# HorizonRobotics/HoloAgent

Hardware: AMD Instinct MI355X
Metric: HMSG frames/sec (one scene per GPU: map A1-A2, fusion A3-A5, merge A6, pooling A7, floors A8, rooms by the device watershed N1, room clouds, room embeddings and View nodes A9, objects with the view <-> object test A10 and graph assembly A11, nothing handed in -- plus 1000 coarse-to-fine retrieval qu (higher is better)
Workload: dtype f64 geometry / f32 features

## Files before the change

### holoagent_amd/csrc/hmsg_api.hip

```cpp
#include "hmsg_common.h"
#include "hmsg_ckdtree.h"
#include "hmsg_nn.h"

#include <algorithm>
#include <cstring>

void hmsg_bitset_and_fp(hmsg_ctx* h, int first, int n, int M, const unsigned char* d_masks, const float* d_fg,
                        const float* d_fm, const float* d_fc, const int* d_nmask);

__global__ void k_nn_patch(const long long* __restrict__ qid, const int* __restrict__ val, unsigned n, int* __restrict__ target) {
    const unsigned i = blockIdx.x * blockDim.x + threadIdx.x;
    if (i < n) target[qid[i]] = val[i];
}

void hmsg_kd_join(hmsg_ctx* h) {
    if (h->kd_thread.joinable()) h->kd_thread.join();
}

void hmsg_kd_start(hmsg_ctx* h) {
    hmsg_kd_join(h);
    h->host_pts.resize((size_t)h->V * 3);
    if (h->V) HIP_TRY(hipMemcpyAsync(h->host_pts.data(), h->pts.p, (size_t)h->V * 24, hipMemcpyDeviceToHost, h->stream));
    HIP_TRY(hipStreamSynchronize(h->stream));
    h->kd = std::make_shared<CKDTree>();
    std::shared_ptr<CKDTree> kd = h->kd;
    const double* pts = h->host_pts.data();
    const long long V = h->V;
    h->kd_thread = std::thread([kd, pts, V] { kd->build(pts, V); });
}

bool hmsg_resolve_ties(hmsg_ctx* h, TieBuf& tb, int* target) {
    unsigned n = 0;
    HIP_TRY(hipMemcpyAsync(&n, tb.count.p, 4, hipMemcpyDeviceToHost, h->stream));
    HIP_TRY(hipStreamSynchronize(h->stream));
    if (n == 0) return true;
    if (n > tb.cap) {
        tb.cap = 0;
        tb.prepare(h->stream, n + n / 2 + 1024);
        return false;
    }
    std::vector<TieRec> recs(n);
    HIP_TRY(hipMemcpy(recs.data(), tb.recs.p, (size_t)n * sizeof(TieRec), hipMemcpyDeviceToHost));
    hmsg_kd_join(h);
    std::vector<long long> q(n);
    std::vector<int> v(n);
    for (unsigned i = 0; i < n; ++i) {
        const double x[3] = {recs[i].x, recs[i].y, recs[i].z};
        q[i] = recs[i].qid;
        v[i] = (int)h->kd->query1(x);
    }
    tb.pq.ensure(n);
    tb.pv.ensure(n);
    HIP_TRY(hipMemcpyAsync(tb.pq.p, q.data(), (size_t)n * 8, hipMemcpyHostToDevice, h->stream));
    HIP_TRY(hipMemcpyAsync(tb.pv.p, v.data(), (size_t)n * 4, hipMemcpyHostToDevice, h->stream));
    hipLaunchKernelGGL(k_nn_patch, dim3(cdiv(n, 256)), dim3(256), 0, h->stream, (const long long*)tb.pq.p, (const int*)tb.pv.p, n,
                       target);
    HMSG_CHECK_LAUNCH();
    HIP_TRY(hipStreamSynchronize(h->stream));
    h->n_tie_queries += n;
    return true;
}

namespace {

void copy_in(void* dst, const void* src, size_t bytes, hipStream_t s) {
    if (!bytes) return;
    HIP_TRY(hipMemcpyAsync(dst, src, bytes, hmsg_is_device_ptr(src) ? hipMemcpyDeviceToDevice : hipMemcpyHostToDevice, s));
}

template <typename F>
int guard(hmsg_ctx* h, F&& fn) {
    try {
        if (h) HIP_TRY(hipSetDevice(h->cfg.device_id));
        fn();
        return HMSG_OK;
    } catch (const hmsg_error& e) {
        if (h) h->err = e.msg;
        return e.code;
    } catch (const std::exception& e) {
        if (h) h->err = e.what();
        return HMSG_ERR_INVALID;
    } catch (...) {
        if (h) h->err = "unknown error";
        return HMSG_ERR_INVALID;
    }
}

static const size_t FRAME_STORE_LARGE = (size_t)96 << 30;
void alloc_frame_store(hmsg_ctx* h) {
    const size_t HW = (size_t)h->cfg.height * h->cfg.width, F = (size_t)h->cfg.max_frames, NW = (size_t)h->NW;
    const size_t b_rgb = HW * 3 * F, b_depth = HW * 2 * F, b_bits = HW * NW * 8 * F, b_nn = HW * 4 * F;
    auto up = [](size_t v) { return (v + ((size_t)1 << 21) - 1) & ~(((size_t)1 << 21) - 1); };
    if (b_rgb + b_depth + b_bits + b_nn >= FRAME_STORE_LARGE) {
        h->frame_arena.alloc(up(b_rgb) + up(b_depth) + up(b_bits) + up(b_nn));
        unsigned char* p = h->frame_arena.p;
        h->rgb.view(p, HW * 3 * F);
        p += up(b_rgb);
        h->depth.view((unsigned short*)p, HW * F);
        p += up(b_depth);
        h->bits.view((unsigned long long*)p, HW * NW * F);
        p += up(b_bits);
        h->nn.view((int*)p, HW * F);
    } else {
        h->rgb.alloc(HW * 3 * F);
        h->depth.alloc(HW * F);
    }
}

void release_frame_store_if_large(hmsg_ctx* h) {
    const size_t bytes = h->rgb.bytes() + h->depth.bytes() + h->bits.bytes() + h->nn.bytes();
    if (bytes < FRAME_STORE_LARGE || h->n_fused < h->n_feat_frames) return;
    HIP_TRY(hipStreamSynchronize(h->stream));
    h->rgb.release();
    h->depth.release();
    h->bits.release();
    h->nn.release();
    h->frame_arena.release();
    h->frames_released = true;
    if (h->fold_pipe) dev_cache().trim();
}

}

extern "C" {

const char* hmsg_version(void) { return "hmsg-mi355x 0.1 (gfx950)"; }

void hmsg_default_config(hmsg_config* c) {
    memset(c, 0, sizeof(*c));
    c->device_id = 0;
    c->feat_dim = 512;
    c->height = 480;
    c->width = 640;
    c->max_frames = 1024;
    c->max_masks = 64;
    c->voxel_size = 0.05;
    c->depth_scale = 1000.0;
    c->init_overlap_thresh = 0.75;
    c->overlap_thresh_factor = 0.025;
    c->iou_thresh = 0.05;
    c->clip_masked_weight = 0.4418;
    c->max_mask_distance = 10000.0;
    c->merge_type = HMSG_MERGE_SEQUENTIAL;
    c->outlier_nb_points = 1000;
    c->outlier_radius = 1.0;
    c->pool_max_dist = 0.8;
    c->feat_dbscan_eps = 0.01;
    c->feat_dbscan_min = 100;
    c->merge_dbscan_eps = 0.1;
    c->merge_dbscan_min = 10;
    c->min_instance_points = 10;
    c->skip_frames = 1;
    c->depth_cut = 0.0;
    c->grid_resolution = 0.05;
    c->overlap_distance_form = HMSG_OVERLAP_DIRECT;
}

size_t hmsg_config_size(void) { return sizeof(hmsg_config); }

int hmsg_create(const hmsg_config* cfg, hmsg_t** out) {
    if (!cfg || !out) return HMSG_ERR_INVALID;
    *out = nullptr;
    if (cfg->feat_dim <= 0 || cfg->height <= 0 || cfg->width <= 0 || cfg->max_frames <= 0 || cfg->voxel_size <= 0 ||
        cfg->max_masks <= 0 || cfg->max_masks > 256)
        return HMSG_ERR_INVALID;
    hmsg_ctx* h = new hmsg_ctx();
    h->cfg = *cfg;
    h->NW = (cfg->max_masks + 63) / 64;
    h->MS = h->NW * 64;
    int rc = guard(h, [&] {
        int ndev = 0;
        HIP_TRY(hipGetDeviceCount(&ndev));
        HMSG_REQUIRE(cfg->device_id >= 0 && cfg->device_id < ndev, HMSG_ERR_INVALID, "device_id out of range");
        HIP_TRY(hipSetDevice(cfg->device_id));
        HIP_TRY(hipStreamCreateWithFlags(&h->stream, hipStreamNonBlocking));
        alloc_frame_store(h);
        h->pose.alloc((size_t)16 * cfg->max_frames);
    });
    if (rc != HMSG_OK) {
        fprintf(stderr, "hmsg_create: %s\n", h->err.c_str());
        delete h;
        return rc;
    }
    *out = h;
    return HMSG_OK;
}

void hmsg_destroy(hmsg_t* h) {
    if (!h) return;
    hmsg_kd_join(h);
    (void)hipSetDevice(h->cfg.device_id);
    try {
        hmsg_fold_pipe_abort(h);
    } catch (...) {
    }
    h->fold_cache.trim();
    if (h->stream) {
        (void)hipStreamSynchronize(h->stream);
        (void)hipStreamDestroy(h->stream);
    }
    delete h;
}

const char* hmsg_last_error(const hmsg_t* h) { return h ? h->err.c_str() : "null handle"; }

void hmsg_release_cached_memory(void) { dev_cache().trim(); }

int hmsg_reset(hmsg_t* h) {
    if (!h) return HMSG_ERR_INVALID;
    return guard(h, [&] {
        HIP_TRY(hipStreamSynchronize(h->stream));
        hmsg_kd_join(h);
        hmsg_fold_pipe_abort(h);
        h->n_tie_queries = 0;
        h->n_frames = h->n_feat_frames = h->n_fused = 0;
        h->n_offered = 0;
        h->room_n = 0;
        h->room_total = 0;
        if (h->frames_released) {
            alloc_frame_store(h);
            h->frames_released = false;
        }
        h->nmask.clear();
        h->mask_first.clear();
        h->have_K = false;
        h->map_ready = h->feats_final = h->merged = h->pooled = h->inst_denoised = h->tree_partial = false;
        h->frame_window = 0;
        h->nodes.clear();
        h->V = h->V0 = 0;
        h->masks3d.off.clear();
        h->masks3d.total = 0;
        h->inst.off.clear();
        h->inst.total = 0;
        h->prof.clear();
    });
}

int hmsg_set_profiling(hmsg_t* h, int32_t on) {
    if (!h) return HMSG_ERR_INVALID;
    h->prof.enabled = on != 0;
    h->prof.detail = on >= 2;
    return HMSG_OK;
}

static void prof_aggregate(hmsg_ctx* h, std::vector<std::string>& names, std::vector<long long>& cnt, std::vector<double>& ms,
                           std::vector<double>* work = nullptr) {
    (void)hipStreamSynchronize(h->stream);
    for (auto& e : h->prof.ev) {
        float t = 0.f;
        if (hipEventElapsedTime(&t, e.a, e.b) != hipSuccess) continue;
        size_t k = 0;
        for (; k < names.size(); ++k)
            if (names[k] == e.name) break;
        if (k == names.size()) {
            names.push_back(e.name);
            cnt.push_back(0);
            ms.push_back(0.0);
            if (work) work->push_back(0.0);
        }
        cnt[k]++;
        ms[k] += t;
        if (work) (*work)[k] += e.work;
    }
}

int32_t hmsg_profile_count(hmsg_t* h) {
    if (!h) return 0;
    std::vector<std::string> n;
    std::vector<long long> c;
    std::vector<double> m;
    prof_aggregate(h, n, c, m);
    return (int32_t)n.size();
}

int hmsg_profile_entry(hmsg_t* h, int32_t i, char* name, int64_t* launches, double* total_ms, double* total_work) {
    if (!h || !name || !launches || !total_ms) return HMSG_ERR_INVALID;
    std::vector<std::string> n;
    std::vector<long long> c;
    std::vector<double> m, w;
    prof_aggregate(h, n, c, m, &w);
    if (i < 0 || i >= (int32_t)n.size()) return HMSG_ERR_INVALID;
    snprintf(name, 64, "%s", n[i].c_str());
    *launches = c[i];
    *total_ms = m[i];
    if (total_work) *total_work = w[i];
    return HMSG_OK;
}

__global__ void k_depth_cut(unsigned short* __restrict__ depth, size_t n, double limit) {
    const size_t i = (size_t)blockIdx.x * blockDim.x + threadIdx.x;
    if (i < n && (double)depth[i] > limit) depth[i] = 0;
}

int hmsg_add_frames(hmsg_t* h, int32_t n, const uint8_t* rgb, const uint16_t* depth, const double* pose, const double* K) {
    if (!h) return HMSG_ERR_INVALID;
    return guard(h, [&] {
        HMSG_REQUIRE(n >= 0 && rgb && depth && pose && K, HMSG_ERR_INVALID, "hmsg_add_frames: null argument");
        HMSG_REQUIRE(!h->map_ready, HMSG_ERR_INVALID, "hmsg_add_frames after hmsg_finalize_map");
        HMSG_REQUIRE(!h->frames_released, HMSG_ERR_INVALID, "hmsg_add_frames: the frame store was released (hmsg_reset first)");
        double Kh[9];
        if (hmsg_is_device_ptr(K)) {
            HIP_TRY(hipMemcpy(Kh, K, sizeof(Kh), hipMemcpyDeviceToHost));
        } else {
            memcpy(Kh, K, sizeof(Kh));
        }
        if (h->have_K)
            HMSG_REQUIRE(memcmp(Kh, h->K, sizeof(Kh)) == 0, HMSG_ERR_UNSUPPORTED, "intrinsics must be the same for all frames");
        memcpy(h->K, Kh, sizeof(Kh));
        h->have_K = true;
        h->cam = CamK{Kh[0], Kh[4], Kh[2], Kh[5]};
        const size_t HW = (size_t)h->cfg.height * h->cfg.width;
        const int skip = std::max(1, h->cfg.skip_frames);
        int kept = 0;
        if (skip == 1) {
            HMSG_REQUIRE(h->n_frames + n <= h->cfg.max_frames, HMSG_ERR_INVALID, "frame store full (cfg.max_frames)");
            copy_in(h->rgb.p + (size_t)h->n_frames * HW * 3, rgb, (size_t)n * HW * 3, h->stream);
            copy_in(h->depth.p + (size_t)h->n_frames * HW, depth, (size_t)n * HW * 2, h->stream);
            copy_in(h->pose.p + (size_t)h->n_frames * 16, pose, (size_t)n * 16 * 8, h->stream);
            kept = n;
        } else {
            for (int i = 0; i < n; ++i) {
                if ((h->n_offered + i) % skip != 0) continue;
                HMSG_REQUIRE(h->n_frames + kept < h->cfg.max_frames, HMSG_ERR_INVALID, "frame store full (cfg.max_frames)");
                const size_t f = (size_t)h->n_frames + kept;
                copy_in(h->rgb.p + f * HW * 3, rgb + (size_t)i * HW * 3, HW * 3, h->stream);
                copy_in(h->depth.p + f * HW, depth + (size_t)i * HW, HW * 2, h->stream);
                copy_in(h->pose.p + f * 16, pose + (size_t)i * 16, 16 * 8, h->stream);
                ++kept;
            }
        }
        h->n_offered += n;
        if (h->cfg.depth_cut > 0.0 && kept > 0) {
            const size_t cnt = (size_t)kept * HW;
            hipLaunchKernelGGL(k_depth_cut, dim3(cdiv(cnt, 256)), dim3(256), 0, h->stream, h->depth.p + (size_t)h->n_frames * HW, cnt,
                               h->cfg.depth_cut * h->cfg.depth_scale);
            HMSG_CHECK_LAUNCH();
        }
        HIP_TRY(hipStreamSynchronize(h->stream));
        h->n_frames += kept;
    });
}

int hmsg_finalize_map(hmsg_t* h) {
    if (!h) return HMSG_ERR_INVALID;
    return guard(h, [&] {
        HMSG_REQUIRE(!h->map_ready, HMSG_ERR_INVALID, "map already finalised");
        hmsg_build_map(h);
    });
}
// ... 8 lines not shown
    return guard(h, [&] {
        HMSG_REQUIRE(h->map_ready, HMSG_ERR_INVALID, "map not finalised");
        if (xyz) d2h_bounce(xyz, h->pts.p, (size_t)h->V * 24);
        if (rgb) d2h_bounce(rgb, h->cols.p, (size_t)h->V * 24);
    });
}

int hmsg_add_frame_features(hmsg_t* h, int32_t first, int32_t n, int32_t M, const uint8_t* masks, const float* F_g,
                            const float* F_masked, const float* F_crop, const int32_t* n_masks) {
    if (!h) return HMSG_ERR_INVALID;
    return guard(h, [&] {
        HMSG_REQUIRE(n >= 0 && F_g, HMSG_ERR_INVALID, "hmsg_add_frame_features: null argument");
        HMSG_REQUIRE(M >= 0 && M <= h->cfg.max_masks, HMSG_ERR_INVALID, "M out of range (cfg.max_masks, <= 256)");
        HMSG_REQUIRE(M == 0 || (masks && F_masked && F_crop), HMSG_ERR_INVALID, "hmsg_add_frame_features: null argument");
        HMSG_REQUIRE(first == h->n_feat_frames, HMSG_ERR_INVALID, "frames must be handed over in order (first == #frames so far)");
        HMSG_REQUIRE(first + n <= h->n_frames, HMSG_ERR_INVALID, "features for a frame without geometry");
        HMSG_REQUIRE(!h->frames_released, HMSG_ERR_INVALID, "hmsg_add_frame_features: the frame store was released (hmsg_reset first)");
        if (n == 0) return;
        const size_t HW = (size_t)h->cfg.height * h->cfg.width;
        const int D = h->cfg.feat_dim;
        const size_t NW = (size_t)h->NW, MS = (size_t)h->MS;
        if (h->bits.n < (size_t)h->cfg.max_frames * HW * NW) h->bits.alloc((size_t)h->cfg.max_frames * HW * NW);
        if (h->fp.n < (size_t)h->cfg.max_frames * MS * D) h->fp.alloc((size_t)h->cfg.max_frames * MS * D);
        std::vector<int> nm((size_t)n, M);
        if (n_masks) {
            if (hmsg_is_device_ptr(n_masks)) {
                HIP_TRY(hipMemcpy(nm.data(), n_masks, (size_t)n * 4, hipMemcpyDeviceToHost));
            } else {
                memcpy(nm.data(), n_masks, (size_t)n * 4);
            }
            for (int v : nm) HMSG_REQUIRE(v >= 0 && v <= M, HMSG_ERR_INVALID, "n_masks[f] must be in [0, M]");
        }
        DevBuf<int> d_nm;
        d_nm.alloc((size_t)n);
        HIP_TRY(hipMemcpyAsync(d_nm.p, nm.data(), (size_t)n * 4, hipMemcpyHostToDevice, h->stream));
        if (M == 0) {
            HIP_TRY(hipMemsetAsync(h->bits.p + (size_t)first * HW * NW, 0, (size_t)n * HW * NW * 8, h->stream));
            HIP_TRY(hipStreamSynchronize(h->stream));
            h->nmask.insert(h->nmask.end(), nm.begin(), nm.end());
            h->n_feat_frames += n;
            return;
        }
        const bool dev = hmsg_is_device_ptr(masks);
        const int chunk = dev ? n : std::max(1, (int)(((size_t)512 << 20) / ((size_t)M * HW)));
        DevBuf<unsigned char> st_m;
        DevBuf<float> st_f;
        for (int c0 = 0; c0 < n; c0 += chunk) {
            int nc = std::min(chunk, n - c0);
            const unsigned char* dm = masks + (size_t)c0 * M * HW;
            const float *dg = F_g + (size_t)c0 * D, *dfm = F_masked + (size_t)c0 * M * D, *dfc = F_crop + (size_t)c0 * M * D;
            if (!dev) {
                st_m.ensure((size_t)nc * M * HW);
                HIP_TRY(hipMemcpyAsync(st_m.p, dm, (size_t)nc * M * HW, hipMemcpyHostToDevice, h->stream));
                dm = st_m.p;
            }
            if (!hmsg_is_device_ptr(F_g) || !hmsg_is_device_ptr(F_masked) || !hmsg_is_device_ptr(F_crop)) {
                st_f.ensure((size_t)nc * (2 * M + 1) * D);
                float* g = st_f.p;
                float* fm = g + (size_t)nc * D;
                float* fc = fm + (size_t)nc * M * D;
                copy_in(g, dg, (size_t)nc * D * 4, h->stream);
                copy_in(fm, dfm, (size_t)nc * M * D * 4, h->stream);
                copy_in(fc, dfc, (size_t)nc * M * D * 4, h->stream);
                dg = g;
                dfm = fm;
                dfc = fc;
            }
            hmsg_bitset_and_fp(h, first + c0, nc, M, dm, dg, dfm, dfc, d_nm.p + c0);
            HIP_TRY(hipStreamSynchronize(h->stream));
        }
        h->nmask.insert(h->nmask.end(), nm.begin(), nm.end());
        h->n_feat_frames += n;
    });
}

int hmsg_set_frame_window(hmsg_t* h, int32_t first_frame) {
    if (!h) return HMSG_ERR_INVALID;
    return guard(h, [&] {
        HMSG_REQUIRE(h->map_ready, HMSG_ERR_INVALID, "hmsg_set_frame_window: call hmsg_finalize_map first");
        HMSG_REQUIRE(h->n_feat_frames == 0 && h->n_fused == 0, HMSG_ERR_INVALID, "hmsg_set_frame_window: features already handed over");
        HMSG_REQUIRE(first_frame >= 0 && first_frame <= h->n_frames, HMSG_ERR_INVALID, "hmsg_set_frame_window: frame out of range");
        h->frame_window = first_frame;
        h->n_feat_frames = h->n_fused = first_frame;
        h->nmask.assign((size_t)first_frame, 0);
        h->mask_first.assign((size_t)first_frame + 1, 0);
        h->masks3d.off.assign(1, 0);
        h->masks3d.total = 0;
    });
}

int hmsg_merge_tree_local(hmsg_t* h, int32_t total_frames, double* th_next, int64_t* lists_now, int64_t* my_index) {
    if (!h || !th_next || !lists_now || !my_index) return HMSG_ERR_INVALID;
    return guard(h, [&] {
        long long l = 0, i = 0;
        hmsg_fold_pipe_abort(h);
        release_frame_store_if_large(h);
        hmsg_merge_tree_local_impl(h, total_frames, th_next, &l, &i);
        *lists_now = l;
        *my_index = i;
    });
}

int hmsg_merge_tree_join(hmsg_t* h, int32_t n_ext, const int64_t* ext_sizes, const double* ext_points, double th, int32_t final_pass) {
    if (!h) return HMSG_ERR_INVALID;
    return guard(h, [&] { hmsg_merge_tree_join_impl(h, n_ext, (const long long*)ext_sizes, ext_points, th, final_pass); });
}

int hmsg_fuse_frames(hmsg_t* h) {
    if (!h) return HMSG_ERR_INVALID;
    return guard(h, [&] { hmsg_fuse(h); });
}

int hmsg_get_map_feats(const hmsg_t* hc, float* feats, float* counter) {
    hmsg_ctx* h = const_cast<hmsg_ctx*>(hc);
    if (!h) return HMSG_ERR_INVALID;
    return guard(h, [&] {
        HMSG_REQUIRE(h->feats_final, HMSG_ERR_INVALID, "hmsg_fuse_frames not run");
        if (feats) d2h_bounce(feats, h->feats.p, (size_t)h->V * h->cfg.feat_dim * 4);
        if (counter) {
            std::vector<unsigned> c((size_t)h->V);
            HIP_TRY(hipMemcpy(c.data(), h->cnt.p, (size_t)h->V * 4, hipMemcpyDeviceToHost));
            for (long long i = 0; i < h->V; ++i) counter[i] = (float)c[i];
        }
    });
}

__global__ void k_feats_refresh(const float* __restrict__ sum, const unsigned* __restrict__ cnt, long long V, int D,
                                float* __restrict__ feats) {
    size_t t = (size_t)blockIdx.x * blockDim.x + threadIdx.x;
    if (t >= (size_t)V * D) return;
    unsigned c = cnt[t / D];
    float d = c == 0u ? 1e-5f : (float)c;
    feats[t] = __fdiv_rn(sum[t], d);
}

int hmsg_get_feature_sums(const hmsg_t* hc, float* sum, uint32_t* counter) {
    hmsg_ctx* h = const_cast<hmsg_ctx*>(hc);
    if (!h) return HMSG_ERR_INVALID;
    return guard(h, [&] {
        HMSG_REQUIRE(h->feats_final, HMSG_ERR_INVALID, "hmsg_fuse_frames not run");
        const size_t n = (size_t)h->V * h->cfg.feat_dim;
        if (sum && n) HIP_TRY(hipMemcpyAsync(sum, h->sum.p, n * 4, hmsg_is_device_ptr(sum) ? hipMemcpyDeviceToDevice : hipMemcpyDeviceToHost, h->stream));
        if (counter && h->V)
            HIP_TRY(hipMemcpyAsync(counter, h->cnt.p, (size_t)h->V * 4, hmsg_is_device_ptr(counter) ? hipMemcpyDeviceToDevice : hipMemcpyDeviceToHost, h->stream));
        HIP_TRY(hipStreamSynchronize(h->stream));
    });
}

int hmsg_set_feature_sums(hmsg_t* h, const float* sum, const uint32_t* counter) {
    if (!h) return HMSG_ERR_INVALID;
    return guard(h, [&] {
        HMSG_REQUIRE(h->feats_final && sum && counter, HMSG_ERR_INVALID, "hmsg_set_feature_sums: run hmsg_fuse_frames first");
        HMSG_REQUIRE(!h->pooled, HMSG_ERR_INVALID, "hmsg_set_feature_sums after hmsg_pool_instances");
        const size_t n = (size_t)h->V * h->cfg.feat_dim;
        copy_in(h->sum.p, sum, n * 4, h->stream);
        copy_in(h->cnt.p, counter, (size_t)h->V * 4, h->stream);
        if (n) hipLaunchKernelGGL(k_feats_refresh, dim3(cdiv(n, 256)), dim3(256), 0, h->stream, (const float*)h->sum.p,
                                  (const unsigned*)h->cnt.p, (long long)h->V, h->cfg.feat_dim, h->feats.p);
        HMSG_CHECK_LAUNCH();
        HIP_TRY(hipStreamSynchronize(h->stream));
    });
}

int hmsg_get_frame_nn(const hmsg_t* hc, int32_t frame, int32_t* idx) {
    hmsg_ctx* h = const_cast<hmsg_ctx*>(hc);
    if (!h) return HMSG_ERR_INVALID;
    return guard(h, [&] {
        HMSG_REQUIRE(frame >= 0 && frame < h->n_fused && idx, HMSG_ERR_INVALID, "frame not fused");
        HMSG_REQUIRE(!h->frames_released, HMSG_ERR_INVALID, "hmsg_get_frame_nn: the frame store was released by the merge (very long episode)");
        const size_t HW = (size_t)h->cfg.height * h->cfg.width;
        HIP_TRY(hipMemcpy(idx, h->nn.p + (size_t)frame * HW, HW * 4, hipMemcpyDeviceToHost));
    });
}

int hmsg_get_frame_fp(const hmsg_t* hc, int32_t frame, float* f_p) {
    hmsg_ctx* h = const_cast<hmsg_ctx*>(hc);
    if (!h) return HMSG_ERR_INVALID;
    return guard(h, [&] {
        HMSG_REQUIRE(frame >= 0 && frame < h->n_feat_frames && f_p, HMSG_ERR_INVALID, "frame has no features");
        const size_t D = (size_t)h->cfg.feat_dim, n = (size_t)h->nmask[frame] * D;
        if (n) HIP_TRY(hipMemcpy(f_p, h->fp.p + (size_t)frame * h->MS * D, n * 4, hipMemcpyDeviceToHost));
    });
}

int32_t hmsg_get_frame_num_masks(const hmsg_t* h, int32_t frame) {
    return (h && frame >= 0 && frame < h->n_feat_frames) ? h->nmask[frame] : -1;
}

int hmsg_get_frame_mask_sizes(const hmsg_t* hc, int32_t frame, int64_t* sizes) {
    hmsg_ctx* h = const_cast<hmsg_ctx*>(hc);
    if (!h) return HMSG_ERR_INVALID;
    return guard(h, [&] {
        HMSG_REQUIRE(frame >= 0 && frame < h->n_fused && sizes, HMSG_ERR_INVALID, "frame not fused");
        for (int i = 0; i < h->nmask[frame]; ++i) {
            size_t k = (size_t)h->mask_first[frame] + i;
            sizes[i] = h->masks3d.off[k + 1] - h->masks3d.off[k];
        }
    });
}

int hmsg_get_frame_mask_points(const hmsg_t* hc, int32_t frame, double* xyz) {
    hmsg_ctx* h = const_cast<hmsg_ctx*>(hc);
    if (!h) return HMSG_ERR_INVALID;
    return guard(h, [&] {
        HMSG_REQUIRE(frame >= 0 && frame < h->n_fused && xyz, HMSG_ERR_INVALID, "frame not fused");
        long long a = h->masks3d.off[(size_t)h->mask_first[frame]], b = h->masks3d.off[(size_t)h->mask_first[frame + 1]];
        if (b > a) d2h_bounce(xyz, h->masks3d.pts.p + (size_t)a * 3, (size_t)(b - a) * 24);
    });
}

int hmsg_merge_instances(hmsg_t* h) {
    if (!h) return HMSG_ERR_INVALID;
    return guard(h, [&] {
        release_frame_store_if_large(h);
        hmsg_merge(h);
    });
}

int64_t hmsg_num_instances(const hmsg_t* h) { return h && (h->merged || h->tree_partial) ? (int64_t)h->inst.off.size() - 1 : -1; }

int hmsg_get_instance_sizes(const hmsg_t* hc, int64_t* sizes) {
    hmsg_ctx* h = const_cast<hmsg_ctx*>(hc);
    if (!h) return HMSG_ERR_INVALID;
    return guard(h, [&] {
        HMSG_REQUIRE((h->merged || h->tree_partial) && sizes, HMSG_ERR_INVALID, "hmsg_merge_instances not run");
        for (size_t i = 0; i + 1 < h->inst.off.size(); ++i) sizes[i] = h->inst.off[i + 1] - h->inst.off[i];
    });
}

int hmsg_get_instance_points(const hmsg_t* hc, double* xyz) {
    hmsg_ctx* h = const_cast<hmsg_ctx*>(hc);
    if (!h) return HMSG_ERR_INVALID;
    return guard(h, [&] {
        HMSG_REQUIRE((h->merged || h->tree_partial) && xyz, HMSG_ERR_INVALID, "hmsg_merge_instances not run");
        if (h->inst.total) {
            if (hmsg_is_device_ptr(xyz)) {
                HIP_TRY(hipMemcpyAsync(xyz, h->inst.pts.p, (size_t)h->inst.total * 24, hipMemcpyDeviceToDevice, h->stream));
                HIP_TRY(hipStreamSynchronize(h->stream));
            } else
                d2h_bounce(xyz, h->inst.pts.p, (size_t)h->inst.total * 24);
        }
    });
}

int hmsg_denoise_instances(hmsg_t* h, double eps, int32_t min_points) {
    if (!h) return HMSG_ERR_INVALID;
    return guard(h, [&] {
        hmsg_denoise_inst(h, eps, min_points);
        if (eps == 0.05 && min_points == 10) h->inst_denoised = true;
    });
}

int hmsg_voxel_down_sample(hmsg_t* h, const double* points, int64_t n, double voxel_size, double* out_points, int64_t* out_n) {
    if (!h) return HMSG_ERR_INVALID;
    return guard(h, [&] {
        HMSG_REQUIRE((points || n == 0) && out_points && out_n, HMSG_ERR_INVALID, "hmsg_voxel_down_sample: null argument");
        *out_n = (int64_t)hmsg_voxel_ds(h, points, (long long)n, voxel_size, out_points);
    });
}

int hmsg_instance_room_share(hmsg_t* h, int32_t n_rooms, const int64_t* vert_off, const double* verts_xz, double radius,
                             double* share) {
    if (!h) return HMSG_ERR_INVALID;
    return guard(h, [&] {
        HMSG_REQUIRE(n_rooms >= 0 && vert_off && verts_xz && share && radius > 0, HMSG_ERR_INVALID,
                     "hmsg_instance_room_share: bad argument");
        hmsg_room_share(h, n_rooms, (const long long*)vert_off, verts_xz, radius, share);
    });
}

int hmsg_get_instance_boxes(const hmsg_t* hc, double* boxes) {
    hmsg_ctx* h = const_cast<hmsg_ctx*>(hc);
    if (!h) return HMSG_ERR_INVALID;
    return guard(h, [&] {
        HMSG_REQUIRE(h->merged && boxes, HMSG_ERR_INVALID, "hmsg_merge_instances not run");
        if (!h->inst.box.empty()) memcpy(boxes, h->inst.box.data(), h->inst.box.size() * 8);
    });
}

int hmsg_pool_instances(hmsg_t* h) {
    if (!h) return HMSG_ERR_INVALID;
    return guard(h, [&] { hmsg_pool(h); });
}

int hmsg_get_instance_feats(const hmsg_t* hc, float* feats) {
    hmsg_ctx* h = const_cast<hmsg_ctx*>(hc);
    if (!h) return HMSG_ERR_INVALID;
    return guard(h, [&] {
        HMSG_REQUIRE(h->pooled && feats, HMSG_ERR_INVALID, "hmsg_pool_instances not run");
        size_t n = (h->inst.off.size() - 1) * (size_t)h->cfg.feat_dim;
        if (n) d2h_bounce(feats, h->inst_feats.p, n * 4);
    });
}

int hmsg_test_ckdtree(const double* pts, int64_t n, const double* queries, int64_t nq, int64_t* out_idx,
                      int64_t* out_indices, int64_t* out_n_nodes) {
    if (!pts || n < 0 || nq < 0) return HMSG_ERR_INVALID;
    CKDTree t;
    t.build(pts, n);
    if (out_indices) memcpy(out_indices, t.indices.data(), (size_t)n * 8);
    if (out_n_nodes) *out_n_nodes = (int64_t)t.nodes.size();
    for (int64_t i = 0; i < nq; ++i) out_idx[i] = t.query1(queries + i * 3);
    return HMSG_OK;
}

}
// ... 1 lines not shown
```

### holoagent_amd/csrc/hmsg_comm.hip

```cpp
#include "hmsg_common.h"

#include <dlfcn.h>

#include <algorithm>

#include <functional>
#include <mutex>

__global__ void k_cm_gather_rows(const float* __restrict__ src, const int* __restrict__ row, int n, int D, float* __restrict__ dst) {
    const size_t t = (size_t)blockIdx.x * blockDim.x + threadIdx.x;
    if (t >= (size_t)n * D) return;
    dst[t] = src[(size_t)row[t / D] * D + t % D];
}
__global__ void k_cm_feats_refresh(const float* __restrict__ sum, const unsigned* __restrict__ cnt, long long V, int D, float* __restrict__ feats) {
    const size_t t = (size_t)blockIdx.x * blockDim.x + threadIdx.x;
    if (t >= (size_t)V * D) return;
    const unsigned c = cnt[t / D];
    const float d = c == 0u ? 1e-5f : (float)c;
    feats[t] = __fdiv_rn(sum[t], d);
}

namespace {

typedef void* rcclComm_t;
// ... 112 lines not shown
        if (err) *err = "unknown error";
        return HMSG_ERR_INVALID;
    }
}
}

extern "C" {

int hmsg_comm_unique_id(uint8_t* out_id) {
    if (!out_id) return HMSG_ERR_INVALID;
    return comm_guard(&g_comm_err, [&] {
        rccl_need();
        rcclUniqueId id;
        rccl_try(rccl().GetUniqueId(&id), "ncclGetUniqueId");
        memcpy(out_id, id.internal, sizeof(id.internal));
    });
}

int hmsg_comm_create(const uint8_t* id, int32_t rank, int32_t world, int32_t device_id, hmsg_comm_t** out) {
    if (!out) return HMSG_ERR_INVALID;
    *out = nullptr;
    if (world < 1 || rank < 0 || rank >= world) return HMSG_ERR_INVALID;
    hmsg_comm* c = nullptr;
    const int rc = comm_guard(&g_comm_err, [&] {
        c = new hmsg_comm();
        c->rank = rank;
        c->world = world;
        c->device = device_id;
        if (id == nullptr) {
            HMSG_REQUIRE(world == 1, HMSG_ERR_INVALID, "hmsg_comm_create: more than one rank needs the id of hmsg_comm_unique_id");
            return;
        }
        rccl_need();
        HIP_TRY(hipSetDevice(device_id));
        rcclUniqueId uid;
        memcpy(uid.internal, id, sizeof(uid.internal));
        rccl_try(rccl().CommInitRank(&c->comm, world, uid, rank), "ncclCommInitRank");
        HIP_TRY(hipMalloc((void**)&c->flag, 64));
        HIP_TRY(hipMalloc((void**)&c->hdr, (size_t)world * HMSG_COMM_HDR_BYTES));
    });
    if (rc != HMSG_OK) {
        delete c;
        return rc;
    }
    *out = c;
    return HMSG_OK;
}

void hmsg_comm_destroy(hmsg_comm_t* c) {
    if (!c) return;
    if (c->comm) (void)rccl().CommDestroy(c->comm);
    if (c->flag) (void)hipFree(c->flag);
    if (c->hdr) (void)hipFree(c->hdr);
    delete c;
}

const char* hmsg_comm_last_error(const hmsg_comm_t* c) { return c ? c->err.c_str() : g_comm_err.c_str(); }

int hmsg_allgather_nodes(hmsg_t* h, hmsg_comm_t* c, int32_t n_rooms_local, hmsg_index_t** out_index, int64_t* node_off, int64_t* room_off) {
    if (!h || !c || !out_index) return HMSG_ERR_INVALID;
    *out_index = nullptr;
    int rc_index = HMSG_OK;
    const int rc = comm_guard(&h->err, [&] {
        HIP_TRY(hipSetDevice(h->cfg.device_id));
        hipStream_t s = h->stream;
        const int W = c->world, D = h->cfg.feat_dim;
        const long long n = (long long)h->nodes.size();
        std::string mine;
        if (n_rooms_local < 0) mine = "hmsg_allgather_nodes: negative room count";
        for (long long k = 0; k < n && mine.empty(); ++k)
            if (h->nodes[(size_t)k].room < 0 || h->nodes[(size_t)k].room >= n_rooms_local) mine = "hmsg_allgather_nodes: a node's room lies outside n_rooms_local";
        if (n && !h->pooled) mine = "hmsg_allgather_nodes: run hmsg_pool_instances first";
        if (!all_ranks_ok(c, mine.empty(), s))
            throw hmsg_error{HMSG_ERR_INVALID, mine.empty() ? "hmsg_allgather_nodes: another rank's node table is invalid (see its hmsg_last_error)" : mine};
        std::vector<long long> meta((size_t)W * 2, 0);
        meta[(size_t)c->rank * 2] = n;
        meta[(size_t)c->rank * 2 + 1] = n_rooms_local;
        if (c->comm) {
            DevBuf<long long> dm;
            dm.alloc((size_t)W * 2);
            HIP_TRY(hipMemcpyAsync(dm.p + (size_t)c->rank * 2, meta.data() + (size_t)c->rank * 2, 16, hipMemcpyHostToDevice, s));
            rccl_try(rccl().AllGather(dm.p + (size_t)c->rank * 2, dm.p, 2, RCCL_INT64, c->comm, s), "ncclAllGather (counts)");
            HIP_TRY(hipMemcpyAsync(meta.data(), dm.p, (size_t)W * 16, hipMemcpyDeviceToHost, s));
            HIP_TRY(hipStreamSynchronize(s));
        }
        std::vector<long long> noff((size_t)W + 1, 0), roff((size_t)W + 1, 0);
        long long nmax = 1;
        for (int r = 0; r < W; ++r) {
            noff[(size_t)r + 1] = noff[(size_t)r] + meta[(size_t)r * 2];
            roff[(size_t)r + 1] = roff[(size_t)r] + meta[(size_t)r * 2 + 1];
            nmax = std::max(nmax, meta[(size_t)r * 2]);
        }
        const long long N = noff[(size_t)W];
        if (node_off) for (int r = 0; r <= W; ++r) node_off[r] = noff[(size_t)r];
        if (room_off) for (int r = 0; r <= W; ++r) room_off[r] = roff[(size_t)r];
        HMSG_REQUIRE(N > 0, HMSG_ERR_INVALID, "hmsg_allgather_nodes: no nodes on any rank (hmsg_build_object_nodes)");
        DevBuf<float> emb;
        DevBuf<int> room;
        float* my_emb = nullptr;
        int* my_room = nullptr;
        local_phase_then_agree(c, s, "hmsg_allgather_nodes", [&] {
        emb.alloc((size_t)W * nmax * D);
        room.alloc((size_t)W * nmax);
        my_emb = emb.p + (size_t)c->rank * nmax * D;
        my_room = room.p + (size_t)c->rank * nmax;
        if (n) {
            std::vector<int> inst((size_t)n), rm((size_t)n);
            for (long long k = 0; k < n; ++k) {
                inst[(size_t)k] = h->nodes[(size_t)k].instance;
                rm[(size_t)k] = h->nodes[(size_t)k].room + (int)roff[(size_t)c->rank];
            }
            DevBuf<int> d_inst;
            d_inst.alloc((size_t)n);
            HIP_TRY(hipMemcpyAsync(d_inst.p, inst.data(), (size_t)n * 4, hipMemcpyHostToDevice, s));
            HIP_TRY(hipMemcpyAsync(my_room, rm.data(), (size_t)n * 4, hipMemcpyHostToDevice, s));
            hipLaunchKernelGGL(k_cm_gather_rows, dim3(cdiv((size_t)n * D, 256)), dim3(256), 0, s, (const float*)h->inst_feats.p, (const int*)d_inst.p,
                               (int)n, D, my_emb);
            HMSG_CHECK_LAUNCH();
            HIP_TRY(hipStreamSynchronize(s));
        }
        });
        if (c->comm) {
            rccl_try(rccl().AllGather(my_emb, emb.p, (size_t)nmax * D, RCCL_FLOAT32, c->comm, s), "ncclAllGather (embeddings)");
            rccl_try(rccl().AllGather(my_room, room.p, (size_t)nmax, RCCL_INT32, c->comm, s), "ncclAllGather (rooms)");
        }
        DevBuf<float> packed;
        DevBuf<int> proom;
        packed.alloc((size_t)N * D);
        proom.alloc((size_t)N);
        for (int r = 0; r < W; ++r) {
            const long long nr = meta[(size_t)r * 2];
            if (!nr) continue;
            HIP_TRY(hipMemcpyAsync(packed.p + (size_t)noff[(size_t)r] * D, emb.p + (size_t)r * nmax * D, (size_t)nr * D * 4, hipMemcpyDeviceToDevice, s));
            HIP_TRY(hipMemcpyAsync(proom.p + (size_t)noff[(size_t)r], room.p + (size_t)r * nmax, (size_t)nr * 4, hipMemcpyDeviceToDevice, s));
        }
        HIP_TRY(hipStreamSynchronize(s));
        rc_index = hmsg_index_create(h->cfg.device_id, D, N, packed.p, 0, proom.p, out_index);
        if (rc_index != HMSG_OK) throw hmsg_error{rc_index, "hmsg_allgather_nodes: hmsg_index_create failed"};
    });
    if (rc != HMSG_OK) c->err = h->err;
    return rc;
}

int hmsg_allreduce_feature_sums(hmsg_t* h, hmsg_comm_t* c) {
    if (!h || !c) return HMSG_ERR_INVALID;
    const int rc = comm_guard(&h->err, [&] {
        HIP_TRY(hipSetDevice(h->cfg.device_id));
        hipStream_t s = h->stream;
        std::string mine;
        if (!h->feats_final) mine = "hmsg_allreduce_feature_sums: run hmsg_fuse_frames first";
        else if (h->pooled) mine = "hmsg_allreduce_feature_sums after hmsg_pool_instances";
        if (!all_ranks_ok(c, mine.empty(), s))
            throw hmsg_error{HMSG_ERR_INVALID, mine.empty() ? "hmsg_allreduce_feature_sums: another rank is not ready (see its hmsg_last_error)" : mine};
        const size_t n = (size_t)h->V * h->cfg.feat_dim;
        if (c->comm && n) {
            rccl_try(rccl().AllReduce(h->sum.p, h->sum.p, n, RCCL_FLOAT32, RCCL_SUM, c->comm, s), "ncclAllReduce (feature sums)");
            rccl_try(rccl().AllReduce(h->cnt.p, h->cnt.p, (size_t)h->V, RCCL_UINT32, RCCL_SUM, c->comm, s), "ncclAllReduce (frame counters)");
        }
        if (n) hipLaunchKernelGGL(k_cm_feats_refresh, dim3(cdiv(n, 256)), dim3(256), 0, s, (const float*)h->sum.p, (const unsigned*)h->cnt.p,
                                  (long long)h->V, h->cfg.feat_dim, h->feats.p);
        HMSG_CHECK_LAUNCH();
        HIP_TRY(hipStreamSynchronize(s));
    });
    if (rc != HMSG_OK) c->err = h->err;
    return rc;
}

}

void hmsg_comm_allgather_bytes(hmsg_ctx* h, hmsg_comm* c, const void* mine, size_t my_bytes, std::vector<std::vector<char>>& all) {
    const int W = c->world;
    all.assign((size_t)W, std::vector<char>());
    if (!c->comm) {
        all[0].assign((const char*)mine, (const char*)mine + my_bytes);
        return;
    }
    hipStream_t s = h->stream;
    std::vector<long long> len((size_t)W, 0);
    len[(size_t)c->rank] = (long long)my_bytes;
    DevBuf<long long> dl;
    dl.alloc((size_t)W);
    HIP_TRY(hipMemcpyAsync(dl.p + c->rank, &len[(size_t)c->rank], 8, hipMemcpyHostToDevice, s));
    rccl_try(rccl().AllGather(dl.p + c->rank, dl.p, 1, RCCL_INT64, c->comm, s), "ncclAllGather (table lengths)");
    HIP_TRY(hipMemcpyAsync(len.data(), dl.p, (size_t)W * 8, hipMemcpyDeviceToHost, s));
    HIP_TRY(hipStreamSynchronize(s));
    long long mx = 1;
    for (long long v : len) mx = std::max(mx, v);
    mx = (mx + 15) & ~15ll;
    DevBuf<char> buf;
    buf.alloc((size_t)W * (size_t)mx);
    if (my_bytes) HIP_TRY(hipMemcpyAsync(buf.p + (size_t)c->rank * (size_t)mx, mine, my_bytes, hipMemcpyHostToDevice, s));
    rccl_try(rccl().AllGather(buf.p + (size_t)c->rank * (size_t)mx, buf.p, (size_t)mx, RCCL_INT8, c->comm, s), "ncclAllGather (tables)");
    std::vector<char> hostbuf((size_t)W * (size_t)mx);
    HIP_TRY(hipMemcpyAsync(hostbuf.data(), buf.p, hostbuf.size(), hipMemcpyDeviceToHost, s));
    HIP_TRY(hipStreamSynchronize(s));
    for (int r = 0; r < W; ++r) all[(size_t)r].assign(hostbuf.begin() + (ptrdiff_t)((size_t)r * (size_t)mx), hostbuf.begin() + (ptrdiff_t)((size_t)r * (size_t)mx + (size_t)len[(size_t)r]));
}
int hmsg_comm_rank(const hmsg_comm* c) { return c->rank; }
int hmsg_comm_world(const hmsg_comm* c) { return c->world; }
void hmsg_comm_set_error(hmsg_comm* c, const std::string& e) { c->err = e; }
int hmsg_comm_device(const hmsg_comm* c) { return c->device; }
void hmsg_comm_local_phase_then_agree(hmsg_comm* c, hipStream_t s, const char* what, const std::function<void()>& f) {
    if (!c) {
        f();
        return;
    }
    local_phase_then_agree(c, s, what, f);
}
void hmsg_comm_allgather_header(hmsg_comm* c, const void* mine, size_t bytes, void* all, hipStream_t s) {
    if (bytes > HMSG_COMM_HDR_BYTES) throw hmsg_error{HMSG_ERR_INVALID, "hmsg_comm_allgather_header: header too long"};
    if (!c->comm) {
        memcpy(all, mine, bytes);
        return;
    }
    HIP_TRY(hipMemcpyAsync(c->hdr + (size_t)c->rank * HMSG_COMM_HDR_BYTES, mine, bytes, hipMemcpyHostToDevice, s));
    rccl_try(rccl().AllGather(c->hdr + (size_t)c->rank * HMSG_COMM_HDR_BYTES, c->hdr, HMSG_COMM_HDR_BYTES, RCCL_INT8, c->comm, s), "ncclAllGather (header)");
    std::vector<char> h((size_t)c->world * HMSG_COMM_HDR_BYTES);
    HIP_TRY(hipMemcpyAsync(h.data(), c->hdr, h.size(), hipMemcpyDeviceToHost, s));
    HIP_TRY(hipStreamSynchronize(s));
    for (int r = 0; r < c->world; ++r) memcpy((char*)all + (size_t)r * bytes, h.data() + (size_t)r * HMSG_COMM_HDR_BYTES, bytes);
}
void hmsg_comm_allgather_inplace(hmsg_comm* c, void* buf, size_t slot_bytes, hipStream_t s) {
    if (!c->comm || !slot_bytes) return;
    char* b = (char*)buf;
    rccl_try(rccl().AllGather(b + (size_t)c->rank * slot_bytes, b, slot_bytes, RCCL_INT8, c->comm, s), "ncclAllGather (sharded query)");
}

extern "C" {

int hmsg_comm_send(hmsg_t* h, hmsg_comm_t* c, const void* dev_buf, int64_t bytes, int32_t dst) {
    if (!h || !c || bytes < 0 || (bytes && !dev_buf) || dst < 0 || dst >= c->world || dst == c->rank) return HMSG_ERR_INVALID;
    const int rc = comm_guard(&h->err, [&] {
        HMSG_REQUIRE(c->comm, HMSG_ERR_INVALID, "hmsg_comm_send: a communicator of one rank has nobody to send to");
        HIP_TRY(hipSetDevice(h->cfg.device_id));
        if (bytes) rccl_try(rccl().Send(dev_buf, (size_t)bytes, RCCL_INT8, dst, c->comm, h->stream), "ncclSend");
        HIP_TRY(hipStreamSynchronize(h->stream));
    });
    if (rc != HMSG_OK) c->err = h->err;
    return rc;
}
int hmsg_comm_recv(hmsg_t* h, hmsg_comm_t* c, void* dev_buf, int64_t bytes, int32_t src) {
    if (!h || !c || bytes < 0 || (bytes && !dev_buf) || src < 0 || src >= c->world || src == c->rank) return HMSG_ERR_INVALID;
    const int rc = comm_guard(&h->err, [&] {
        HMSG_REQUIRE(c->comm, HMSG_ERR_INVALID, "hmsg_comm_recv: a communicator of one rank has nobody to receive from");
        HIP_TRY(hipSetDevice(h->cfg.device_id));
        if (bytes) rccl_try(rccl().Recv(dev_buf, (size_t)bytes, RCCL_INT8, src, c->comm, h->stream), "ncclRecv");
        HIP_TRY(hipStreamSynchronize(h->stream));
    });
    if (rc != HMSG_OK) c->err = h->err;
    return rc;
}

int hmsg_merge_tree_sharded(hmsg_t* h, hmsg_comm_t* c, int32_t total_frames, int32_t* holds_result) {
    if (!h || !c || !holds_result) return HMSG_ERR_INVALID;
    *holds_result = 0;
    const int rc = comm_guard(&h->err, [&] {
        HIP_TRY(hipSetDevice(h->cfg.device_id));
        hipStream_t s = h->stream;
        const int W = c->world, me = c->rank;
        const double factor = h->cfg.overlap_thresh_factor;
        auto next_th = [&](double th, long long lists) { return lists > 1 ? th - factor * (double)(lists - 2) / (double)std::max<long long>(1, lists - 1) : th; };
        double th = 0.0;
        int64_t lists = 0, idx = 0;
        const int rc_local = hmsg_merge_tree_local(h, total_frames, &th, &lists, &idx);
        if (!all_ranks_ok(c, rc_local == HMSG_OK, s))
            throw hmsg_error{rc_local != HMSG_OK ? rc_local : HMSG_ERR_INVALID,
                             rc_local != HMSG_OK ? h->err : std::string("hmsg_merge_tree_sharded: another rank's local merge failed (see its hmsg_last_error)")};
        std::vector<long long> meta((size_t)W * 2, 0);
        meta[(size_t)me * 2] = lists;
        meta[(size_t)me * 2 + 1] = idx;
        if (c->comm) {
            DevBuf<long long> dm;
            dm.alloc((size_t)W * 2);
            HIP_TRY(hipMemcpyAsync(dm.p + (size_t)me * 2, meta.data() + (size_t)me * 2, 16, hipMemcpyHostToDevice, s));
            rccl_try(rccl().AllGather(dm.p + (size_t)me * 2, dm.p, 2, RCCL_INT64, c->comm, s), "ncclAllGather (tree levels)");
            HIP_TRY(hipMemcpyAsync(meta.data(), dm.p, (size_t)W * 16, hipMemcpyDeviceToHost, s));
            HIP_TRY(hipStreamSynchronize(s));
        }
        long long target = meta[0];
        for (int r = 0; r < W; ++r) target = std::min(target, meta[(size_t)r * 2]);
        std::vector<int> owner;
        for (int r = 0; r < W; ++r) {
            long long l = meta[(size_t)r * 2], i = meta[(size_t)r * 2 + 1];
            double t = th;
            while (l > target) {
                HMSG_REQUIRE(i == l - 1 && l % 2 == 1, HMSG_ERR_INVALID,
                             "hmsg_merge_tree_sharded: rank " + std::to_string(r) + "'s frame window is not a subtree of the merge tree");
                i /= 2;
                l = (l + 1) / 2;
                t = next_th(t, l);
            }
            if ((long long)owner.size() <= i) owner.resize((size_t)i + 1, -1);
            HMSG_REQUIRE(owner[(size_t)i] < 0, HMSG_ERR_INVALID, "hmsg_merge_tree_sharded: two ranks hold list " + std::to_string(i));
            owner[(size_t)i] = r;
            if (r == me) {
                th = t;
                lists = l;
                idx = i;
            }
        }
        HMSG_REQUIRE((long long)owner.size() == lists && std::find(owner.begin(), owner.end(), -1) == owner.end(), HMSG_ERR_INVALID,
                     "hmsg_merge_tree_sharded: the ranks' windows do not cover the lists of their common level");
        if (lists == 1) {
            if (owner[0] == me) {
                const int rj = hmsg_merge_tree_join(h, 0, nullptr, nullptr, th, 1);
                if (rj != HMSG_OK) throw hmsg_error{rj, h->err};
// ... 69 lines not shown
```

### holoagent_amd/csrc/hmsg_common.h

```cpp
#pragma once
#include <hip/hip_runtime.h>

#include <algorithm>
#include <chrono>
#include <cstdarg>
#include <cstdint>
#include <cstdio>
#include <cstdlib>
#include <cstring>
#include <map>
#include <memory>
#include <mutex>
#include <thread>
#include <string>
#include <vector>

#include "../../include/hmsg.h"
#include "../../include/hmsg_test.h"

#define HMSG_WAVE 64

struct hmsg_error {
    int code;
    std::string msg;
// ... 382 lines not shown
    return v;
}
__device__ __forceinline__ int wave_sum_i32(int v) {
    for (int o = 32; o > 0; o >>= 1) v += __shfl_xor(v, o);
    return v;
}

__device__ __forceinline__ double repeat_add(double s, double p, int len) {
    while (len > 0) {
        const double as = fabs(s), ap = fabs(p);
        if (ap == 0.0) return __dadd_rn(s, p);
        const long long bs = __double_as_longlong(as);
        const int e = (int)(bs >> 52);
        if (as >= ap && ((s < 0.0) == (p < 0.0)) && e >= 1 && e < 2046) {
            unsigned long long S = ((unsigned long long)bs & 0xfffffffffffffull) | (1ull << 52);
            const double q = ldexp(ap, 1075 - e);
            if (q < 0.5) return s;
            const double qi = floor(q), qf = q - qi;
            if (qf != 0.5) {
                const unsigned long long iq = (unsigned long long)qi;
                const unsigned long long d = iq + (qf > 0.5 ? 1ull : 0ull);
                const unsigned long long top = (1ull << 53) - 1ull;
                if (S + iq <= top) {
                    unsigned long long k = (unsigned long long)len;
                    const unsigned long long room = top - iq - S;
                    if (__umul64hi(k - 1ull, d) != 0ull || (k - 1ull) * d > room) k = room / d + 1ull;
                    S += k * d;
                    const double r = ldexp((double)S, e - 1075);
                    s = s < 0.0 ? -r : r;
                    len -= (int)k;
                    continue;
                }
            }
        }
        s = __dadd_rn(s, p);
        --len;
    }
    return s;
}

__device__ __forceinline__ double wave_bcast_f64(double v, int src) {
    const long long b = __double_as_longlong(v);
    const unsigned lo = (unsigned)__builtin_amdgcn_readlane((int)(unsigned)b, src);
    const unsigned hi = (unsigned)__builtin_amdgcn_readlane((int)(unsigned)((unsigned long long)b >> 32), src);
    return __longlong_as_double((long long)(((unsigned long long)hi << 32) | lo));
}

struct MaskCloudSet {
    DevBuf<double> pts;
    std::vector<long long> off;
    long long total = 0;
};

struct InstanceSet {
    DevBuf<double> pts;
    std::vector<long long> off;
    std::vector<double> box;
    long long total = 0;
};

struct ProfEntry {
    std::string name;
    hipEvent_t a, b;
    double work;
};
struct Prof {
    bool enabled = false;
    bool detail = false;
    std::vector<ProfEntry> ev;
    void clear() {
        for (auto& e : ev) {
            (void)hipEventDestroy(e.a);
            (void)hipEventDestroy(e.b);
        }
        ev.clear();
    }
};
struct ProfScope {
    Prof* p;
    hipStream_t s;
    size_t i = 0;
    ProfScope(Prof& pr, hipStream_t st, const char* name, double work = 0.0, bool fine = false) : ProfScope(&pr, st, name, work, fine) {}
    ProfScope(Prof* pr, hipStream_t st, const char* name, double work = 0.0, bool fine = false)
        : p(pr && pr->enabled && (!fine || pr->detail) ? pr : nullptr), s(st) {
        if (!p) return;
        ProfEntry e;
        e.name = name;
        e.work = work;
        (void)hipEventCreate(&e.a);
        (void)hipEventCreate(&e.b);
        (void)hipEventRecord(e.a, s);
        i = p->ev.size();
        p->ev.push_back(e);
    }
    ~ProfScope() {
        if (p) (void)hipEventRecord(p->ev[i].b, s);
    }
};

struct hmsg_ctx {
    Prof prof;
    hmsg_config cfg;
    hipStream_t stream = nullptr;
    std::string err;
    int n_frames = 0;
    long long n_offered = 0;
    int n_feat_frames = 0;
    int n_fused = 0;
    int MS = 0;
    int NW = 0;
    std::vector<int> nmask;
    std::vector<long long> mask_first;
    CamK cam;
    double K[9];
    bool have_K = false;
    DevBuf<unsigned char> rgb;
    DevBuf<unsigned short> depth;
    DevBuf<double> pose;
    DevBuf<unsigned long long> bits;
    DevBuf<float> fp;
    DevBuf<int> nn;
    DevBuf<unsigned char> frame_arena;
    bool map_ready = false;
    GridGeom grid;
    long long V0 = 0;
    long long V = 0;
    DevBuf<unsigned long long> bitmap;
    DevBuf<unsigned> rank;
    DevBuf<double> pts;
    DevBuf<double> cols;
    std::vector<double> host_pts;
    std::shared_ptr<struct CKDTree> kd;
    std::thread kd_thread;
    long long n_tie_queries = 0;
    DevBuf<unsigned long long> bitmap_rm;
    DevBuf<unsigned> rank_rm, cand_off;
    DevBuf<int> cand;
    bool have_cand = false;
    DevBuf<float> sum;
    DevBuf<unsigned> cnt;
    bool feats_final = false;
    DevBuf<float> feats;
    MaskCloudSet masks3d;
    InstanceSet inst;
    bool merged = false;
    int frame_window = 0;
    bool tree_partial = false;
    bool frames_released = false;
    DevBuf<float> inst_feats;
    bool pooled = false;
    std::shared_ptr<struct FoldPipe> fold_pipe;
    int fold_pipe_frames = 0;
    DevCache fold_cache;
    bool inst_denoised = false;
    std::vector<hmsg_node> nodes;
    DevBuf<int> room_sel, room_fmap;
    DevBuf<long long> room_off_dev;
    std::shared_ptr<void> room_scratch;
    int room_n = 0;
    long long room_total = 0;
    std::vector<int> node_label;
    DevBuf<unsigned> scan_tmp;
};

__device__ __forceinline__ unsigned long long scan_pack(unsigned epoch, unsigned flag, unsigned value) {
    return ((unsigned long long)((epoch << 2) | flag) << 32) | (unsigned long long)value;
}
__device__ __forceinline__ unsigned scan_lookback_prefix(unsigned long long* __restrict__ state, long long tile, unsigned epoch,
                                                         unsigned agg) {
    const int lane = threadIdx.x & 63;
    if (lane == 0)
        __hip_atomic_store(&state[tile], scan_pack(epoch, tile == 0 ? 2u : 1u, agg), __ATOMIC_RELAXED, __HIP_MEMORY_SCOPE_AGENT);
    unsigned prefix = 0;
    if (tile > 0) {
        long long hi = tile - 1;
        for (;;) {
            const long long idx = hi - lane;
            unsigned long long sw = scan_pack(epoch, 2u, 0u);
            if (idx >= 0) sw = __hip_atomic_load(&state[idx], __ATOMIC_RELAXED, __HIP_MEMORY_SCOPE_AGENT);
            const unsigned tag = (unsigned)(sw >> 32);
            const unsigned flag = (tag >> 2) == (epoch & 0x3fffffffu) ? (tag & 3u) : 0u;
            const unsigned long long has_prefix = __ballot(flag == 2u), not_ready = __ballot(flag == 0u);
            unsigned long long take = ~0ull;
            if (has_prefix) {
                const int first = __ffsll(has_prefix) - 1;
                take = first == 63 ? ~0ull : ((1ull << (first + 1)) - 1ull);
            }
            if (not_ready & take) continue;
            unsigned part = ((take >> lane) & 1ull) ? (unsigned)sw : 0u;
            for (int o = 32; o > 0; o >>= 1) part += __shfl_xor(part, o);
            prefix += part;
            if (has_prefix) break;
            hi -= 64;
        }
        if (lane == 0)
            __hip_atomic_store(&state[tile], scan_pack(epoch, 2u, prefix + agg), __ATOMIC_RELAXED, __HIP_MEMORY_SCOPE_AGENT);
    }
    return prefix;
}
unsigned hmsg_scan_epoch(DevBuf<unsigned>& tmp, size_t ntiles, hipStream_t s);
void hmsg_scan_u32(const unsigned* in, unsigned* out, size_t n, hipStream_t s, DevBuf<unsigned>& tmp,
                   unsigned long long* total);
unsigned long long hmsg_bitmap_rank(const unsigned long long* bitmap, unsigned* rank, size_t nwords, hipStream_t s,
                                    DevBuf<unsigned>& tmp);

struct SortBufs {
    DevBuf<unsigned> keys, keys_alt, hist, scan_tmp;
    DevBuf<unsigned long long> vals, vals_alt;
    unsigned* res_keys = nullptr;
    unsigned long long* res_vals = nullptr;
};
void hmsg_sort_pairs(SortBufs& b, size_t n, int key_bits, hipStream_t s);
void hmsg_sort_segment_starts(const unsigned* sorted_keys, size_t n, unsigned* off, unsigned nkeys, hipStream_t s);
static inline int bits_for(unsigned long long n) {
    int b = 1;
    while (b < 63 && (1ull << b) < n) ++b;
    return b;
}

struct DbgLaps {
    const char* tag;
    hipStream_t s;
    bool on;
    std::chrono::steady_clock::time_point t;
    DbgLaps(const char* tag_, hipStream_t s_) : tag(tag_), s(s_), on(getenv("HMSG_DEBUG_TIMING") != nullptr) {
        if (on) {
            (void)hipStreamSynchronize(s);
            t = std::chrono::steady_clock::now();
        }
    }
    void lap(const char* what) {
        if (!on) return;
        (void)hipStreamSynchronize(s);
        const auto n = std::chrono::steady_clock::now();
        fprintf(stderr, "[hmsg %s] %-26s %.3f ms\n", tag, what, std::chrono::duration<double, std::milli>(n - t).count());
        t = n;
    }
};

static inline void hmsg_dump(const char* name, const void* dev, size_t bytes, hipStream_t s) {
    const char* dir = getenv("HMSG_DEBUG_DUMP");
    if (!dir || !bytes) return;
    std::vector<char> host(bytes);
    (void)hipStreamSynchronize(s);
    (void)hipMemcpy(host.data(), dev, bytes, hipMemcpyDeviceToHost);
    std::string path = std::string(dir) + "/" + name + ".bin";
    if (FILE* f = fopen(path.c_str(), "wb")) {
        fwrite(host.data(), 1, bytes, f);
        fclose(f);
    }
}

void hmsg_kd_start(hmsg_ctx* h);
void hmsg_kd_join(hmsg_ctx* h);
void hmsg_build_map(hmsg_ctx* h);
void hmsg_fuse(hmsg_ctx* h);
void hmsg_merge(hmsg_ctx* h);
void hmsg_fold_pipe_feed(hmsg_ctx* h, int f0, int nfr);
void hmsg_fold_pipe_abort(hmsg_ctx* h);
void hmsg_merge_tree_local_impl(hmsg_ctx* h, int total_frames, double* th_next, long long* lists_now, long long* my_index);
void hmsg_merge_tree_join_impl(hmsg_ctx* h, int n_ext, const long long* ext_sizes, const double* ext_pts, double th, int final_pass);
void hmsg_denoise_inst(hmsg_ctx* h, double eps, int min_points);
void hmsg_room_share(hmsg_ctx* h, int R, const long long* vert_off, const double* verts_xz, double radius,
                     double* share_out);
void hmsg_pool(hmsg_ctx* h);
long long hmsg_voxel_ds(hmsg_ctx* h, const double* pts, long long n, double vs, double* out);
```

### holoagent_amd/csrc/hmsg_fuse.hip

```cpp
#include "hmsg_common.h"

#include <hip/hip_fp16.h>

#include <algorithm>
#include <cmath>

#define FB 64
#define MFIX_SCALE 17592186044416.0

__global__ void k_bitset(const unsigned char* __restrict__ masks, int M, size_t HW, int nfr, size_t mask_stride_frame,
                         const int* __restrict__ nmask, int NW, unsigned long long* __restrict__ bits) {
    const size_t chunks = (HW + 15) / 16;
    size_t t = (size_t)blockIdx.x * blockDim.x + threadIdx.x;
    if (t >= chunks * nfr) return;
    int f = (int)(t / chunks);
    size_t p0 = (t - (size_t)f * chunks) * 16;
    const unsigned char* mf = masks + (size_t)f * mask_stride_frame;
    const int nm = min(nmask[f], M);
    unsigned long long* o = bits + ((size_t)f * HW + p0) * NW;
    _Pragma("unroll") for (int w = 0; w < 4; ++w) if (w < NW) {
        unsigned long long b[16];
        for (int j = 0; j < 16; ++j) b[j] = 0ull;
        const int i0 = w * 64, i1 = min(nm, i0 + 64);
        if (p0 + 16 <= HW && (HW & 15) == 0) {
// ... 448 lines not shown
            const unsigned long long rec = recs[k];
            const double* p = pts + (size_t)(rec >> 8) * 3;
            s_len[k - c0] = (unsigned char)(rec & 255ull);
            s_v[k - c0] = (unsigned)(rec >> 8);
            s_p[k - c0][0] = p[0];
            s_p[k - c0][1] = p[1];
            s_p[k - c0][2] = p[2];
        }
        __syncthreads();
        const unsigned e = r1 < c1 ? r1 : c1;
        for (;;) {
            if (rem == 0) {
                if (r >= e) break;
                const unsigned i = r - c0;
                rem = (int)s_len[i];
                px = s_p[i][0];
                py = s_p[i][1];
                pz = s_p[i][2];
                ++r;
                while (r < e && s_v[r - c0] == s_v[i]) rem += (int)s_len[r++ - c0];
                n += (unsigned long long)rem;
                if (rem >= 256) {
                    sx = repeat_add(sx, px, rem);
                    sy = repeat_add(sy, py, rem);
                    sz = repeat_add(sz, pz, rem);
                    rem = 0;
                    continue;
                }
            }
            sx = __dadd_rn(sx, px);
            sy = __dadd_rn(sy, py);
            sz = __dadd_rn(sz, pz);
            --rem;
        }
        __syncthreads();
    }
    if (live) {
        const double dn = (double)n;
        out[(size_t)s * 3 + 0] = __ddiv_rn(sx, dn);
        out[(size_t)s * 3 + 1] = __ddiv_rn(sy, dn);
        out[(size_t)s * 3 + 2] = __ddiv_rn(sz, dn);
    }
}

__global__ void __launch_bounds__(256) k_mwalk_heavy(const unsigned* __restrict__ off, const unsigned long long* __restrict__ recs,
                                                     const double* __restrict__ pts, double* __restrict__ out,
                                                     const unsigned* __restrict__ heavy_cnt, const unsigned* __restrict__ heavy_list) {
    const int lane = threadIdx.x & 63;
    const unsigned nwaves = (gridDim.x * blockDim.x) >> 6, nheavy = *heavy_cnt;
    if (__ballot(1) == 0ull) return;
    const unsigned long long top = (1ull << 53) - 1ull;
    for (unsigned t = (blockIdx.x * blockDim.x + threadIdx.x) >> 6; t < nheavy; t += nwaves) {
        const unsigned slot = heavy_list[t];
        const unsigned r0 = off[slot], r1 = off[slot + 1];
        double res[3];
        unsigned long long n = 0;
        for (int c = 0; c < 3; ++c) {
            double s = 0.0;
            for (unsigned rb = r0; rb < r1; rb += 64) {
                const int cnt = (int)min(64u, r1 - rb);
                const unsigned long long rec = lane < cnt ? recs[rb + lane] : 0ull;
                const int len = (int)(rec & 255ull);
                const double p = lane < cnt ? pts[(size_t)(rec >> 8) * 3 + c] : 0.0;
                if (c == 0) {
                    int tl = len;
                    for (int o = 32; o > 0; o >>= 1) tl += __shfl_xor(tl, o);
                    n += (unsigned long long)tl;
                }
                int j0 = 0;
                while (j0 < cnt) {
                    const double as = fabs(s);
                    const long long bs = __double_as_longlong(as);
                    const int e = (int)(bs >> 52);
                    const unsigned long long S = ((unsigned long long)bs & 0xfffffffffffffull) | (1ull << 52);
                    const bool st_ok = e >= 1 && e < 2046;
                    const double ap = fabs(p);
                    bool ok = st_ok && lane >= j0 && lane < cnt && as >= ap && (ap == 0.0 || (p < 0.0) == (s < 0.0));
                    unsigned long long d = 0ull, iq = 0ull;
                    if (ok && ap != 0.0) {
                        const double q = ldexp(ap, 1075 - e);
                        if (q >= 0.5) {
                            const double qi = floor(q), qf = q - qi;
                            iq = (unsigned long long)qi;
                            d = iq + (qf > 0.5 ? 1ull : 0ull);
                            ok = qf != 0.5 && d < (1ull << 44);
                        }
                    }
                    const unsigned long long inc = ok ? (unsigned long long)len * d : 0ull;
                    unsigned long long pre = inc;
                    for (int o = 1; o < 64; o <<= 1) {
                        const unsigned long long u = __shfl_up(pre, o);
                        if (lane >= o) pre += u;
                    }
                    const bool fits = ok && S + pre - d + iq <= top;
                    const unsigned long long todo = ((cnt == 64 ? ~0ull : ((1ull << cnt) - 1ull)) >> j0) << j0;
                    const unsigned long long bad = ~__ballot(fits) & todo;
                    const int f = bad ? __ffsll(bad) - 1 : cnt;
                    if (f > j0) {
                        const unsigned long long add = __shfl(pre, f - 1);
                        const double rr = ldexp((double)(S + add), e - 1075);
                        s = s < 0.0 ? -rr : rr;
                    }
                    if (f < cnt) s = repeat_add(s, wave_bcast_f64(p, f), __builtin_amdgcn_readlane(len, f));
                    j0 = f + 1;
                }
            }
            res[c] = s;
        }
        if (lane == 0) {
            const double dn = (double)n;
            out[(size_t)slot * 3 + 0] = __ddiv_rn(res[0], dn);
            out[(size_t)slot * 3 + 1] = __ddiv_rn(res[1], dn);
            out[(size_t)slot * 3 + 2] = __ddiv_rn(res[2], dn);
        }
    }
}

__global__ void k_gather_u32(const unsigned* __restrict__ src, const long long* __restrict__ idx, int n, unsigned* __restrict__ dst) {
    int t = blockIdx.x * blockDim.x + threadIdx.x;
    if (t < n) dst[t] = src[idx[t]];
}

template <int VEC, int NJ>
static void launch_fuse(hmsg_ctx* h, const unsigned* stamp, int f0, int nfr) {
    const size_t HW = (size_t)h->cfg.height * h->cfg.width;
    hipLaunchKernelGGL((k_fuse<VEC, NJ>), dim3(cdiv((size_t)h->V * 64, 256)), dim3(256), 0, h->stream, stamp, h->V, f0, nfr,
                       h->MS, h->NW, h->cfg.feat_dim, HW, (const unsigned long long*)h->bits.p, (const float*)h->fp.p, h->sum.p,
                       h->cnt.p);
    HMSG_CHECK_LAUNCH();
}

static void dispatch_fuse(hmsg_ctx* h, const unsigned* stamp, int f0, int nfr) {
    const int D = h->cfg.feat_dim;
    if (D % 256 == 0 && D <= 1024) {
        switch (D / 256) {
            case 1: launch_fuse<4, 1>(h, stamp, f0, nfr); return;
            case 2: launch_fuse<4, 2>(h, stamp, f0, nfr); return;
            case 3: launch_fuse<4, 3>(h, stamp, f0, nfr); return;
            case 4: launch_fuse<4, 4>(h, stamp, f0, nfr); return;
        }
    }
    if (D <= 64) return launch_fuse<1, 1>(h, stamp, f0, nfr);
    if (D <= 128) return launch_fuse<1, 2>(h, stamp, f0, nfr);
    if (D <= 192) return launch_fuse<1, 3>(h, stamp, f0, nfr);
    if (D <= 256) return launch_fuse<1, 4>(h, stamp, f0, nfr);
    throw hmsg_error{HMSG_ERR_UNSUPPORTED, "feat_dim must be <= 256 or a multiple of 256 up to 1024"};
}

void hmsg_fuse(hmsg_ctx* h) {
    const hmsg_config& c = h->cfg;
    hipStream_t s = h->stream;
    HMSG_REQUIRE(h->map_ready, HMSG_ERR_INVALID, "hmsg_fuse_frames: call hmsg_finalize_map first");
    HMSG_REQUIRE(!h->feats_final || h->n_fused == h->n_feat_frames, HMSG_ERR_INVALID, "feature map already finalised");
    const int H = c.height, W = c.width, D = c.feat_dim, MS = h->MS, NW = h->NW;
    const size_t HW = (size_t)H * W;
    const long long V = h->V;
    const float scale = (float)c.depth_scale;
    if (h->sum.n < (size_t)V * D || h->n_fused == h->frame_window) {
        h->sum.alloc((size_t)V * D);
        h->cnt.alloc((size_t)V);
        h->sum.zero(s);
        h->cnt.zero(s);
    }
    if (h->nn.n < (size_t)c.max_frames * HW) h->nn.alloc((size_t)c.max_frames * HW);
    DevBuf<unsigned> stamp;
    stamp.alloc((size_t)std::max<long long>(V, 1) * FB);
    const int nmask_max = FB * MS;
    DevBuf<unsigned long long> d_bounds, d_dstat;
    d_bounds.alloc((size_t)nmask_max * 6);
    d_dstat.alloc((size_t)nmask_max * 2);
    DevBuf<MaskGeom> d_geom;
    d_geom.alloc((size_t)nmask_max);
    DevBuf<unsigned long long> mbitmap;
    DevBuf<unsigned> mrank, chunk_recs, rec_off, heavy, run_count;
    DevBuf<unsigned long long> runs;
    const unsigned heavy_thr = getenv("HMSG_DEBUG_MWALK_HEAVY") ? (unsigned)atoi(getenv("HMSG_DEBUG_MWALK_HEAVY")) : 32u;
    DevBuf<long long> d_offidx;
    DevBuf<unsigned> d_offval;
    d_offidx.alloc((size_t)nmask_max);
    d_offval.alloc((size_t)nmask_max);
    SortBufs sb;
    TieBuf ties;
    std::vector<unsigned long long> hb((size_t)nmask_max * 6), hd((size_t)nmask_max * 2);
    std::vector<MaskGeom> hg((size_t)nmask_max);
    std::vector<long long> hoffidx((size_t)nmask_max);
    std::vector<unsigned> hoffval((size_t)nmask_max);
    if (h->masks3d.off.empty()) h->masks3d.off.assign(1, 0);
    if (h->mask_first.empty()) h->mask_first.assign(1, 0);
    const double filt_mm = c.max_mask_distance * c.depth_scale;

    for (int fb0 = h->n_fused; fb0 < h->n_feat_frames; fb0 += FB) {
        const int nb = std::min(FB, h->n_feat_frames - fb0);
        stamp.zero(s);
        for (;;) {
            ties.prepare(s);
            {
                ProfScope ps(h->prof, s, "k_nn", (double)nb * ((double)HW * 6.0 + 128.0));
                hipLaunchKernelGGL(k_nn, dim3(cdiv(HW * nb, 256)), dim3(256), 0, s, (const unsigned short*)h->depth.p,
                                   (const double*)h->pose.p, h->cam, scale, H, W, fb0, nb, hmsg_nn_index(h), h->nn.p, ties.list());
            }
            HMSG_CHECK_LAUNCH();
            if (hmsg_resolve_ties(h, ties, h->nn.p)) break;
        }
        hipLaunchKernelGGL(k_stamp, dim3(cdiv(HW * nb, 256)), dim3(256), 0, s, (const int*)h->nn.p, HW, fb0, nb, stamp.p);
        HMSG_CHECK_LAUNCH();
        {
            ProfScope ps(h->prof, s, "k_fuse", (double)V * 256.0);
            dispatch_fuse(h, stamp.p, fb0, nb);
        }
        const int nmask = nb * MS;
        const unsigned cpf = cdiv(HW, MCHUNK);
        const unsigned nchunks = cpf * (unsigned)nb;
        for (int i = 0; i < nmask; ++i)
            for (int a = 0; a < 6; ++a) hb[(size_t)i * 6 + a] = a < 3 ? ~0ull : 0ull;
        HIP_TRY(hipMemcpyAsync(d_bounds.p, hb.data(), (size_t)nmask * 48, hipMemcpyHostToDevice, s));
        HIP_TRY(hipMemsetAsync(d_dstat.p, 0, (size_t)nmask * 16, s));
        runs.ensure((size_t)nchunks * MCHUNK * (size_t)(1 + NW));
        run_count.ensure((size_t)nchunks);
        {
            ProfScope ps(h->prof, s, "k_mbounds", (double)nb * (double)HW * (6.0 + 8.0 * NW));
            hipLaunchKernelGGL(k_mbounds, dim3(cpf, nb), dim3(256), 0, s, (const int*)h->nn.p, (const unsigned long long*)h->bits.p,
                               (const unsigned short*)h->depth.p, HW, W, fb0, NW, MS, (const double*)h->pts.p, d_bounds.p,
                               d_dstat.p, runs.p, run_count.p);
        }
        HMSG_CHECK_LAUNCH();
        HIP_TRY(hipMemcpyAsync(hb.data(), d_bounds.p, (size_t)nmask * 48, hipMemcpyDeviceToHost, s));
        HIP_TRY(hipMemcpyAsync(hd.data(), d_dstat.p, (size_t)nmask * 16, hipMemcpyDeviceToHost, s));
        HIP_TRY(hipStreamSynchronize(s));
        long long nwords = 0;
        for (int i = 0; i < nmask; ++i) {
            MaskGeom& mg = hg[i];
            mg.word_off = nwords;
            mg.pad = 0;
            const bool none = hb[(size_t)i * 6] == ~0ull;
            const bool far = !none && (double)hd[(size_t)i * 2] / (double)hd[(size_t)i * 2 + 1] > filt_mm;
            if (none || far) {
                mg.ox = mg.oy = mg.oz = 0.0;
                mg.nx = mg.ny = mg.nz = 0;
                continue;
            }
            double mn[3], mx[3];
            for (int a = 0; a < 3; ++a) {
                mn[a] = dec_f64(hb[(size_t)i * 6 + a]);
                mx[a] = dec_f64(hb[(size_t)i * 6 + 3 + a]);
            }
            mg.ox = mn[0] - c.voxel_size * 0.5;
            mg.oy = mn[1] - c.voxel_size * 0.5;
            mg.oz = mn[2] - c.voxel_size * 0.5;
            mg.nx = (int)std::floor((mx[0] - mg.ox) / c.voxel_size) + 2;
            mg.ny = (int)std::floor((mx[1] - mg.oy) / c.voxel_size) + 2;
            mg.nz = (int)std::floor((mx[2] - mg.oz) / c.voxel_size) + 2;
            nwords += ((long long)mg.nx * mg.ny * mg.nz + 63) / 64;
        }
        long long npts = 0;
        std::vector<long long> start(nmask + 1, 0);
        if (nwords) {
            HMSG_REQUIRE(nwords < (1ll << 31), HMSG_ERR_UNSUPPORTED, "mask grids of one frame batch exceed 2^31 words");
            HIP_TRY(hipMemcpyAsync(d_geom.p, hg.data(), (size_t)nmask * sizeof(MaskGeom), hipMemcpyHostToDevice, s));
            mbitmap.ensure((size_t)nwords);
            mrank.ensure((size_t)nwords);
            chunk_recs.ensure((size_t)nchunks + 1);
            HIP_TRY(hipMemsetAsync(mbitmap.p, 0, (size_t)nwords * 8, s));
            {
                ProfScope ps(h->prof, s, "k_mmark", (double)nb * (double)HW * (4.0 + 8.0 * NW));
                hipLaunchKernelGGL(k_mmark, dim3(cpf, nb), dim3(256), 0, s, (const unsigned long long*)runs.p, (const unsigned*)run_count.p, NW,
                                   MS, (const double*)h->pts.p, (const MaskGeom*)d_geom.p, c.voxel_size, mbitmap.p, chunk_recs.p);
            }
            HMSG_CHECK_LAUNCH();
            npts = (long long)hmsg_bitmap_rank(mbitmap.p, mrank.p, (size_t)nwords, s, h->scan_tmp);
            unsigned long long nrec = 0;
            hmsg_scan_u32(chunk_recs.p, chunk_recs.p, (size_t)nchunks, s, h->scan_tmp, &nrec);
            HMSG_REQUIRE(npts < (1ll << 32) && nrec < (1ull << 32), HMSG_ERR_UNSUPPORTED, "mask batch too large");
            sb.keys.ensure((size_t)std::max<unsigned long long>(nrec, 1));
            sb.vals.ensure((size_t)std::max<unsigned long long>(nrec, 1));
            {
                ProfScope ps(h->prof, s, "k_memit", (double)nb * (double)HW * (4.0 + 8.0 * NW) + (double)nrec * 12.0);
                hipLaunchKernelGGL(k_memit, dim3(cpf, nb), dim3(256), 0, s, (const unsigned long long*)runs.p, (const unsigned*)run_count.p, NW,
                                   MS, (const double*)h->pts.p, (const MaskGeom*)d_geom.p, c.voxel_size,
                                   (const unsigned long long*)mbitmap.p, (const unsigned*)mrank.p, (const unsigned*)chunk_recs.p,
                                   sb.keys.p, sb.vals.p);
            }
            HMSG_CHECK_LAUNCH();
            {
                ProfScope ps(h->prof, s, "sort_mask_recs", (double)nrec * 12.0 * 4.0);
                hmsg_sort_pairs(sb, (size_t)nrec, bits_for((unsigned long long)npts), s);
            }
            rec_off.ensure((size_t)npts + 1);
            hmsg_sort_segment_starts(sb.res_keys, (size_t)nrec, rec_off.p, (unsigned)npts, s);
            size_t need = (size_t)(h->masks3d.total + npts) * 3;
            if (need > h->masks3d.pts.n) {
                DevBuf<double> bigger;
                bigger.alloc(std::max(need * 2, (size_t)1 << 20));
                if (h->masks3d.total)
                    HIP_TRY(hipMemcpyAsync(bigger.p, h->masks3d.pts.p, (size_t)h->masks3d.total * 24, hipMemcpyDeviceToDevice, s));
                HIP_TRY(hipStreamSynchronize(s));
                bigger.swap(h->masks3d.pts);
            }
            {
                ProfScope ps(h->prof, s, "k_mwalk", (double)nrec * 8.0 + (double)npts * 32.0);
                heavy.ensure((size_t)npts + 1);
                HIP_TRY(hipMemsetAsync(heavy.p, 0, 4, s));
                hipLaunchKernelGGL(k_mwalk, dim3(cdiv((size_t)npts, 256)), dim3(256), 0, s, (const unsigned*)rec_off.p,
                                   (const unsigned long long*)sb.res_vals, npts, (const double*)h->pts.p,
                                   h->masks3d.pts.p + (size_t)h->masks3d.total * 3, heavy.p, heavy.p + 1, heavy_thr);
                hipLaunchKernelGGL(k_mwalk_heavy, dim3(2048), dim3(256), 0, s, (const unsigned*)rec_off.p,
                                   (const unsigned long long*)sb.res_vals, (const double*)h->pts.p,
                                   h->masks3d.pts.p + (size_t)h->masks3d.total * 3, (const unsigned*)heavy.p,
                                   (const unsigned*)(heavy.p + 1));
            }
            HMSG_CHECK_LAUNCH();
            if (getenv("HMSG_DEBUG_TIMING"))
                fprintf(stderr, "[hmsg fuse] batch at frame %d: mask voxels %lld  records %llu  bitmap words %lld\n", fb0, npts, nrec, nwords);
            int ng = 0;
            for (int i = 0; i < nmask; ++i)
                if (hg[i].nx) hoffidx[ng++] = hg[i].word_off;
            HIP_TRY(hipMemcpyAsync(d_offidx.p, hoffidx.data(), (size_t)ng * 8, hipMemcpyHostToDevice, s));
            hipLaunchKernelGGL(k_gather_u32, dim3(cdiv(ng, 256)), dim3(256), 0, s, (const unsigned*)mrank.p,
                               (const long long*)d_offidx.p, ng, d_offval.p);
            HMSG_CHECK_LAUNCH();
            HIP_TRY(hipMemcpyAsync(hoffval.data(), d_offval.p, (size_t)ng * 4, hipMemcpyDeviceToHost, s));
            HIP_TRY(hipStreamSynchronize(s));
            start.assign(nmask + 1, npts);
            int k = 0;
            for (int i = 0; i < nmask; ++i)
                if (hg[i].nx) start[i] = hoffval[k++];
            for (int i = nmask - 1; i >= 0; --i)
                if (!hg[i].nx) start[i] = start[i + 1];
        }
        for (int fl = 0; fl < nb; ++fl) {
            const int nm = h->nmask[(size_t)fb0 + fl];
            for (int i = 0; i < nm; ++i) h->masks3d.off.push_back(h->masks3d.total + start[(size_t)fl * MS + i + 1]);
            h->mask_first.push_back(h->mask_first.back() + nm);
        }
        h->masks3d.total += npts;
        h->n_fused = fb0 + nb;
        hmsg_fold_pipe_feed(h, fb0, nb);
    }
    h->feats.alloc((size_t)std::max<long long>(V, 1) * D);
    hipLaunchKernelGGL(k_feats_final, dim3(cdiv((size_t)V * D, 256)), dim3(256), 0, s, (const float*)h->sum.p,
                       (const unsigned*)h->cnt.p, V, D, h->feats.p);
    HMSG_CHECK_LAUNCH();
    HIP_TRY(hipStreamSynchronize(s));
    h->feats_final = true;
}

void hmsg_bitset_and_fp(hmsg_ctx* h, int first, int n, int M, const unsigned char* d_masks, const float* d_fg,
                        const float* d_fm, const float* d_fc, const int* d_nmask) {
    const size_t HW = (size_t)h->cfg.height * h->cfg.width;
    const int D = h->cfg.feat_dim;
    const size_t chunks = (HW + 15) / 16;
    {
        ProfScope ps(h->prof, h->stream, "k_bitset", (double)n * (double)HW * (M + 8.0 * h->NW));
        hipLaunchKernelGGL(k_bitset, dim3(cdiv(chunks * n, 256)), dim3(256), 0, h->stream, d_masks, M, HW, n, (size_t)M * HW,
                           d_nmask, h->NW, h->bits.p + (size_t)first * HW * h->NW);
    }
    HMSG_CHECK_LAUNCH();
    const float wm = (float)h->cfg.clip_masked_weight, wc = (float)(1.0 - h->cfg.clip_masked_weight);
    hipLaunchKernelGGL(k_fp, dim3(n), dim3(256), 0, h->stream, d_fg, d_fm, d_fc, M, D, wm, wc, d_nmask, h->MS,
                       h->fp.p + (size_t)first * h->MS * D);
    HMSG_CHECK_LAUNCH();
}
```

### holoagent_amd/csrc/hmsg_merge.hip

```cpp
#include "hmsg_cloudops.h"

#include <algorithm>
#include <cmath>
#include <numeric>
#include <chrono>
#include <unordered_map>
#include <condition_variable>
#include <deque>
#include <mutex>
#include <thread>

namespace {

struct Cloud {
    long long off = 0;
    int n = 0;
    double mn[3] = {0, 0, 0}, mx[3] = {0, 0, 0};
    bool fixed = false;
    bool fresh = true;
    bool raw = false;
    bool anchor = false;
    unsigned long long uid = 0;
    unsigned id = 0;
    int cap = 0;
    bool has_index = false;
    bool has_index_before = false;
    int nb = 0;
    long long ix_cell = 0, ix_pt = 0;
    int gd[3] = {0, 0, 0};
    float bmn[3] = {0, 0, 0};
    bool has_delta = false;
    long long ix_cell2 = 0, ix_pt2 = 0;
    int gd2[3] = {0, 0, 0};
    float dmn[3] = {0, 0, 0};
};

template <typename T>
__device__ __forceinline__ int find_entry(const T* __restrict__ e, int n, unsigned blk) {
    int lo = 0, hi = n - 1;
    while (lo < hi) {
        const int mid = (lo + hi + 1) >> 1;
        if ((unsigned)e[mid].blk0 <= blk) lo = mid; else hi = mid - 1;
    }
    return lo;
}

struct OvGrid {
    int blk0, next;
    long long pt_off;
    long long ix_pt;
    long long ix_cell;
    int n, gx, gy, gz;
    float mnx, mny, mnz, mxx, mxy, mxz;
    double ox, oy, oz, cell;
};

struct OvTask {
    int x, y;
    int dep_n;
    int blk0;
};

struct OvSpec {
    OvGrid g;
    int seg, singleton, inherit, nb_first, n_first, n_in, out_mode, delta_always;
    long long out_off;
    long long ncell;
};
__host__ __device__ inline int ov_spec_decide(const OvSpec& sp, int n_out, int first_kept, int* first, int* n_idx) {
    *first = 0;
    *n_idx = 0;
    if (n_out <= 0) return 0;
    if (sp.singleton && n_out == sp.n_in) return 0;
    const bool inherit = sp.inherit && first_kept >= 0 && first_kept == sp.n_first && sp.nb_first > 0;
    if (inherit && sp.nb_first == n_out) return 1;
    const bool delta = inherit && sp.nb_first < n_out &&
                       (sp.delta_always || ((long long)(n_out - sp.nb_first) * 4 <= (long long)sp.nb_first && sp.ncell <= 4ll * sp.nb_first));
    *first = delta ? sp.nb_first : 0;
    *n_idx = n_out - *first;
    return delta ? 2 : 3;
}
__host__ __device__ inline void ov_spec_result(const OvSpec& sp, const unsigned* res, int K, int* n_out, int* first_kept, int* start) {
    const int oend = (int)res[sp.seg], ostart = (int)res[(size_t)K * 16 + 8 + sp.seg], ofirst = (int)res[(size_t)K * 17 + 8 + sp.seg];
    *start = ostart;
    *n_out = sp.out_mode == 2 ? sp.n_first + oend : oend - ostart;
    *first_kept = sp.n_first <= 0 ? -1 : (sp.out_mode == 2 ? sp.n_first : (sp.n_first < sp.n_in ? ofirst - ostart : *n_out));
}
__global__ void k_ov_spec(const OvSpec* __restrict__ spec , int nspec, const unsigned* __restrict__ res, int K,
                          OvGrid* __restrict__ out) {
    const int j = blockIdx.x * blockDim.x + threadIdx.x;
    if (j >= nspec) return;
    const OvSpec sp = spec[j];
    int n_out, first_kept, start, first, n_idx;
    ov_spec_result(sp, res, K, &n_out, &first_kept, &start);
    ov_spec_decide(sp, n_out, first_kept, &first, &n_idx);
    OvGrid g = sp.g;
    g.n = n_idx;
    g.pt_off = sp.out_off + (sp.out_mode == 0 ? (long long)start : 0ll) + first;
    out[j] = g;
}

}

__device__ __forceinline__ long long ov_cell(const OvGrid& g, float x, float y, float z) {
    int ix = (int)floor(((double)x - g.ox) / g.cell), iy = (int)floor(((double)y - g.oy) / g.cell),
        iz = (int)floor(((double)z - g.oz) / g.cell);
    ix = min(max(ix, 0), g.gx - 1);
    iy = min(max(iy, 0), g.gy - 1);
    iz = min(max(iz, 0), g.gz - 1);
    return g.ix_cell + ((long long)ix * g.gy + iy) * g.gz + iz;
}
static const int OVI_CHUNK = 512;
__global__ void k_ov_count(const double* __restrict__ pool, const OvGrid* __restrict__ gr, int ngr, unsigned* __restrict__ cursor,
                           long long cursor_base, int chunk) {
    const OvGrid g = gr[find_entry(gr, ngr, blockIdx.x)];
    const int i0 = (int)(blockIdx.x - (unsigned)g.blk0) * chunk, i1 = min(g.n, i0 + chunk);
    for (int i = i0 + threadIdx.x; i < i1; i += blockDim.x) {
        const double* p = pool + (size_t)(g.pt_off + i) * 3;
        atomicAdd(&cursor[ov_cell(g, (float)p[0], (float)p[1], (float)p[2]) - cursor_base], 1u);
    }
}
__global__ void k_ov_fill(const double* __restrict__ pool, const OvGrid* __restrict__ gr, int ngr, const unsigned* __restrict__ cells,
                          unsigned* __restrict__ cursor, long long cursor_base, float* __restrict__ sorted, int chunk) {
    const OvGrid g = gr[find_entry(gr, ngr, blockIdx.x)];
    const int i0 = (int)(blockIdx.x - (unsigned)g.blk0) * chunk, i1 = min(g.n, i0 + chunk);
    for (int i = i0 + threadIdx.x; i < i1; i += blockDim.x) {
        const double* p = pool + (size_t)(g.pt_off + i) * 3;
        float x = (float)p[0], y = (float)p[1], z = (float)p[2];
        long long c = ov_cell(g, x, y, z);
        size_t pos = (size_t)g.ix_pt + cells[c] + (atomicSub(&cursor[c - cursor_base], 1u) - 1u);
        sorted[(size_t)pos * 3] = x;
        sorted[(size_t)pos * 3 + 1] = y;
        sorted[(size_t)pos * 3 + 2] = z;
    }
}

#define OV_UNROLL 4
__device__ __forceinline__ float ov_norm2(float a, float b, float c) { return __fadd_rn(__fadd_rn(__fmul_rn(a, a), __fmul_rn(b, b)), __fmul_rn(c, c)); }
template <bool BLAS>
__device__ __forceinline__ float ov_dist2(float x, float y, float z, float qx, float qy, float qz, float nx) {
    if (!BLAS) {
        const float ddx = __fsub_rn(x, qx), ddy = __fsub_rn(y, qy), ddz = __fsub_rn(z, qz);
        return __fadd_rn(__fadd_rn(__fmul_rn(ddx, ddx), __fmul_rn(ddy, ddy)), __fmul_rn(ddz, ddz));
    }
    const float ip = __fmaf_rn(z, qz, __fmaf_rn(y, qy, __fmul_rn(x, qx)));
    const float d = __fsub_rn(__fadd_rn(nx, ov_norm2(qx, qy, qz)), __fmul_rn(2.0f, ip));
    return d < 0.f ? 0.f : d;
}
template <bool BLAS = false>
__device__ __forceinline__ bool ov_scan(const float* __restrict__ sorted, unsigned s0, unsigned e0, float x, float y, float z,
                                        float r2, unsigned* ncand = nullptr, float nx = 0.f) {
    for (unsigned k = s0; k < e0; k += OV_UNROLL) {
        bool h = false;
#pragma unroll
        for (int j = 0; j < OV_UNROLL; ++j) {
            const unsigned kk = min(k + (unsigned)j, e0 - 1u);
            const float d2 = ov_dist2<BLAS>(x, y, z, sorted[(size_t)kk * 3], sorted[(size_t)kk * 3 + 1], sorted[(size_t)kk * 3 + 2], nx);
            h = h || (k + (unsigned)j < e0 && d2 < r2);
        }
        if (ncand) *ncand += min(OV_UNROLL, (int)(e0 - k));
        if (h) return true;
    }
    return false;
}

struct OvProbe {
    int cx, cy, cz, z0, z1;
    bool own, any;
};
__device__ __forceinline__ OvProbe ov_probe(const OvGrid& Y, float x, float y, float z) {
    OvProbe p;
    p.cx = (int)floor(((double)x - Y.ox) / Y.cell);
    p.cy = (int)floor(((double)y - Y.oy) / Y.cell);
    p.cz = (int)floor(((double)z - Y.oz) / Y.cell);
    p.z0 = max(p.cz - 1, 0);
// ... 214 lines not shown
    }
    for (int o = 32; o > 0; o >>= 1) local += __shfl_xor(local, o);
    if ((threadIdx.x & 63) == 0 && local) atomicAdd(&counts[ti], local);
}
#define OV2_MAX_PAIRS 2048
template <bool BLAS, bool STATS>
__global__ void __launch_bounds__(256) k_ov_query_second(const double* __restrict__ pool, const OvGrid* __restrict__ gr, const OvTask* __restrict__ tasks,
                                                         const unsigned* __restrict__ cells, const float* __restrict__ sorted, float r2, float r,
                                                         int npairs, unsigned* __restrict__ counts, double th, int chunk,
                                                         unsigned long long* __restrict__ st, int sorted_src) {
    __shared__ unsigned s_off[OV2_MAX_PAIRS + 1];
    __shared__ unsigned s_w[4], s_carry;
    const int tid = threadIdx.x, lane = tid & 63, wv = tid >> 6;
    if (tid == 0) s_carry = 0u;
    __syncthreads();
    for (int k0 = 0; k0 < npairs; k0 += 256) {
        const int k = k0 + tid;
        unsigned nch = 0;
        if (k < npairs) {
            const OvTask t = tasks[npairs + k];
            const bool first_decides = (double)counts[k] / (double)t.dep_n > th;
            const bool bounded = counts[npairs + k] == 0x80000000u;
            if (!first_decides && !bounded) nch = ((unsigned)gr[t.x].n + (unsigned)chunk - 1u) / (unsigned)chunk;
        }
        unsigned incl = nch;
        for (int o = 1; o < 64; o <<= 1) {
            const unsigned u = __shfl_up(incl, o);
            if (lane >= o) incl += u;
        }
        if (lane == 63) s_w[wv] = incl;
        __syncthreads();
        unsigned base = s_carry;
        for (int q = 0; q < wv; ++q) base += s_w[q];
        if (k < npairs) s_off[k] = base + incl - nch;
        __syncthreads();
        if (tid == 0) s_carry += s_w[0] + s_w[1] + s_w[2] + s_w[3];
        __syncthreads();
    }
    if (tid == 0) s_off[npairs] = s_carry;
    __syncthreads();
    const unsigned total = s_off[npairs];
    for (unsigned j = blockIdx.x; j < total; j += gridDim.x) {
        int lo = 0, hi = npairs - 1;
        while (lo < hi) {
            const int mid = (lo + hi + 1) >> 1;
            if (s_off[mid] <= j) lo = mid; else hi = mid - 1;
        }
        const OvTask t = tasks[npairs + lo];
        const OvGrid X = gr[t.x], Y = gr[t.y];
        const int b0 = (int)(j - s_off[lo]) * chunk;
        const int b1 = b0 + chunk < X.n ? b0 + chunk : X.n;
        unsigned local = ov_probe_chunk<BLAS, STATS>(pool, gr, X, Y, t.x, t.y, cells, sorted, r2, r, b0, b1, sorted_src, st);
        for (int o = 32; o > 0; o >>= 1) local += __shfl_xor(local, o);
        if (lane == 0 && local) atomicAdd(&counts[npairs + lo], local);
    }
}

static const int CAT_CHUNK = 512;
__global__ void k_concat(const double* __restrict__ pool, const CatSeg* __restrict__ segs, int nsegs, double* __restrict__ dst,
                         const unsigned char* __restrict__ poolcore, unsigned char* __restrict__ dstcore, int chunk) {
    const CatSeg sg = segs[find_entry(segs, nsegs, blockIdx.x)];
    const long long p0 = (long long)(blockIdx.x - (unsigned)sg.blk0) * chunk, p1 = min((long long)sg.n, p0 + chunk);
    for (long long i = p0 * 3 + threadIdx.x; i < p1 * 3; i += blockDim.x) dst[sg.dst * 3 + i] = pool[sg.src * 3 + i];
    if (dstcore)
        for (long long i = p0 + threadIdx.x; i < p1; i += blockDim.x)
            dstcore[sg.dst + i] = sg.anchor ? poolcore[sg.src + i] : (unsigned char)0;
}

namespace {

double bbox_iou(const Cloud& a, const Cloud& b) {
    if (a.mx[0] <= b.mn[0] || b.mx[0] <= a.mn[0] || a.mx[1] <= b.mn[1] || b.mx[1] <= a.mn[1] || a.mx[2] <= b.mn[2] ||
        b.mx[2] <= a.mn[2])
        return 0.0;
    double ov = 1, va = 1, vb = 1;
    for (int k = 0; k < 3; ++k) {
        double omin = std::max(a.mn[k], b.mn[k]), omax = std::min(a.mx[k], b.mx[k]);
        ov *= std::max(omax - omin, 0.0);
        va *= a.mx[k] - a.mn[k];
        vb *= b.mx[k] - b.mn[k];
    }
    return ov / (va + vb - ov);
}

#define HMSG_BOX_MASK_BODY                                                                                          \
    for (int j = 0; j < n; ++j)                                                                                     \
        cm[j] = (unsigned char)!((q[1] <= lo0[j]) | (hi0[j] <= q[0]) | (q[3] <= lo1[j]) | (hi1[j] <= q[2]) |        \
                                 (q[5] <= lo2[j]) | (hi2[j] <= q[4]));
#if !defined(__HIP_DEVICE_COMPILE__) && defined(__x86_64__)
__attribute__((target("avx2"))) void box_mask_avx2(int n, const double* lo0, const double* hi0, const double* lo1,
                                                   const double* hi1, const double* lo2, const double* hi2, const double* q,
                                                   unsigned char* cm) {
    HMSG_BOX_MASK_BODY
}
#endif
void box_mask(int n, const double* lo0, const double* hi0, const double* lo1, const double* hi1, const double* lo2,
              const double* hi2, const double* q, unsigned char* cm) {
#if !defined(__HIP_DEVICE_COMPILE__) && defined(__x86_64__)
    static const bool have_avx2 = __builtin_cpu_supports("avx2");
    if (have_avx2) {
        box_mask_avx2(n, lo0, hi0, lo1, hi1, lo2, hi2, q, cm);
        return;
    }
#endif
    HMSG_BOX_MASK_BODY
}

struct IntSpan {
    const int* b;
    const int* e;
    size_t size() const { return (size_t)(e - b); }
    int operator[](size_t k) const { return b[k]; }
    const int* begin() const { return b; }
    const int* end() const { return e; }
};
struct CompList {
    std::vector<int> off, mem;
    size_t size() const { return off.empty() ? 0 : off.size() - 1; }
    IntSpan operator[](size_t c) const { return IntSpan{mem.data() + off[c], mem.data() + off[c + 1]}; }
};

struct Merger {
    hmsg_ctx* h = nullptr;
    hipStream_t s = nullptr;
    CloudOps ops;
    DevBuf<double> pool;
    DevBuf<unsigned char> poolcore;
    long long pool_used = 0;
    DevBuf<unsigned> ix_cells;
    long long ix_cells_used = 0;
    DevBuf<float> ix_pts;
    long long ix_pts_used = 0;
    DevBuf<double> concat;
    DevBuf<unsigned char> concat_core;
    DevBuf<OvGrid> d_grids;
    PinnedBuf<OvGrid> h_grids;
    PinnedBuf<CatSeg> h_cat;
    DevBuf<unsigned> d_cursor;
    DevBuf<CatSeg> d_cat;
    DevBuf<unsigned long long> ovstat;
    Publisher pub_counts;
    PinnedBuf<char> h_ovpack;
    DevBuf<char> d_ovpack;
    PinnedBuf<OvSpec> h_spec[2];
    DevBuf<OvGrid> d_spec[2];
    int spec_turn = 0;
    std::vector<OvSpec> spec;
    std::vector<int> spec_of_seg;
    bool spec_wanted = getenv("HMSG_DEBUG_NO_SPEC_INDEX") == nullptr;
    double spec_built = 0, spec_built_pts = 0, spec_skipped = 0;
    size_t cursor_clean = 0;
    SpinWait spin;
    unsigned long long next_uid = 1;
    std::unordered_map<unsigned long long, double> ratio_cache;
    bool use_cache = false;
    bool use_anchor = true;
    bool inplace_wanted = getenv("HMSG_DEBUG_NO_INPLACE") == nullptr;
    double radius = 0;
    double reach = 0;
    int faiss_form = 0;
    double cell = 0;
    double eps = 0.1;
    int minpts = 10;
    double iou_thresh = 0.05;
    double tphase[6] = {0, 0, 0, 0, 0, 0};
    struct Stats {
        double steps = 0, clouds = 0, fresh_raw = 0, fresh_g = 0, pairs_raw = 0, pairs_g = 0;
        double scan1_raw = 0, scan2_raw = 0, scan1_g = 0, scan2_g = 0;
        double idx_pts = 0;
        double ccount[5] = {0, 0, 0, 0, 0}, cpts[5] = {0, 0, 0, 0, 0}, cB[5] = {0, 0, 0, 0, 0}, cmem[5] = {0, 0, 0, 0, 0};
        double cchanged[5] = {0, 0, 0, 0, 0}, cmulti[5] = {0, 0, 0, 0, 0}, ccontested[5] = {0, 0, 0, 0, 0}, cnonfixed[5] = {0, 0, 0, 0, 0};
    } st;
    bool want_stats = false;

    template <typename T>
    void grow(DevBuf<T>& b, size_t used_elems, size_t need_elems) {
        if (need_elems <= b.n) return;
        CarveScope carve;
        DevBuf<T> nb;
        nb.alloc(std::max(need_elems * 2, (size_t)1 << 18));
        if (used_elems) HIP_TRY(hipMemcpyAsync(nb.p, b.p, used_elems * sizeof(T), hipMemcpyDeviceToDevice, s));
        HIP_TRY(hipStreamSynchronize(s));
        nb.swap(b);
    }

    OvGrid grid_at(const Cloud& c, const float* lo, const int* gd, long long ix_cell, long long ix_pt, long long pt_off, int n) const {
        OvGrid g;
        g.blk0 = 0;
        g.next = -1;
        g.pt_off = pt_off;
        g.ix_cell = ix_cell;
        g.ix_pt = ix_pt;
        g.n = n;
        g.gx = gd[0];
        g.gy = gd[1];
        g.gz = gd[2];
        g.mnx = (float)c.mn[0]; g.mny = (float)c.mn[1]; g.mnz = (float)c.mn[2];
        g.mxx = (float)c.mx[0]; g.mxy = (float)c.mx[1]; g.mxz = (float)c.mx[2];
        g.ox = (double)lo[0] - 1e-3;
        g.oy = (double)lo[1] - 1e-3;
        g.oz = (double)lo[2] - 1e-3;
        g.cell = cell;
        return g;
    }
    void push_grids(const Cloud& c, std::vector<OvGrid>& g) const {
        g.push_back(grid_at(c, c.bmn, c.gd, c.ix_cell, c.ix_pt, c.off, c.n));
        g.back().blk0 = c.nb;
        if (c.has_delta) {
            g.back().next = (int)g.size();
            g.push_back(grid_at(c, c.dmn, c.gd2, c.ix_cell2, c.ix_pt2, c.off + c.nb, c.n - c.nb));
        }
    }

    void build_indices(std::vector<Cloud>& L) {
        std::vector<int> todo;
        long long ncell_new = 0, npts_new = 0;
        int maxn = 0;
        std::vector<OvGrid> g;
        unsigned nblk = 0;
        for (int i = 0; i < (int)L.size(); ++i) {
            Cloud& c = L[i];
            if (c.has_index || c.n == 0) continue;
            const float lo[3] = {(float)c.mn[0], (float)c.mn[1], (float)c.mn[2]};
            int gd[3];
            for (int a = 0; a < 3; ++a) gd[a] = (int)std::floor(((double)(float)c.mx[a] - (double)lo[a] + 2e-3) / cell) + 1;
            const long long ncell = (long long)gd[0] * gd[1] * gd[2] + 1;
            const bool delta = c.nb > 0 && c.nb < c.n && (delta_always || ((long long)(c.n - c.nb) * 4 <= (long long)c.nb && ncell <= 4ll * c.nb));
            (delta ? grid_delta : grid_full) += 1;
            (delta ? grid_delta_pts : grid_full_pts) += delta ? c.n - c.nb : c.n;
            int first = 0;
            if (delta) {
                first = c.nb;
                c.has_delta = true;
                for (int a = 0; a < 3; ++a) {
                    c.gd2[a] = gd[a];
                    c.dmn[a] = lo[a];
                }
                c.ix_cell2 = ix_cells_used + ncell_new;
                c.ix_pt2 = ix_pts_used;
                g.push_back(grid_at(c, lo, c.gd2, c.ix_cell2, c.ix_pt2, c.off + first, c.n - first));
            } else {
                c.nb = c.n;
                c.has_delta = false;
                for (int a = 0; a < 3; ++a) {
                    c.gd[a] = gd[a];
                    c.bmn[a] = lo[a];
                }
                c.ix_cell = ix_cells_used + ncell_new;
                c.ix_pt = ix_pts_used;
                g.push_back(grid_at(c, lo, c.gd, c.ix_cell, c.ix_pt, c.off, c.n));
            }
            g.back().blk0 = (int)nblk;
            nblk += cdiv((size_t)(c.n - first), OVI_CHUNK);
            ncell_new += ncell;
            npts_new += c.n - first;
            maxn = std::max(maxn, c.n - first);
            todo.push_back(i);
        }
        if (todo.empty()) return;
        HMSG_REQUIRE(ncell_new < (1ll << 32) && npts_new < (1ll << 32), HMSG_ERR_UNSUPPORTED,
                     "one batch of overlap grids exceeds 2^32 entries");
        grow(ix_cells, (size_t)ix_cells_used, (size_t)(ix_cells_used + ncell_new));
        grow(ix_pts, (size_t)ix_pts_used * 3, (size_t)(ix_pts_used + npts_new) * 3);
        d_grids.ensure(g.size());
        h_grids.ensure(g.size());
        memcpy(h_grids.p, g.data(), g.size() * sizeof(OvGrid));
        upload_pinned(d_grids.p, h_grids.p, g.size() * sizeof(OvGrid), s);
        unsigned* cells = ix_cells.p + ix_cells_used;
        {
            const unsigned* before = d_cursor.p;
            d_cursor.ensure((size_t)ncell_new);
            if (d_cursor.p != before) cursor_clean = 0;
            if (cursor_clean < (size_t)ncell_new) {
                HIP_TRY(hipMemsetAsync(d_cursor.p, 0, d_cursor.n * 4, s));
                cursor_clean = d_cursor.n;
            }
        }
        hipLaunchKernelGGL(k_ov_count, dim3(nblk), dim3(256), 0, s, (const double*)pool.p, (const OvGrid*)d_grids.p, (int)g.size(),
                           d_cursor.p, ix_cells_used, OVI_CHUNK);
        HMSG_CHECK_LAUNCH();
        hmsg_scan_u32(d_cursor.p, cells, (size_t)ncell_new, s, ops.scan_tmp, nullptr);
        hipLaunchKernelGGL(k_ov_fill, dim3(nblk), dim3(256), 0, s, (const double*)pool.p, (const OvGrid*)d_grids.p, (int)g.size(),
                           (const unsigned*)ix_cells.p, d_cursor.p, ix_cells_used, ix_pts.p, OVI_CHUNK);
        HMSG_CHECK_LAUNCH();
        for (int i : todo) L[i].has_index = true;
        ix_cells_used += ncell_new;
        ix_pts_used += npts_new;
    }

    void prebuild(std::vector<std::vector<Cloud>>& frames, size_t a, size_t b) {
        b = std::min(b, frames.size());
        std::vector<Cloud> all;
        for (size_t f = a; f < b; ++f) all.insert(all.end(), frames[f].begin(), frames[f].end());
        build_indices(all);
        spin.wait(s);
        size_t k = 0;
        for (size_t f = a; f < b; ++f)
            for (auto& cl : frames[f]) cl = all[k++];
    }

    bool needs_collect() const {
        return pool_used > (long long)gc_pool_points || ix_cells_used > (long long)gc_index_entries || ix_pts_used > (long long)gc_index_entries;
    }
    void collect(std::vector<Cloud>& G, std::vector<std::vector<Cloud>>& frames, size_t f_next) {
        long long live = 0;
        unsigned blocks = 0;
// ... 481 lines not shown
        for (auto& sd : segs) {
            if (sd.out_mode == 1) sd.out_off += pool_used;
            if (sd.out_mode == 0) dense_total += sd.n;
        }
        long long out_base = pool_used + region_total;
        if (!segs.empty() && cat_total > 0) {
            concat.ensure((size_t)cat_total * 3);
            concat_core.ensure((size_t)cat_total);
            grow(pool, (size_t)pool_used * 3, (size_t)(out_base + dense_total) * 3);
            grow(poolcore, (size_t)pool_used, (size_t)(out_base + dense_total));
            lap(3);
            DbGather ga;
            ga.pool = pool.p;
            ga.host_segs = cat.data();
            ga.nsegs = (int)cat.size();
            ga.poolcore = poolcore.p;
            ga.dstcore = use_anchor ? concat_core.p : nullptr;
            ga.pool_w = pool.p;
            ga.poolcore_w = poolcore.p;
            spec.clear();
            spec_of_seg.assign(segs.size(), -1);
            const bool speculate = spec_wanted && CloudOps::regions_supported();
            ops.dbscan_keep_largest(concat.p, segs, eps, minpts, pool.p + (size_t)out_base * 3, res,
                                    use_anchor ? (const unsigned char*)concat_core.p : nullptr, poolcore.p + out_base, &ga,
                                    speculate ? std::function<void(const unsigned*, int)>([&](const unsigned* d_res, int K) {
                                        speculate_indices(L, comps, seg_of_comp, segs, out_base, d_res, K);
                                    }) : std::function<void(const unsigned*, int)>());
            lap(4);
            if (want_stats) {
                for (size_t c = 0; c < comps.size(); ++c) {
                    if (seg_of_comp[c] < 0) continue;
                    const auto& mem = comps[c];
                    const DbscanResult& r = res[seg_of_comp[c]];
                    long long tot = 0, rest = 0;
                    bool rest_raw = true;
                    for (size_t q = 0; q < mem.size(); ++q) {
                        tot += L[mem[q]].n;
                        if (q) {
                            rest += L[mem[q]].n;
                            rest_raw = rest_raw && L[mem[q]].raw;
                        }
                    }
                    int cls;
                    if (mem.size() == 1) cls = L[mem[0]].raw ? 0 : 1;
                    else if (L[mem[0]].anchor && L[mem[0]].n > rest) cls = rest_raw ? 2 : 3;
                    else cls = 4;
                    st.ccount[cls] += 1;
                    st.cpts[cls] += tot;
                    st.cB[cls] += mem.size() == 1 ? tot : rest;
                    st.cmem[cls] += mem.size();
                    st.cchanged[cls] += r.changed;
                    st.cmulti[cls] += r.n_clusters > 1;
                    st.ccontested[cls] += r.contested != 0;
                    const bool fx = !r.changed || r.n_clusters == 1 || (r.n_clusters > 1 && !r.contested);
                    st.cnonfixed[cls] += !fx;
                }
            }
            static const bool stats_step = getenv("HMSG_DEBUG_MERGESTATS_STEP") != nullptr;
            if (stats_step) {
                long long fixed_pts = 0, big_fixed = 0, removed = 0;
                int nchanged = 0, multi = 0, multicl = 0, multicl_changed = 0;
                long long multicl_pts = 0;
                for (size_t c = 0; c < comps.size(); ++c) {
                    if (seg_of_comp[c] < 0) continue;
                    multi += comps[c].size() > 1;
                    int best = 0;
                    for (int i : comps[c])
                        if (L[i].fixed) {
                            fixed_pts += L[i].n;
                            best = std::max(best, L[i].n);
                        }
                    big_fixed += best;
                    const DbscanResult& r = res[seg_of_comp[c]];
                    nchanged += r.changed;
                    removed += segs[seg_of_comp[c]].n - r.n_out;
                    if (r.n_clusters > 1) {
                        ++multicl;
                        multicl_pts += r.n_out;
                        multicl_changed += r.changed;
                    }
                }
                fprintf(stderr, "[mstat] clouds %d pairs %zu segs %zu multi %d N %lld fixed_pts %lld anchor_pts %lld changed %d removed %lld multicl %d multicl_changed %d multicl_pts %lld\n",
                        n, pairs.size(), segs.size(), multi, cat_total, fixed_pts, big_fixed, nchanged, removed, multicl,
                        multicl_changed, multicl_pts);
            }
        } else {
            res.assign(segs.size(), DbscanResult{});
            spec.clear();
            spec_of_seg.assign(segs.size(), -1);
        }
        std::vector<int> spec_code(spec.size(), 0), spec_first(spec.size(), 0);
        std::vector<long long> spec_pt(spec.size(), 0);
        {
            long long pts = 0, cells_end = 0;
            for (size_t j = 0; j < spec.size(); ++j) {
                const DbscanResult& r = res[(size_t)spec[j].seg];
                int n_idx = 0;
                spec_code[j] = ov_spec_decide(spec[j], r.n_out, r.first_kept, &spec_first[j], &n_idx);
                spec_pt[j] = pts;
                pts += n_idx;
                if (n_idx > 0) {
                    cells_end = (spec[j].g.ix_cell - ix_cells_used) + spec[j].ncell;
                    spec_built += 1;
                    spec_built_pts += n_idx;
                    (spec_code[j] == 2 ? grid_delta : grid_full) += 1;
                    (spec_code[j] == 2 ? grid_delta_pts : grid_full_pts) += n_idx;
                } else {
                    spec_skipped += 1;
                }
            }
            for (size_t j = 0; j < spec.size(); ++j) spec_pt[j] = ix_pts_used;
            ix_cells_used += cells_end;
            ix_pts_used += pts;
        }
        std::vector<Cloud> out;
        out.reserve(comps.size());
        long long cursor = out_base;
        for (size_t c = 0; c < comps.size(); ++c) {
            const auto& mem = comps[c];
            int sg = seg_of_comp[c];
            if (sg < 0) {
                Cloud k = L[mem[0]];
                k.fresh = false;
                k.fixed = true;
                out.push_back(k);
                continue;
            }
            const DbscanResult& r = res[sg];
            if (mem.size() == 1 && !r.changed) {
                Cloud k = L[mem[0]];
                k.fresh = false;
                k.fixed = true;
                k.raw = false;
                k.off = cursor;
                k.cap = k.n;
                k.anchor = r.n_clusters == 1;
                out.push_back(k);
                cursor += r.n_out;
                continue;
            }
            Cloud k;
            const int mode = segs[sg].out_mode;
            k.off = mode ? segs[sg].out_off : cursor;
            k.cap = mode ? seg_cap[sg] : r.n_out;
            k.n = r.n_out;
            for (int a = 0; a < 3; ++a) {
                k.mn[a] = r.mn[a];
                k.mx[a] = r.mx[a];
            }
            k.fixed = !r.changed || r.n_clusters == 1 || (r.n_clusters > 1 && !r.contested);
            k.anchor = k.fixed && r.n_clusters >= 1 && (r.changed || r.n_clusters == 1);
            k.fresh = true;
            k.uid = next_uid++;
            int f = -1;
            for (int i : mem)
                if (L[i].n > 0) {
                    f = i;
                    break;
                }
            auto take_base = [&] {
                k.nb = L[f].nb;
                k.ix_cell = L[f].ix_cell;
                k.ix_pt = L[f].ix_pt;
                for (int a = 0; a < 3; ++a) {
                    k.gd[a] = L[f].gd[a];
                    k.bmn[a] = L[f].bmn[a];
                }
            };
            const int sj = spec_of_seg.empty() ? -1 : spec_of_seg[(size_t)sg];
            if (sj >= 0) {
                const OvSpec& sp = spec[(size_t)sj];
                const int code = spec_code[(size_t)sj];
                if (code == 1 || code == 2) take_base();
                if (code == 2) {
                    k.has_delta = true;
                    k.ix_cell2 = sp.g.ix_cell;
                    k.ix_pt2 = spec_pt[(size_t)sj];
                    k.gd2[0] = sp.g.gx, k.gd2[1] = sp.g.gy, k.gd2[2] = sp.g.gz;
                    for (int a = 0; a < 3; ++a) k.dmn[a] = (float)segs[sg].mn[a];
                }
                if (code == 3) {
                    k.nb = k.n;
                    k.ix_cell = sp.g.ix_cell;
                    k.ix_pt = spec_pt[(size_t)sj];
                    k.gd[0] = sp.g.gx, k.gd[1] = sp.g.gy, k.gd[2] = sp.g.gz;
                    for (int a = 0; a < 3; ++a) k.bmn[a] = (float)segs[sg].mn[a];
                }
                k.has_index = code != 0;
            } else if (inherit_grids && r.first_kept >= 0 && f >= 0 && r.first_kept == L[f].n && L[f].has_index && L[f].nb > 0) {
                take_base();
                k.has_index = k.nb == k.n;
            }
            out.push_back(k);
            if (!mode) cursor += r.n_out;
        }
        pool_used = cursor;
        lap(5);
        return out;
    }
};

}

#include "hmsg_fold.inl"

namespace {

void merger_init(Merger& m, hmsg_ctx* h) {
    const hmsg_config& c = h->cfg;
    m.h = h;
    m.s = h->stream;
    m.ops.s = h->stream;
    m.ops.prof = &h->prof;
    m.radius = 1.5 * c.voxel_size;
    m.reach = m.radius;
    m.faiss_form = c.overlap_distance_form == HMSG_OVERLAP_FAISS_BLAS ? 1 : 0;
    if (m.faiss_form) {
        const GridGeom& g = h->grid;
        double m2 = 0.0;
        const double lo[3] = {g.ox, g.oy, g.oz}, ext[3] = {g.nx * g.vs, g.ny * g.vs, g.nz * g.vs};
        for (int a = 0; a < 3; ++a) {
            const double v = std::max(std::fabs(lo[a]), std::fabs(lo[a] + ext[a])) + 1.0;
            m2 += v * v;
        }
        m.reach = std::sqrt(m.radius * m.radius + 16.0 * 5.9604644775390625e-08 * m2);
    }
    m.cell = m.reach * (1.0 + 1e-3) + 2e-3;
    m.eps = c.merge_dbscan_eps;
    m.minpts = c.merge_dbscan_min;
    m.iou_thresh = c.iou_thresh;
    m.use_anchor = !getenv("HMSG_DEBUG_NOANCHOR");
    m.want_stats = getenv("HMSG_DEBUG_MERGESTATS") != nullptr;
    HMSG_REQUIRE(c.iou_thresh >= 0.0, HMSG_ERR_UNSUPPORTED, "pipeline.iou_thresh must be >= 0");
}

std::vector<std::vector<Cloud>> seed_frames(Merger& m, hmsg_ctx* h, int first, bool legacy_grids = true, long long pool_factor = 2) {
    const int F = h->n_fused;
    const long long total = h->masks3d.total;
    m.pool.alloc((size_t)std::max<long long>(total * pool_factor, 1 << 16) * 3);
    m.poolcore.alloc((size_t)std::max<long long>(total * pool_factor, 1 << 16));
    if (total) HIP_TRY(hipMemcpyAsync(m.pool.p, h->masks3d.pts.p, (size_t)total * 24, hipMemcpyDeviceToDevice, h->stream));
    m.pool_used = total;
    std::vector<SegDesc> msegs((size_t)h->mask_first[F]);
    for (size_t id = 0; id < msegs.size(); ++id) {
        msegs[id].pt_base = h->masks3d.off[id];
        msegs[id].n = (int)(h->masks3d.off[id + 1] - h->masks3d.off[id]);
    }
    m.ops.bounds(m.pool.p, msegs);
    std::vector<std::vector<Cloud>> frames((size_t)(F - first));
    for (int f = first; f < F; ++f) {
        const int nm = (int)(h->mask_first[f + 1] - h->mask_first[f]);
        auto& fr = frames[(size_t)(f - first)];
        fr.reserve(nm);
        for (int i = 0; i < nm; ++i) {
            const SegDesc& sd = msegs[(size_t)h->mask_first[f] + i];
            if (sd.n == 0) continue;
            fr.emplace_back();
            Cloud& k = fr.back();
            k.off = sd.pt_base;
            k.n = sd.n;
            k.raw = true;
            k.uid = m.next_uid++;
            for (int a = 0; a < 3; ++a) {
                k.mn[a] = sd.mn[a];
                k.mx[a] = sd.mx[a];
            }
        }
    }
    if (!legacy_grids) return frames;
    if (h->cfg.merge_type == HMSG_MERGE_HIERARCHICAL || first != 0) {
        for (size_t a = 0; a < frames.size(); a += Merger::PREBUILD_WINDOW) m.prebuild(frames, a, a + Merger::PREBUILD_WINDOW);
    } else {
        m.prebuild(frames, 0, Merger::PREBUILD_WINDOW);
    }
    return frames;
}

void store_instances(Merger& m, hmsg_ctx* h, const std::vector<Cloud>& result, int min_points) {
    long long keep_total = 0;
    unsigned cat_blocks = 0;
    std::vector<CatSeg> cat;
    h->inst.off.assign(1, 0);
    h->inst.box.clear();
    for (auto& k : result) {
        if (k.n < min_points) continue;
        for (int a = 0; a < 3; ++a) h->inst.box.push_back(k.mn[a]);
        for (int a = 0; a < 3; ++a) h->inst.box.push_back(k.mx[a]);
        cat.push_back(CatSeg{k.off, keep_total, k.n, 0, (int)cat_blocks, 0});
        cat_blocks += cdiv((size_t)k.n, CAT_CHUNK);
        keep_total += k.n;
        h->inst.off.push_back(keep_total);
    }
    h->inst.total = keep_total;
    DevBuf<double> fresh;
    fresh.alloc((size_t)std::max<long long>(keep_total, 1) * 3);
    if (!cat.empty()) {
        m.d_cat.ensure(cat.size());
        HIP_TRY(hipMemcpyAsync(m.d_cat.p, cat.data(), cat.size() * sizeof(CatSeg), hipMemcpyHostToDevice, m.s));
        if (cat_blocks)
            hipLaunchKernelGGL(k_concat, dim3(cat_blocks), dim3(256), 0, m.s, (const double*)m.pool.p, (const CatSeg*)m.d_cat.p,
                               (int)cat.size(), fresh.p, (const unsigned char*)nullptr, (unsigned char*)nullptr, CAT_CHUNK);
        HMSG_CHECK_LAUNCH();
    }
    HIP_TRY(hipStreamSynchronize(m.s));
    fresh.swap(h->inst.pts);
}

double next_level_threshold(double th, double factor, long long lists) {
    return th - factor * (double)(lists - 2) / (double)std::max<long long>(1, lists - 1);
}

}

static bool fold_begin(Folder& m, hmsg_ctx* h, std::vector<Cloud>& G, std::vector<std::vector<Cloud>>& frames, size_t f_next) {
    const double cs = m.eps / std::sqrt(3.0) * (1.0 - 1e-7);
    if (!(m.radius + 1e-4 < 1.9 * cs)) return false;
    if (m.faiss_form) return false;
    long long live = 0, n_clouds = 0;
    for (auto& k : G) live += k.n, ++n_clouds;
    for (size_t f = f_next; f < frames.size(); ++f)
        for (auto& k : frames[f]) live += k.n, ++n_clouds;
    if (n_clouds == 0 || live >= (1ll << 28) || n_clouds >= (1ll << 23)) return false;
    CarveScope carve;
    const size_t keep_gc = m.gc_pool_points;
    m.gc_pool_points = (size_t)live * 11;
    m.collect(G, frames, f_next);
    m.gc_pool_points = keep_gc;
    double lo[3] = {1e300, 1e300, 1e300}, hi[3] = {-1e300, -1e300, -1e300};
    std::vector<FInsSeg> segs;
    auto take = [&](Cloud& k) {
        for (int a = 0; a < 3; ++a) {
            lo[a] = std::min(lo[a], k.mn[a]);
            hi[a] = std::max(hi[a], k.mx[a]);
        }
        k.id = m.next_id++;
        k.cap = k.n;
        segs.push_back(FInsSeg{k.off, k.id, k.n, 0, 0, k.anchor ? 1 : 0, 0});
    };
    for (auto& k : G) take(k);
    for (size_t f = f_next; f < frames.size(); ++f)
        for (auto& k : frames[f]) take(k);
    m.index_init(live, n_clouds, lo, hi);
    m.index_bulk(segs);
    return true;
}
static void fold_report(Folder& m, hmsg_ctx* h) {
    fprintf(stderr, "[hmsg fold] pairs(host) %.1f  overlap %.1f  tables %.1f  step kernels %.1f  bookkeeping %.1f ms\n", m.tphase[1],
            m.tphase[2], m.tphase[3], m.tphase[4], m.tphase[5]);
    fprintf(stderr, "[hmsg fold] steps %.0f  components: anchor %.0f  plain %.0f  batch %.0f   active points %.0f  relocated %.0f   ids %u\n",
            m.fstat[0], m.fstat[1], m.fstat[2], m.fstat[3], m.fstat[4], m.fstat[5], m.next_id);
    unsigned cnt[FC_N];
    HIP_TRY(hipMemcpy(cnt, m.ix_counters.p, sizeof(cnt), hipMemcpyDeviceToHost));
    fprintf(stderr, "[hmsg fold] index: %u of %u bricks, %u of %u records, hash %u slots\n", cnt[FC_BRICKS], m.ix.brick_cap, cnt[FC_RECS],
            m.ix.rec_cap, m.ix.hmask + 1);
    fprintf(stderr, "[hmsg fold] point pool: %lld points in use (%.2f GB), %lld in the frame masks\n", m.pool_used, m.pool_used * 25e-9, (long long)h->masks3d.total);
    fprintf(stderr, "[hmsg fold] walks: count %u  touch %u  link %u  label %u   touched anchor points %u\n", cnt[FC_STAT], cnt[FC_STAT + 1],
            cnt[FC_STAT + 2], cnt[FC_STAT + 3], cnt[FC_STAT + 4]);
    fprintf(stderr, "[hmsg fold] link walks: anchor comps own %u promoted %u raw %u | plain comps own %u promoted %u raw %u\n", cnt[FC_DBG], cnt[FC_DBG + 1],
            cnt[FC_DBG + 2], cnt[FC_DBG + 4], cnt[FC_DBG + 5], cnt[FC_DBG + 6]);
}

static void merge_report(Folder& m) {
    if (getenv("HMSG_DEBUG_TIMING"))
        fprintf(stderr, "[hmsg merge] index %.1f  pairs(host) %.1f  overlap %.1f  components+concat %.1f  dbscan %.1f  bookkeeping %.1f ms\n",
                m.tphase[0], m.tphase[1], m.tphase[2], m.tphase[3], m.tphase[4], m.tphase[5]);
    if (m.want_stats) {
        const auto& t = m.st;
        const double S = std::max(1.0, t.steps);
        fprintf(stderr, "[mstat] steps %.0f  per step: clouds %.1f  fresh raw %.1f  fresh G %.1f  indexed pts %.0f\n", t.steps, t.clouds / S,
                t.fresh_raw / S, t.fresh_g / S, t.idx_pts / S);
        fprintf(stderr, "[mstat] pairs/step raw %.1f (scan1 %.0f scan2 %.0f pts)   G-fresh %.1f (scan1 %.0f scan2 %.0f pts)\n", t.pairs_raw / S,
                t.scan1_raw / S, t.scan2_raw / S, t.pairs_g / S, t.scan1_g / S, t.scan2_g / S);
        if (m.ovstat.p) {
            unsigned long long hs[16];
            (void)hipMemcpy(hs, m.ovstat.p, 128, hipMemcpyDeviceToHost);
            fprintf(stderr, "[mstat] overlap probes with > 32 candidates: %.1f per step, %.0f candidates per step; longest candidate list of a probe %llu\n",
                    hs[8] / S, hs[9] / S, hs[7]);
            fprintf(stderr, "[mstat] overlap probes/step %.0f: outside the box %.0f  hit own cell %.0f  hit neighbour %.0f  miss %.0f | candidates/step own %.0f  neighbour %.0f\n",
                    hs[0] / S, hs[1] / S, hs[2] / S, hs[3] / S, hs[4] / S, hs[5] / S, hs[6] / S);
        }
        const char* nmc[5] = {"singleton raw", "singleton non-fixed", "anchor+raw", "anchor+any", "other"};
        for (int c = 0; c < 5; ++c)
            fprintf(stderr, "[mstat] dbscan class %-20s comps/step %.2f  pts/step %.0f  B pts/step %.0f  members %.2f  changed %.0f multi %.0f contested %.0f nonfixed %.0f (totals)\n",
                    nmc[c], t.ccount[c] / S, t.cpts[c] / S, t.cB[c] / S, t.ccount[c] ? t.cmem[c] / t.ccount[c] : 0.0, t.cchanged[c],
                    t.cmulti[c], t.ccontested[c], t.cnonfixed[c]);
    }
    if (getenv("HMSG_DEBUG_TIMING"))
        fprintf(stderr, "[hmsg merge] overlap grids: %.0f over whole clouds (%.0f points), %.0f delta grids (%.0f points); of them behind the DBSCAN batches: %.0f (%.0f points), %.0f not needed\n", m.grid_full,
                m.grid_full_pts, m.grid_delta, m.grid_delta_pts, m.spec_built, m.spec_built_pts, m.spec_skipped);
    if (getenv("HMSG_DEBUG_TIMING") && m.n_collects)
        fprintf(stderr, "[hmsg merge] %d collections of the point pool / grid arenas\n", m.n_collects);
    if (getenv("HMSG_DEBUG_TIMING") && m.ops.stat_calls > 0)
        fprintf(stderr, "[hmsg merge] dbscan batches %.0f: mean points %.0f  grid cells %.0f  occupied cells %.0f  counted points %.0f\n",
                m.ops.stat_calls, m.ops.stat_points / m.ops.stat_calls, m.ops.stat_cells / m.ops.stat_calls,
                m.ops.stat_core_cells / m.ops.stat_calls, m.ops.stat_needy / m.ops.stat_calls);
    if (getenv("HMSG_DEBUG_TIMING") && m.ops.stat_calls > 0)
        fprintf(stderr, "[hmsg merge] dbscan segments with a cropped anchor member: %.0f (%.0f anchor points a batch), %.0f of them in place; pool %.2f GB\n",
                m.ops.stat_forced, m.ops.stat_forced_first / m.ops.stat_calls, m.ops.stat_inplace, (double)m.pool_used * 24 / 1e9);
    if (getenv("HMSG_DEBUG_MAXCELL") && m.ops.stat_calls > 0)
        fprintf(stderr, "[hmsg merge] fullest cell of a dbscan batch: mean %.0f points, max %.0f\n", m.ops.stat_maxcell_sum / m.ops.stat_calls, m.ops.stat_maxcell_max);
}

struct SeqFold {
    Folder m;
    hmsg_ctx* h = nullptr;
    std::vector<std::vector<Cloud>> frames;
    size_t f_next = 0;
    size_t prebuilt_upto = 0;
    std::vector<Cloud> G;
    bool incremental = false, never = false;
    int f_switch = -1;
    double batch_mean = 0.0, switch_points = 1500000.0;

    void init(hmsg_ctx* hh, hipStream_t stream, Prof* prof) {
        h = hh;
        merger_init(m, h);
        m.s = stream;
        m.ops.s = stream;
        m.ops.prof = prof;
        if (const char* e = getenv("HMSG_DEBUG_GC_POINTS")) m.gc_pool_points = (size_t)atoll(e);
        never = getenv("HMSG_FOLD_LEGACY") != nullptr;
        switch_points = getenv("HMSG_FOLD_INCREMENTAL") ? 0.0 : 1500000.0;
        if (const char* e = getenv("HMSG_FOLD_SWITCH")) switch_points = atof(e);
        if (const char* e = getenv("HMSG_FOLD_BIG_ACTIVE")) m.big_active = atoll(e);
    }
    void ingest(const double* src, long long npts, const long long* off, const std::vector<int>& nm, long long reserve) {
        if (m.pool.n == 0) {
            m.pool.alloc((size_t)std::max<long long>(npts * reserve, 1 << 16) * 3);
            m.poolcore.alloc((size_t)std::max<long long>(npts * reserve, 1 << 16));
        } else {
            m.grow(m.pool, (size_t)m.pool_used * 3, (size_t)(m.pool_used + npts) * 3);
            m.grow(m.poolcore, (size_t)m.pool_used, (size_t)(m.pool_used + npts));
        }
        const long long base = m.pool_used;
        if (npts) HIP_TRY(hipMemcpyAsync(m.pool.p + (size_t)base * 3, src, (size_t)npts * 24, hipMemcpyDeviceToDevice, m.s));
        m.pool_used += npts;
        size_t nmask = 0;
        for (int v : nm) nmask += (size_t)v;
        std::vector<SegDesc> msegs(nmask);
        for (size_t id = 0; id < nmask; ++id) {
            msegs[id].pt_base = base + (off[id] - off[0]);
            msegs[id].n = (int)(off[id + 1] - off[id]);
        }
        m.ops.bounds(m.pool.p, msegs);
        size_t id = 0;
        for (int v : nm) {
            frames.emplace_back();
            auto& fr = frames.back();
            fr.reserve((size_t)v);
            for (int i = 0; i < v; ++i, ++id) {
                const SegDesc& sd = msegs[id];
                if (sd.n == 0) continue;
                fr.emplace_back();
                Cloud& k = fr.back();
                k.off = sd.pt_base;
                k.n = sd.n;
                k.raw = true;
                k.uid = m.next_uid++;
                for (int a = 0; a < 3; ++a) {
                    k.mn[a] = sd.mn[a];
                    k.mx[a] = sd.mx[a];
                }
            }
        }
    }
    bool pending() const { return f_next < frames.size(); }
    void step(bool input_complete) {
        const hmsg_config& c = h->cfg;
        const size_t f = f_next++;
        if (f == 0) {
            G = std::move(frames[0]);
            std::vector<Cloud>().swap(frames[0]);
            return;
        }
        if (!incremental && !never) {
            const double last_batch = m.ops.stat_points - m.stat_points_seen;
            m.stat_points_seen = m.ops.stat_points;
            batch_mean += (last_batch - batch_mean) / 64.0;
            if (input_complete && (switch_points <= 0.0 || batch_mean > switch_points) && fold_begin(m, h, G, frames, f)) {
                incremental = true;
                f_switch = (int)f;
            }
        }
        if (incremental) {
            G.insert(G.end(), frames[f].begin(), frames[f].end());
            std::vector<Cloud>().swap(frames[f]);
            G = m.fold_step(std::move(G), c.init_overlap_thresh);
            return;
        }
        if (m.needs_collect()) {
            m.collect(G, frames, f);
            prebuilt_upto = f;
        }
        if (f >= prebuilt_upto) {
            const size_t b = std::min(frames.size(), f + Merger::PREBUILD_WINDOW);
            m.prebuild(frames, f, b);
            prebuilt_upto = b;
        }
        G.insert(G.end(), frames[f].begin(), frames[f].end());
        std::vector<Cloud>().swap(frames[f]);
        G = m.merge_3d_masks(std::move(G), c.init_overlap_thresh);
    }
    void finish() {
        const hmsg_config& c = h->cfg;
        std::vector<Cloud> result = incremental ? m.fold_step(std::move(G), c.init_overlap_thresh) : m.merge_3d_masks(std::move(G), c.init_overlap_thresh);
        if (getenv("HMSG_DEBUG_TIMING") && incremental) {
            fprintf(stderr, "[hmsg merge] incremental fold from frame %d of %zu\n", f_switch, frames.size());
            fold_report(m, h);
        }
        store_instances(m, h, result, c.min_instance_points);
        merge_report(m);
    }
};

struct FoldPipe {
    struct Batch {
        DevBuf<double> pts;
        long long npts = 0;
        std::vector<long long> off;
        std::vector<int> nm;
    };
    hmsg_ctx* h = nullptr;
    std::thread th;
    std::mutex mu;
    std::condition_variable cv;
    std::deque<std::unique_ptr<Batch>> q;
    bool closed = false, aborted = false, failed = false;
    hmsg_error err{HMSG_OK, ""};
    Prof prof;
    std::vector<std::unique_ptr<Batch>> spent;

    void run() {
        hipStream_t s = nullptr;
        dev_cache().swap_state(h->fold_cache);
        try {
            HIP_TRY(hipSetDevice(h->cfg.device_id));
            int lo = 0, hi = 0;
            (void)hipDeviceGetStreamPriorityRange(&lo, &hi);
            HIP_TRY(hipStreamCreateWithPriority(&s, hipStreamNonBlocking, hi));
            {
                SeqFold sf;
                sf.init(h, s, &prof);
                for (;;) {
                    std::unique_ptr<Batch> b;
                    bool have = false, done = false, complete = false;
                    {
                        std::unique_lock<std::mutex> lk(mu);
                        if (!sf.pending()) cv.wait(lk, [&] { return !q.empty() || closed || aborted; });
                        if (aborted) break;
                        if (!q.empty()) {
                            b = std::move(q.front());
                            q.pop_front();
                            have = true;
                        }
                        complete = closed && q.empty();
                        done = complete && !have && !sf.pending();
                    }
                    if (have) {
                        sf.ingest(b->pts.p, b->npts, b->off.data(), b->nm, 64);
                        HIP_TRY(hipStreamSynchronize(s));
                        std::lock_guard<std::mutex> lk(mu);
                        spent.push_back(std::move(b));
                        continue;
                    }
                    if (done) {
                        if (!sf.frames.empty()) sf.finish();
                        break;
                    }
                    sf.step(complete);
                }
                HIP_TRY(hipStreamSynchronize(s));
            }
        } catch (const hmsg_error& e) {
            fail(e);
        } catch (const std::exception& e) {
            fail(hmsg_error{HMSG_ERR_HIP, e.what()});
        } catch (...) {
            fail(hmsg_error{HMSG_ERR_HIP, "merge fold worker: unknown exception"});
        }
        if (s) {
            (void)hipStreamSynchronize(s);
            (void)hipStreamDestroy(s);
        }
        h->fold_cache.swap_state(dev_cache());
    }
    void fail(const hmsg_error& e) {
        std::lock_guard<std::mutex> lk(mu);
        failed = true;
        err = e;
    }
    void push(std::unique_ptr<Batch> b) {
        std::vector<std::unique_ptr<Batch>> done;
        {
            std::lock_guard<std::mutex> lk(mu);
            if (!failed) q.push_back(std::move(b));
            done.swap(spent);
        }
        cv.notify_one();
    }
    void join(bool stop) {
        {
            std::lock_guard<std::mutex> lk(mu);
            closed = true;
            aborted = aborted || stop;
        }
        cv.notify_one();
        if (th.joinable()) th.join();
        spent.clear();
        q.clear();
    }
};

static bool fold_pipe_wanted(const hmsg_ctx* h) {
    if (h->rgb.bytes() + h->depth.bytes() + h->bits.bytes() + h->nn.bytes() >= ((size_t)96 << 30)) return false;
    return h->cfg.merge_type != HMSG_MERGE_HIERARCHICAL && h->frame_window == 0 && !getenv("HMSG_FOLD_NOPIPE") &&
           !getenv("HMSG_FOLD_INCREMENTAL") && !getenv("HMSG_FOLD_SWITCH") && !getenv("HMSG_DEBUG_GC_POINTS");
}

void hmsg_fold_pipe_feed(hmsg_ctx* h, int f0, int nfr) {
    if (h->merged || !fold_pipe_wanted(h)) return;
    if (!h->fold_pipe) {
        if (f0 != 0) return;
        h->fold_pipe = std::make_shared<FoldPipe>();
        h->fold_pipe->h = h;
        h->fold_pipe->prof.enabled = h->prof.enabled;
        FoldPipe* fp = h->fold_pipe.get();
        fp->th = std::thread([fp] { fp->run(); });
    }
    std::unique_ptr<FoldPipe::Batch> bp(new FoldPipe::Batch());
    FoldPipe::Batch& b = *bp;
    const size_t m0 = (size_t)h->mask_first[(size_t)f0], m1 = (size_t)h->mask_first[(size_t)f0 + nfr];
    b.off.assign(h->masks3d.off.begin() + (long)m0, h->masks3d.off.begin() + (long)m1 + 1);
    for (int f = f0; f < f0 + nfr; ++f) b.nm.push_back((int)(h->mask_first[(size_t)f + 1] - h->mask_first[(size_t)f]));
    b.npts = b.off.back() - b.off.front();
    b.pts.alloc((size_t)std::max<long long>(b.npts, 1) * 3);
    if (b.npts) {
        HIP_TRY(hipMemcpyAsync(b.pts.p, h->masks3d.pts.p + (size_t)b.off.front() * 3, (size_t)b.npts * 24, hipMemcpyDeviceToDevice, h->stream));
        HIP_TRY(hipStreamSynchronize(h->stream));
    }
    h->fold_pipe_frames = f0 + nfr;
    h->fold_pipe->push(std::move(bp));
}

void hmsg_fold_pipe_abort(hmsg_ctx* h) {
    if (!h->fold_pipe) return;
    h->fold_pipe->join(true);
    h->fold_pipe->prof.clear();
    h->fold_pipe.reset();
    h->fold_pipe_frames = 0;
}

void hmsg_merge(hmsg_ctx* h) {
    const hmsg_config& c = h->cfg;
    HMSG_REQUIRE(h->feats_final && h->n_fused > 0, HMSG_ERR_INVALID, "hmsg_merge_instances: run hmsg_fuse_frames first");
    HMSG_REQUIRE(!h->merged, HMSG_ERR_INVALID, "instances already merged");
    HMSG_REQUIRE(h->frame_window == 0, HMSG_ERR_INVALID, "hmsg_merge_instances on a frame window: use hmsg_merge_tree_local / _join");
    const int F = h->n_fused;
    if (h->fold_pipe && h->fold_pipe_frames == F && fold_pipe_wanted(h)) {
        std::shared_ptr<FoldPipe> fp = h->fold_pipe;
        fp->join(false);
        h->fold_pipe.reset();
        h->fold_pipe_frames = 0;
        for (auto& e : fp->prof.ev) h->prof.ev.push_back(e);
        fp->prof.ev.clear();
        if (fp->failed) throw fp->err;
        h->merged = true;
        return;
    }
    hmsg_fold_pipe_abort(h);
    if (c.merge_type == HMSG_MERGE_HIERARCHICAL) {
        Folder m;
        merger_init(m, h);
        std::vector<std::vector<Cloud>> frames = seed_frames(m, h, 0);
        m.use_cache = true;
        double th = c.init_overlap_thresh;
        std::vector<std::vector<Cloud>> lv = std::move(frames);
        while (lv.size() > 1) {
            std::vector<std::vector<Cloud>> nx;
            for (size_t i = 0; i < lv.size(); i += 2) {
                if (i == lv.size() - 1) {
                    nx.push_back(std::move(lv[i]));
                    break;
                }
                std::vector<Cloud> L = std::move(lv[i]);
                L.insert(L.end(), lv[i + 1].begin(), lv[i + 1].end());
                nx.push_back(m.merge_3d_masks(std::move(L), th));
            }
            lv = std::move(nx);
            if (lv.size() > 1) th = next_level_threshold(th, c.overlap_thresh_factor, (long long)lv.size());
        }
        std::vector<Cloud> result = m.merge_3d_masks(std::move(lv[0]), 0.75);
        store_instances(m, h, result, c.min_instance_points);
        merge_report(m);
    } else {
        SeqFold sf;
        sf.init(h, h->stream, &h->prof);
        std::vector<int> nm((size_t)F);
        for (int f = 0; f < F; ++f) nm[(size_t)f] = (int)(h->mask_first[(size_t)f + 1] - h->mask_first[(size_t)f]);
        sf.ingest(h->masks3d.pts.p, h->masks3d.total, h->masks3d.off.data(), nm, 2);
        while (sf.pending()) sf.step(true);
        sf.finish();
    }
    h->merged = true;
}

void hmsg_merge_tree_local_impl(hmsg_ctx* h, int total_frames, double* th_next, long long* lists_now, long long* my_index) {
    const hmsg_config& c = h->cfg;
    HMSG_REQUIRE(h->feats_final && h->n_fused > h->frame_window, HMSG_ERR_INVALID, "hmsg_merge_tree_local: run hmsg_fuse_frames first");
    HMSG_REQUIRE(!h->merged, HMSG_ERR_INVALID, "instances already merged");
    HMSG_REQUIRE(total_frames >= h->n_fused, HMSG_ERR_INVALID, "hmsg_merge_tree_local: total_frames smaller than the window's end");
    Merger m;
    merger_init(m, h);
    m.use_cache = true;
    std::vector<std::vector<Cloud>> lv = seed_frames(m, h, h->frame_window);
    double th = c.init_overlap_thresh;
    long long lists = total_frames, off = h->frame_window;
    while (lists > 1) {
        const long long n = (long long)lv.size();
        if (n == 1 || (off & 1) || ((n & 1) && off + n < lists)) break;
        std::vector<std::vector<Cloud>> nx;
        for (size_t i = 0; i < lv.size(); i += 2) {
            if (i == lv.size() - 1) {
                nx.push_back(std::move(lv[i]));
                break;
            }
            std::vector<Cloud> L = std::move(lv[i]);
            L.insert(L.end(), lv[i + 1].begin(), lv[i + 1].end());
            nx.push_back(m.merge_3d_masks(std::move(L), th));
        }
        lv = std::move(nx);
        off >>= 1;
        lists = (lists + 1) / 2;
        if (lists > 1) th = next_level_threshold(th, c.overlap_thresh_factor, lists);
    }
    HMSG_REQUIRE(lv.size() == 1, HMSG_ERR_UNSUPPORTED,
                 "hmsg_merge_tree_local: the frame window is not a subtree of the merge tree (first frame must be a multiple of a "
                 "power of two >= the window length)");
    store_instances(m, h, lv[0], 0);
    *th_next = th;
    *lists_now = lists;
    *my_index = off;
    h->tree_partial = true;
}

void hmsg_merge_tree_join_impl(hmsg_ctx* h, int n_ext, const long long* ext_sizes, const double* ext_pts, double th, int final_pass) {
    const hmsg_config& c = h->cfg;
    HMSG_REQUIRE(h->tree_partial, HMSG_ERR_INVALID, "hmsg_merge_tree_join: run hmsg_merge_tree_local first");
    HMSG_REQUIRE(n_ext >= 0 && (n_ext == 0 || (ext_sizes && ext_pts)), HMSG_ERR_INVALID, "hmsg_merge_tree_join: bad argument");
    Merger m;
    merger_init(m, h);
    m.use_cache = true;
    long long ext_total = 0;
    for (int k = 0; k < n_ext; ++k) ext_total += ext_sizes[k];
    const long long own = h->inst.total, total = own + ext_total;
    m.pool.alloc((size_t)std::max<long long>(total * 2, 1 << 16) * 3);
    m.poolcore.alloc((size_t)std::max<long long>(total * 2, 1 << 16));
    if (own) HIP_TRY(hipMemcpyAsync(m.pool.p, h->inst.pts.p, (size_t)own * 24, hipMemcpyDeviceToDevice, h->stream));
    if (ext_total) {
        hipPointerAttribute_t pa;
        memset(&pa, 0, sizeof(pa));
        const bool on_dev = hipPointerGetAttributes(&pa, ext_pts) == hipSuccess && pa.type == hipMemoryTypeDevice;
        if (!on_dev) (void)hipGetLastError();
        HIP_TRY(hipMemcpyAsync(m.pool.p + (size_t)own * 3, ext_pts, (size_t)ext_total * 24, on_dev ? hipMemcpyDeviceToDevice : hipMemcpyHostToDevice, h->stream));
    }
    m.pool_used = total;
    const int n_own = (int)h->inst.off.size() - 1;
    std::vector<SegDesc> segs((size_t)(n_own + n_ext));
    for (int k = 0; k < n_own; ++k) {
        segs[(size_t)k].pt_base = h->inst.off[(size_t)k];
        segs[(size_t)k].n = (int)(h->inst.off[(size_t)k + 1] - h->inst.off[(size_t)k]);
    }
    long long at = own;
    for (int k = 0; k < n_ext; ++k) {
        segs[(size_t)(n_own + k)].pt_base = at;
        segs[(size_t)(n_own + k)].n = (int)ext_sizes[k];
        at += ext_sizes[k];
    }
    m.ops.bounds(m.pool.p, segs);
    std::vector<Cloud> L;
    for (auto& sd : segs) {
        if (sd.n == 0) continue;
        Cloud k;
        k.off = sd.pt_base;
        k.n = sd.n;
        k.uid = m.next_uid++;
        for (int a = 0; a < 3; ++a) {
            k.mn[a] = sd.mn[a];
            k.mx[a] = sd.mx[a];
        }
        L.push_back(k);
    }
    std::vector<Cloud> result = n_ext > 0 ? m.merge_3d_masks(std::move(L), th) : std::move(L);
    if (final_pass) result = m.merge_3d_masks(std::move(result), 0.75);
    store_instances(m, h, result, final_pass ? c.min_instance_points : 0);
    if (final_pass) {
        h->merged = true;
        h->tree_partial = false;
    }
}

void hmsg_denoise_inst(hmsg_ctx* h, double eps, int min_points) {
    HMSG_REQUIRE(h->merged, HMSG_ERR_INVALID, "hmsg_denoise_instances: run hmsg_merge_instances first");
    const int K = (int)h->inst.off.size() - 1;
    if (K <= 0 || h->inst.total == 0) return;
    CloudOps ops;
    ops.s = h->stream;
    std::vector<SegDesc> segs(K);
    for (int k = 0; k < K; ++k) {
        segs[k].pt_base = h->inst.off[k];
        segs[k].n = (int)(h->inst.off[k + 1] - h->inst.off[k]);
    }
    ops.bounds(h->inst.pts.p, segs);
    DevBuf<double> out;
    out.alloc((size_t)h->inst.total * 3);
    std::vector<DbscanResult> res;
    long long total = ops.dbscan_keep_largest(h->inst.pts.p, segs, eps, min_points, out.p, res);
    out.swap(h->inst.pts);
    h->inst.off.assign(1, 0);
// ... 248 lines not shown
```

### holoagent_amd/csrc/hmsg_nn.h

```cpp
#pragma once
#include "hmsg_common.h"

struct NNIndex {
    GridGeom g;
    const unsigned long long* bitmap;
    const unsigned* rank;
    const double* pts;
    const unsigned long long* bitmap_rm;
    const unsigned* rank_rm;
    const unsigned* cand_off;
    const int* cand;
};

struct NNBest {
    double d2;
    int idx;
    int ntie;
};

struct TieRec {
    long long qid;
    double x, y, z;
};
struct TieList {
    unsigned* count;
    TieRec* recs;
    unsigned cap;
};
__device__ __forceinline__ void tie_push(const TieList& t, long long qid, double x, double y, double z) {
    const unsigned k = atomicAdd(t.count, 1u);
    if (k < t.cap) t.recs[k] = TieRec{qid, x, y, z};
}

__device__ __forceinline__ void nn_consider(NNBest& best, int q, double d2) {
    if (d2 < best.d2) {
        best.d2 = d2;
        best.idx = q;
        best.ntie = 1;
    } else if (d2 == best.d2) {
        ++best.ntie;
        if (q < best.idx) best.idx = q;
    }
}
__device__ __forceinline__ double nn_dist2(const double* __restrict__ p, double qx, double qy, double qz) {
    double dx = __dsub_rn(p[0], qx), dy = __dsub_rn(p[1], qy), dz = __dsub_rn(p[2], qz);
    return __dadd_rn(__dadd_rn(__dmul_rn(dx, dx), __dmul_rn(dy, dy)), __dmul_rn(dz, dz));
}

__device__ __forceinline__ void nn_column(const GridGeom& g, const unsigned long long* __restrict__ bitmap,
                                          const unsigned* __restrict__ rank, const double* __restrict__ pts, int ix, int iy,
                                          int z0, int z1, double qx, double qy, double qz, NNBest& best,
                                          const unsigned char* __restrict__ ok = nullptr) {
    if (ix < 0 || iy < 0 || ix >= g.nx || iy >= g.ny) return;
    z0 = z0 < 0 ? 0 : z0;
    z1 = z1 >= g.nz ? g.nz - 1 : z1;
    if (z1 < z0) return;
    long long colw = ((long long)ix * g.ny + iy) * (g.nzp >> 6);
    for (int w = z0 >> 6; w <= z1 >> 6; ++w) {
        unsigned long long word = bitmap[colw + w];
        if (!word) continue;
        int b0 = w * 64;
        int lo = z0 - b0 < 0 ? 0 : z0 - b0, hi = z1 - b0 > 63 ? 63 : z1 - b0;
        unsigned long long m = (hi >= 63 ? ~0ull : ((1ull << (hi + 1)) - 1ull)) & ~((1ull << lo) - 1ull);
        unsigned long long sel = word & m;
        if (!sel) continue;
        unsigned base = rank[colw + w];
        while (sel) {
            int b = __ffsll(sel) - 1;
            sel &= sel - 1;
            int q = (int)(base + (unsigned)__popcll(word & ((1ull << b) - 1ull)));
            if (ok && !ok[q]) continue;
            nn_consider(best, q, nn_dist2(pts + (size_t)q * 3, qx, qy, qz));
        }
    }
}

__device__ inline void nn_rings(const NNIndex& I, int cx, int cy, int cz, double qx, double qy, double qz, NNBest& best,
                                const unsigned char* __restrict__ ok = nullptr) {
    const GridGeom& g = I.g;
    const int rmax = max(g.nx, max(g.ny, g.nz));
    for (int r = 1; r <= rmax; ++r) {
        if (r == 1) {
            for (int dx = -1; dx <= 1; ++dx)
                for (int dy = -1; dy <= 1; ++dy) nn_column(g, I.bitmap, I.rank, I.pts, cx + dx, cy + dy, cz - 1, cz + 1, qx, qy, qz, best, ok);
        } else {
            for (int dx = -r; dx <= r; ++dx)
                for (int dy = -r; dy <= r; ++dy) {
                    bool rim = (dx == -r || dx == r || dy == -r || dy == r);
                    if (rim) {
                        nn_column(g, I.bitmap, I.rank, I.pts, cx + dx, cy + dy, cz - r, cz + r, qx, qy, qz, best, ok);
                    } else {
                        nn_column(g, I.bitmap, I.rank, I.pts, cx + dx, cy + dy, cz - r, cz - r, qx, qy, qz, best, ok);
                        nn_column(g, I.bitmap, I.rank, I.pts, cx + dx, cy + dy, cz + r, cz + r, qx, qy, qz, best, ok);
                    }
                }
        }
        double m = 1e300;
        bool open = false;
        if (cx - r > 0) { m = fmin(m, qx - (g.ox + (cx - r) * g.vs)); open = true; }
        if (cx + r < g.nx - 1) { m = fmin(m, (g.ox + (cx + r + 1) * g.vs) - qx); open = true; }
        if (cy - r > 0) { m = fmin(m, qy - (g.oy + (cy - r) * g.vs)); open = true; }
        if (cy + r < g.ny - 1) { m = fmin(m, (g.oy + (cy + r + 1) * g.vs) - qy); open = true; }
        if (cz - r > 0) { m = fmin(m, qz - (g.oz + (cz - r) * g.vs)); open = true; }
        if (cz + r < g.nz - 1) { m = fmin(m, (g.oz + (cz + r + 1) * g.vs) - qz); open = true; }
        if (!open) break;
        m -= 1e-9;
        if (best.idx >= 0 && m > 0.0 && best.d2 < m * m) break;
    }
}

__device__ inline int nn_search_subset(const NNIndex& I, const unsigned char* __restrict__ ok, double qx, double qy, double qz,
                                       int* out_ntie) {
    const GridGeom& g = I.g;
    int cx, cy, cz;
    cell_of(g, qx, qy, qz, cx, cy, cz);
    NNBest best{1e300, -1, 0};
    cx = cx < 0 ? 0 : (cx >= g.nx ? g.nx - 1 : cx);
    cy = cy < 0 ? 0 : (cy >= g.ny ? g.ny - 1 : cy);
    cz = cz < 0 ? 0 : (cz >= g.nz ? g.nz - 1 : cz);
    nn_rings(I, cx, cy, cz, qx, qy, qz, best, ok);
    if (out_ntie) *out_ntie = best.ntie;
    return best.idx;
}

__device__ inline int nn_search(const NNIndex& I, double qx, double qy, double qz, double* out_d2 = nullptr,
                                int* out_ntie = nullptr) {
    const GridGeom& g = I.g;
    int cx, cy, cz;
    cell_of(g, qx, qy, qz, cx, cy, cz);
    NNBest best{1e300, -1, 0};
    const bool inside = cx >= 0 && cy >= 0 && cz >= 0 && cx < g.nx && cy < g.ny && cz < g.nz;
    bool done = false;
    if (inside && I.bitmap_rm) {
        long long lin = lin_of(g, cx, cy, cz);
        unsigned long long bit = 1ull << (lin & 63);
        unsigned long long wr = I.bitmap_rm[lin >> 6];
        if (wr & bit) {
            unsigned r = I.rank_rm[lin >> 6] + (unsigned)__popcll(wr & (bit - 1ull));
            for (unsigned k = I.cand_off[r]; k < I.cand_off[r + 1]; ++k) {
                int q = I.cand[k];
                nn_consider(best, q, nn_dist2(I.pts + (size_t)q * 3, qx, qy, qz));
            }
            done = best.idx >= 0;
        }
    }
    if (!done) {
        cx = cx < 0 ? 0 : (cx >= g.nx ? g.nx - 1 : cx);
        cy = cy < 0 ? 0 : (cy >= g.ny ? g.ny - 1 : cy);
        cz = cz < 0 ? 0 : (cz >= g.nz ? g.nz - 1 : cz);
        nn_rings(I, cx, cy, cz, qx, qy, qz, best);
    }
    if (out_d2) *out_d2 = best.d2;
    if (out_ntie) *out_ntie = best.ntie;
    return best.idx;
}

struct TieBuf {
    DevBuf<unsigned> count;
    DevBuf<TieRec> recs;
    DevBuf<long long> pq;
    DevBuf<int> pv;
    unsigned cap = 0;
    void prepare(hipStream_t s, unsigned want_cap = 1u << 16) {
        if (cap < want_cap) {
            recs.alloc(want_cap);
            cap = want_cap;
        }
        if (!count.p) count.alloc(1);
        HIP_TRY(hipMemsetAsync(count.p, 0, 4, s));
    }
    TieList list() { return TieList{count.p, recs.p, cap}; }
};
bool hmsg_resolve_ties(hmsg_ctx* h, TieBuf& tb, int* target);

static inline NNIndex hmsg_nn_index(const hmsg_ctx* h) {
    NNIndex I;
    I.g = h->grid;
    I.bitmap = h->bitmap.p;
    I.rank = h->rank.p;
    I.pts = h->pts.p;
    I.bitmap_rm = h->have_cand ? h->bitmap_rm.p : nullptr;
    I.rank_rm = h->rank_rm.p;
    I.cand_off = h->cand_off.p;
    I.cand = h->cand.p;
    return I;
}
```

### holoagent_amd/csrc/hmsg_pool.hip

```cpp
#include "hmsg_cloudops.h"
#include "hmsg_nn.h"
#include "hmsg_dbscan.h"

#include <algorithm>
#include <cmath>

typedef float f32x16 __attribute__((ext_vector_type(16)));

__global__ void k_pool_nn(const double* __restrict__ q, long long N, NNIndex I, double max_dist, int* __restrict__ idx,
                          unsigned* __restrict__ valid, TieList ties) {
    long long i = (long long)blockIdx.x * blockDim.x + threadIdx.x;
    if (i >= N) return;
    double d2 = 0;
    int ntie = 0;
    int v = nn_search(I, q[i * 3], q[i * 3 + 1], q[i * 3 + 2], &d2, &ntie);
    if (ntie > 1) tie_push(ties, i, q[i * 3], q[i * 3 + 1], q[i * 3 + 2]);
    idx[i] = v;
    valid[i] = (v >= 0 && __dsqrt_rn(d2) <= max_dist) ? 1u : 0u;
}

__global__ void k_pool_gather(const int* __restrict__ idx, const unsigned* __restrict__ valid, const unsigned* __restrict__ pos,
                              long long N, const float* __restrict__ feats, int D, float* __restrict__ X, float* __restrict__ Xn) {
    const int lane = threadIdx.x & 63;
    const long long i = ((long long)blockIdx.x * blockDim.x + threadIdx.x) >> 6;
    if (i >= N || !valid[i]) return;
    const float* src = feats + (size_t)idx[i] * D;
    float* dx = X + (size_t)pos[i] * D;
    float* dn = Xn + (size_t)pos[i] * D;
    float n2 = 0.f;
    for (int e = lane; e < D; e += 64) {
        float v = src[e];
        if (v != v) v = 0.f;
        else if (v > 3.4028234663852886e38f) v = 3.4028234663852886e38f;
        else if (v < -3.4028234663852886e38f) v = -3.4028234663852886e38f;
        dx[e] = v;
        n2 += v * v;
    }
    float nrm = __fsqrt_rn(wave_sum_f32(n2));
    if (nrm == 0.f) nrm = 1.f;
    for (int e = lane; e < D; e += 64) dn[e] = __fdiv_rn(dx[e], nrm);
}

#define GRAM_SUP 8
__device__ __forceinline__ void gram_tile_of(long long t, int nt, int& ti, int& tj) {
    int I = 0, r0 = 0, hgt = 0;
    for (;;) {
        r0 = I * GRAM_SUP;
        hgt = min(nt, r0 + GRAM_SUP) - r0;
        const long long cnt = (long long)hgt * (nt - r0) - (long long)hgt * (hgt - 1) / 2;
        if (t < cnt) break;
        t -= cnt;
        ++I;
    }
    const long long dcnt = (long long)hgt * (hgt + 1) / 2;
    if (t < dcnt) {
        int r = 0, len = hgt;
        while (t >= len) {
            t -= len;
            --len;
            ++r;
        }
        ti = r0 + r;
        tj = ti + (int)t;
        return;
    }
    t -= dcnt;
    for (int J = I + 1;; ++J) {
        const int w = min(GRAM_SUP, nt - J * GRAM_SUP);
        const long long c = (long long)hgt * w;
        if (t < c) {
            ti = r0 + (int)(t / w);
            tj = J * GRAM_SUP + (int)(t % w);
            return;
        }
        t -= c;
    }
}
__global__ void __launch_bounds__(256) k_pool_gram(const float* __restrict__ Xn, int D, const PoolSeg* __restrict__ segs, int K,
                                                   float eps, unsigned* __restrict__ adj, unsigned* __restrict__ ncount) {
    __shared__ float sa[GRAM_T][33];
    __shared__ float sb[GRAM_T][33];
    const int tid = threadIdx.x, lane = tid & 63, wv = tid >> 6, wr = wv >> 1, wc = wv & 1;
    const long long tile = blockIdx.x;
    int lo = 0, hi = K - 1;
    while (lo < hi) {
        int mid = (lo + hi + 1) >> 1;
        if (segs[mid].tile_base <= tile) lo = mid; else hi = mid - 1;
    }
    const PoolSeg sg = segs[lo];
    int ti, tj;
    gram_tile_of(tile - sg.tile_base, sg.nt, ti, tj);
    const int r0 = ti * GRAM_T, c0 = tj * GRAM_T;
    f32x16 acc[2][2];
    for (int i = 0; i < 2; ++i)
        for (int j = 0; j < 2; ++j)
            for (int r = 0; r < 16; ++r) acc[i][j][r] = 0.f;
    const float* base = Xn + (size_t)sg.row_base * D;
    const int lrow = tid >> 1, lk = (tid & 1) * 16;
    const bool vec_ok = (D & 3) == 0;
    const int ra = min(r0 + lrow, sg.n - 1), rb = min(c0 + lrow, sg.n - 1);
    for (int k0 = 0; k0 < D; k0 += 32) {
        if (vec_ok && k0 + lk + 16 <= D) {
            const float4* pa = reinterpret_cast<const float4*>(base + (size_t)ra * D + k0 + lk);
            const float4* pb = reinterpret_cast<const float4*>(base + (size_t)rb * D + k0 + lk);
            for (int u = 0; u < 4; ++u) {
                const float4 va = pa[u], vb = pb[u];
                sa[lrow][lk + 4 * u] = va.x; sa[lrow][lk + 4 * u + 1] = va.y; sa[lrow][lk + 4 * u + 2] = va.z; sa[lrow][lk + 4 * u + 3] = va.w;
                sb[lrow][lk + 4 * u] = vb.x; sb[lrow][lk + 4 * u + 1] = vb.y; sb[lrow][lk + 4 * u + 2] = vb.z; sb[lrow][lk + 4 * u + 3] = vb.w;
            }
        } else {
            for (int u = 0; u < 16; ++u) {
                int k = k0 + lk + u;
                sa[lrow][lk + u] = k < D ? base[(size_t)ra * D + k] : 0.f;
                sb[lrow][lk + u] = k < D ? base[(size_t)rb * D + k] : 0.f;
            }
        }
        __syncthreads();
        for (int k = 0; k < 32; k += 2) {
            const int kk = k + (lane >> 5);
            const float a0 = sa[wr * 64 + (lane & 31)][kk], a1 = sa[wr * 64 + 32 + (lane & 31)][kk];
            const float b0 = sb[wc * 64 + (lane & 31)][kk], b1 = sb[wc * 64 + 32 + (lane & 31)][kk];
            acc[0][0] = __builtin_amdgcn_mfma_f32_32x32x2f32(a0, b0, acc[0][0], 0, 0, 0);
            acc[0][1] = __builtin_amdgcn_mfma_f32_32x32x2f32(a0, b1, acc[0][1], 0, 0, 0);
            acc[1][0] = __builtin_amdgcn_mfma_f32_32x32x2f32(a1, b0, acc[1][0], 0, 0, 0);
            acc[1][1] = __builtin_amdgcn_mfma_f32_32x32x2f32(a1, b1, acc[1][1], 0, 0, 0);
        }
        __syncthreads();
    }
    const bool diag_tile = (ti == tj);
    for (int si = 0; si < 2; ++si)
        for (int sj = 0; sj < 2; ++sj) {
            const int rbase = r0 + wr * 64 + si * 32, cbase = c0 + wc * 64 + sj * 32;
            const int col = cbase + (lane & 31);
            unsigned mirror = 0u;
            for (int r = 0; r < 16; ++r) {
                const int rloc = (r & 3) + 8 * (r >> 2) + 4 * (lane >> 5);
                const int row = rbase + rloc;
                float d = __fadd_rn(-acc[si][sj][r], 1.0f);
                d = fminf(fmaxf(d, 0.f), 2.f);
                if (row == col) d = 0.f;
                const bool nb = row < sg.n && col < sg.n && d <= eps;
                mirror |= (nb ? 1u : 0u) << rloc;
                unsigned long long m = __ballot(nb);
                if ((lane & 31) == 0) {
                    unsigned word = (unsigned)(lane ? (m >> 32) : (m & 0xffffffffull));
                    if (row < sg.n && word) {
                        adj[sg.bit_base + (size_t)row * sg.nw + (cbase >> 5)] = word;
                        atomicAdd(&ncount[sg.row_base + row], (unsigned)__popc(word));
                    }
                }
            }
            if (!diag_tile) {
                unsigned other = __shfl_xor(mirror, 32);
                unsigned word = mirror | other;
                if (lane < 32 && col < sg.n && word) {
                    adj[sg.bit_base + (size_t)col * sg.nw + (rbase >> 5)] = word;
                    atomicAdd(&ncount[sg.row_base + col], (unsigned)__popc(word));
                }
// ... 117 lines not shown
                long long j = sg.row_base + (long long)w * 32 + b;
                if (ncount[j] >= (unsigned)minpts) best = label[j] < best ? label[j] : best;
            }
        }
        for (int o = 32; o > 0; o >>= 1) {
            int t = __shfl_xor(best, o);
            best = t < best ? t : best;
        }
        if (best == 0x7fffffff) best = -1;
    }
    if (lane == 0) {
        final_label[i] = best;
        if (best >= 0) {
            atomicAdd(&csize[sg.row_base + best], 1u);
            atomicMin(&cfirst[sg.row_base + best], (unsigned)(i - sg.row_base));
        }
    }
}
__global__ void k_pool_pick(const PoolSeg* __restrict__ segs, const int* __restrict__ seg_of_row, long long N,
                            const unsigned* __restrict__ csize, const unsigned* __restrict__ cfirst,
                            unsigned long long* __restrict__ best) {
    long long i = (long long)blockIdx.x * blockDim.x + threadIdx.x;
    if (i >= N || csize[i] == 0u) return;
    unsigned long long key = ((unsigned long long)csize[i] << 32) | (unsigned long long)(0xffffffffu - cfirst[i]);
    atomicMax(&best[seg_of_row[i]], key);
}
#define POOL_MEAN_AHEAD 16
__global__ void k_pool_mean(const float* __restrict__ X, int D, const PoolSeg* __restrict__ segs, int K,
                            const int* __restrict__ final_label, const unsigned* __restrict__ csize,
                            const unsigned* __restrict__ cfirst, const unsigned long long* __restrict__ best,
                            float* __restrict__ out) {
    const int k = blockIdx.y;
    const int d = blockIdx.x * blockDim.x + threadIdx.x;
    if (d >= D) return;
    const PoolSeg sg = segs[k];
    float* o = out + (size_t)k * D;
    if (sg.n == 0) {
        o[d] = 0.f;
        return;
    }
    int want = -2;
    unsigned long long key = best[k];
    if (key) {
        unsigned first = 0xffffffffu - (unsigned)(key & 0xffffffffull);
        want = final_label[sg.row_base + first];
    }
    float acc = 0.f;
    unsigned cnt = 0;
    const float* const xb = X + (size_t)sg.row_base * D + d;
    const int* const lb = final_label + sg.row_base;
    float cur[POOL_MEAN_AHEAD], nxt[POOL_MEAN_AHEAD];
    int curl[POOL_MEAN_AHEAD], nxtl[POOL_MEAN_AHEAD];
#pragma unroll
    for (int j = 0; j < POOL_MEAN_AHEAD; ++j) {
        const int rr = min(j, sg.n - 1);
        cur[j] = xb[(size_t)rr * D];
        curl[j] = lb[rr];
    }
    for (int r = 0; r < sg.n; r += POOL_MEAN_AHEAD) {
        if (r + POOL_MEAN_AHEAD < sg.n) {
#pragma unroll
            for (int j = 0; j < POOL_MEAN_AHEAD; ++j) {
                const int rr = min(r + POOL_MEAN_AHEAD + j, sg.n - 1);
                nxt[j] = xb[(size_t)rr * D];
                nxtl[j] = lb[rr];
            }
        }
#pragma unroll
        for (int j = 0; j < POOL_MEAN_AHEAD; ++j) {
            if (r + j < sg.n && (want == -2 || curl[j] == want)) {
                acc = __fadd_rn(acc, cur[j]);
                ++cnt;
            }
        }
#pragma unroll
        for (int j = 0; j < POOL_MEAN_AHEAD; ++j) {
            cur[j] = nxt[j];
            curl[j] = nxtl[j];
        }
    }
    o[d] = cnt > 1 ? __fdiv_rn(acc, (float)cnt) : acc;
}

__global__ void k_pool_gather_u32(const unsigned* __restrict__ src, const long long* __restrict__ idx, int n,
                                  unsigned* __restrict__ dst) {
    int t = blockIdx.x * blockDim.x + threadIdx.x;
    if (t < n) dst[t] = src[idx[t]];
}
__global__ void k_seg_rows(const PoolSeg* __restrict__ segs, int* __restrict__ seg_of_row) {
    const PoolSeg sg = segs[blockIdx.y];
    for (int i = blockIdx.x * blockDim.x + threadIdx.x; i < sg.n; i += gridDim.x * blockDim.x) seg_of_row[sg.row_base + i] = blockIdx.y;
}

void pool_cluster(hipStream_t s, const PoolSeg* d_ps, long long R, int minpts, const unsigned* adj, const unsigned* ncount,
                  const int* seg_of_row, int* label, int* seg_first, int* d_changed, int* flabel, unsigned* csize, unsigned* cfirst,
                  unsigned long long* best, DbgLaps* laps) {
    hipLaunchKernelGGL(k_pool_init, dim3(cdiv((size_t)R, 256)), dim3(256), 0, s, ncount, (long long)R,
                       minpts, label, d_ps, seg_of_row, seg_first);
    HMSG_CHECK_LAUNCH();
    DevBuf<unsigned> open_list;
    open_list.alloc((size_t)std::max<long long>(R, 1) + 1);
    const unsigned* d_list = nullptr;
    unsigned n_open = 0;
    static const bool list_wanted = getenv("HMSG_DEBUG_POOL_ALL_ROWS") == nullptr;
    for (int it = 0; it < 100000; ++it) {
        HIP_TRY(hipMemsetAsync(d_changed, 0, 4, s));
        const size_t rows = d_list ? (size_t)n_open : (size_t)R;
        for (int rep = 0; rep < (it == 0 ? 2 : 1) && rows; ++rep) {
            hipLaunchKernelGGL(k_pool_prop, dim3(cdiv(rows * 64, 256)), dim3(256), 0, s, adj,
                               d_ps, seg_of_row, ncount,
                               minpts, (long long)rows, label, d_changed, seg_first, (it == 0 && rep == 0) ? 1 : 0, d_list);
            hipLaunchKernelGGL(k_pool_jump, dim3(cdiv(rows, 256)), dim3(256), 0, s, d_ps,
                               seg_of_row, ncount, minpts, (long long)rows, label, d_list);
        }
        HMSG_CHECK_LAUNCH();
        if (it == 0 && list_wanted) {
            HIP_TRY(hipMemsetAsync(open_list.p, 0, 4, s));
            hipLaunchKernelGGL(k_pool_list, dim3(cdiv((size_t)R, 256)), dim3(256), 0, s, d_ps, seg_of_row,
                               ncount, minpts, (long long)R, label, seg_first,
                               open_list.p + 1, open_list.p);
            HMSG_CHECK_LAUNCH();
            HIP_TRY(hipMemcpyAsync(&n_open, open_list.p, 4, hipMemcpyDeviceToHost, s));
        }
        int ch = 0;
        HIP_TRY(hipMemcpyAsync(&ch, d_changed, 4, hipMemcpyDeviceToHost, s));
        HIP_TRY(hipStreamSynchronize(s));
        if (it == 0 && list_wanted) d_list = open_list.p + 1;
        if (!ch) break;
    }
    if (laps) laps->lap("label propagation");
    hipLaunchKernelGGL(k_pool_border, dim3(cdiv((size_t)R * 64, 256)), dim3(256), 0, s, adj,
                       d_ps, seg_of_row, ncount, minpts,
                       (long long)R, label, flabel, csize, cfirst);
    hipLaunchKernelGGL(k_pool_pick, dim3(cdiv((size_t)R, 256)), dim3(256), 0, s, d_ps,
                       seg_of_row, (long long)R, csize, cfirst, best);
    HMSG_CHECK_LAUNCH();
}

void pool_launch_gram_f32(hipStream_t s, const float* Xn, int D, const PoolSeg* d_ps, int K, long long tiles, float eps, unsigned* adj,
                          unsigned* ncount) {
    hipLaunchKernelGGL(k_pool_gram, dim3((unsigned)tiles), dim3(256), 0, s, Xn, D, d_ps, K, eps, adj, ncount);
    HMSG_CHECK_LAUNCH();
}
void pool_launch_seg_rows(hipStream_t s, const PoolSeg* d_ps, int K, int maxn, int* seg_of_row) {
    hipLaunchKernelGGL(k_seg_rows, dim3(std::max(1u, std::min(cdiv(maxn, 256), 256u)), K), dim3(256), 0, s, d_ps, seg_of_row);
    HMSG_CHECK_LAUNCH();
}
void pool_launch_mean_f32(hipStream_t s, const float* X, int D, const PoolSeg* d_ps, int K, const int* flabel, const unsigned* csize,
                          const unsigned* cfirst, const unsigned long long* best, float* out) {
    hipLaunchKernelGGL(k_pool_mean, dim3(cdiv(D, 64), K), dim3(64), 0, s, X, D, d_ps, K, flabel, csize, cfirst, best, out);
    HMSG_CHECK_LAUNCH();
}

void hmsg_pool(hmsg_ctx* h) {
    const hmsg_config& c = h->cfg;
    hipStream_t s = h->stream;
    HMSG_REQUIRE(h->merged, HMSG_ERR_INVALID, "hmsg_pool_instances: run hmsg_merge_instances first");
    const int K = (int)h->inst.off.size() - 1;
    const int D = c.feat_dim;
    h->inst_feats.alloc((size_t)std::max(K, 1) * D);
    if (K == 0) {
        h->pooled = true;
        return;
    }
    CloudOps ops;
    ops.s = s;
    DbgLaps laps("pool", s);
    std::vector<SegDesc> segs(K);
    for (int k = 0; k < K; ++k) {
        segs[k].pt_base = h->inst.off[k];
        segs[k].n = (int)(h->inst.off[k + 1] - h->inst.off[k]);
    }
    ops.bounds(h->inst.pts.p, segs);
    DevBuf<double> ds;
    ds.alloc((size_t)std::max<long long>(h->inst.total, 1) * 3);
    std::vector<int> dn;
    const long long P = ops.voxel_down_sample(h->inst.pts.p, segs, c.voxel_size, ds.p, dn);
    laps.lap("voxel_down_sample");
    DevBuf<int> idx;
    DevBuf<unsigned> valid, pos;
    idx.alloc((size_t)std::max<long long>(P, 1));
    valid.alloc((size_t)std::max<long long>(P, 1));
    pos.alloc((size_t)std::max<long long>(P, 1));
    if (P) {
        TieBuf ties;
        for (;;) {
            ties.prepare(s);
            hipLaunchKernelGGL(k_pool_nn, dim3(cdiv((size_t)P, 256)), dim3(256), 0, s, (const double*)ds.p, P, hmsg_nn_index(h),
                               c.pool_max_dist, idx.p, valid.p, ties.list());
            HMSG_CHECK_LAUNCH();
            if (hmsg_resolve_ties(h, ties, idx.p)) break;
        }
    }
    laps.lap("nearest map voxel");
    unsigned long long R = 0;
    if (P) hmsg_scan_u32(valid.p, pos.p, (size_t)P, s, ops.scan_tmp, &R);
    std::vector<long long> pstart(K + 1, 0);
    for (int k = 0; k < K; ++k) pstart[k + 1] = pstart[k] + dn[k];
    std::vector<unsigned> hpos(K + 1, (unsigned)R);
    {
        DevBuf<long long> d_i;
        DevBuf<unsigned> d_o;
        std::vector<long long> q;
        std::vector<int> which;
        for (int k = 0; k < K; ++k)
            if (pstart[k] < P) {
                q.push_back(pstart[k]);
                which.push_back(k);
            }
        if (!q.empty()) {
            std::vector<unsigned> tmp(q.size());
            d_i.alloc(q.size());
            d_o.alloc(q.size());
            HIP_TRY(hipMemcpyAsync(d_i.p, q.data(), q.size() * 8, hipMemcpyHostToDevice, s));
            hipLaunchKernelGGL(k_pool_gather_u32, dim3(cdiv(q.size(), 256)), dim3(256), 0, s, (const unsigned*)pos.p,
                               (const long long*)d_i.p, (int)q.size(), d_o.p);
            HIP_TRY(hipMemcpyAsync(tmp.data(), d_o.p, q.size() * 4, hipMemcpyDeviceToHost, s));
            HIP_TRY(hipStreamSynchronize(s));
            for (size_t t = 0; t < q.size(); ++t) hpos[which[t]] = tmp[t];
        }
        for (int k = K - 1; k >= 0; --k)
            if (pstart[k] >= P) hpos[k] = hpos[k + 1];
    }
    std::vector<PoolSeg> ps(K);
    long long bitw = 0, tiles = 0;
    int maxn = 0;
    for (int k = 0; k < K; ++k) {
        PoolSeg& g = ps[k];
        g.row_base = hpos[k];
        g.n = (int)(hpos[k + 1] - hpos[k]);
        g.nw = (g.n + 31) / 32;
        g.nt = (g.n + GRAM_T - 1) / GRAM_T;
        g.bit_base = bitw;
        g.tile_base = tiles;
        g.pad = 0;
        bitw += (long long)g.n * g.nw;
        tiles += (long long)g.nt * (g.nt + 1) / 2;
        maxn = std::max(maxn, g.n);
    }
    DevBuf<PoolSeg> d_ps;
    d_ps.alloc(K);
    HIP_TRY(hipMemcpyAsync(d_ps.p, ps.data(), (size_t)K * sizeof(PoolSeg), hipMemcpyHostToDevice, s));
    DevBuf<float> X, Xn;
    DevBuf<unsigned> adj, ncount, csize, cfirst;
    DevBuf<int> label, flabel, seg_of_row, d_changed, seg_first;
    DevBuf<unsigned long long> best;
    const size_t Rn = (size_t)std::max<unsigned long long>(R, 1);
    X.alloc(Rn * D);
    Xn.alloc(Rn * D);
    adj.alloc((size_t)std::max<long long>(bitw, 1));
    ncount.alloc(Rn);
    csize.alloc(Rn);
    cfirst.alloc(Rn);
    label.alloc(Rn);
    flabel.alloc(Rn);
    seg_of_row.alloc(Rn);
    d_changed.alloc(1);
    seg_first.alloc((size_t)std::max(K, 1));
    HIP_TRY(hipMemsetAsync(seg_first.p, 0x7f, (size_t)std::max(K, 1) * 4, s));
    best.alloc(K);
    adj.zero(s);
    ncount.zero(s);
    csize.zero(s);
    HIP_TRY(hipMemsetAsync(cfirst.p, 0xff, Rn * 4, s));
    best.zero(s);
    laps.lap("row offsets + buffers");
    if (R) {
        hipLaunchKernelGGL(k_pool_gather, dim3(cdiv((size_t)P * 64, 256)), dim3(256), 0, s, (const int*)idx.p,
                           (const unsigned*)valid.p, (const unsigned*)pos.p, P, (const float*)h->feats.p, D, X.p, Xn.p);
        hipLaunchKernelGGL(k_seg_rows, dim3(std::max(1u, std::min(cdiv(maxn, 256), 256u)), K), dim3(256), 0, s,
                           (const PoolSeg*)d_ps.p, seg_of_row.p);
        laps.lap("gather + normalise");
        {
            double flop = 0;
            for (auto& g : ps) flop += (double)g.n * ((double)g.n + 1.0) * D;
            ProfScope psc(h->prof, s, "k_pool_gram", flop);
            hipLaunchKernelGGL(k_pool_gram, dim3((unsigned)tiles), dim3(256), 0, s, (const float*)Xn.p, D, (const PoolSeg*)d_ps.p, K,
                               (float)c.feat_dbscan_eps, adj.p, ncount.p);
        }
        laps.lap("k_pool_gram");
        pool_cluster(s, (const PoolSeg*)d_ps.p, (long long)R, c.feat_dbscan_min, (const unsigned*)adj.p, (const unsigned*)ncount.p,
                     (const int*)seg_of_row.p, label.p, seg_first.p, d_changed.p, flabel.p, csize.p, cfirst.p, best.p, &laps);
    }
    laps.lap("border + pick");
    hmsg_dump("pool_ds", ds.p, (size_t)P * 24, s);
    hmsg_dump("pool_idx", idx.p, (size_t)P * 4, s);
    hmsg_dump("pool_valid", valid.p, (size_t)P * 4, s);
    hmsg_dump("pool_ncount", ncount.p, (size_t)R * 4, s);
    hmsg_dump("pool_flabel", flabel.p, (size_t)R * 4, s);
    hmsg_dump("pool_label", label.p, (size_t)R * 4, s);
    hmsg_dump("pool_segs", d_ps.p, (size_t)K * sizeof(PoolSeg), s);
    hipLaunchKernelGGL(k_pool_mean, dim3(cdiv(D, 64), K), dim3(64), 0, s, (const float*)X.p, D, (const PoolSeg*)d_ps.p, K,
                       (const int*)flabel.p, (const unsigned*)csize.p, (const unsigned*)cfirst.p,
                       (const unsigned long long*)best.p, h->inst_feats.p);
    HMSG_CHECK_LAUNCH();
    HIP_TRY(hipStreamSynchronize(s));
    laps.lap("k_pool_mean");
    h->pooled = true;
}
```

Before: 2673.

## Pool settled merge instances early on a background stream during the fold

Adds a background pooler thread and stream. It receives snapshots of instances that have stayed unchanged for a number of fold steps and computes their pooled features while the merge fold is still running. At pooling time, precomputed rows are matched by instance uid and point count, only the remaining instances are pooled, and a place kernel scatters all rows into the feature table. This aims to move pooling work off the critical path. In exchange it adds a second GPU stream that competes with the fold, extra copies, possible wasted work on instances that later change, and cancel logic wherever features are modified.

```diff
diff --git a/holoagent_amd/csrc/hmsg_api.hip b/holoagent_amd/csrc/hmsg_api.hip
--- a/holoagent_amd/csrc/hmsg_api.hip
+++ b/holoagent_amd/csrc/hmsg_api.hip
@@ -29,14 +29,14 @@
     h->kd_thread = std::thread([kd, pts, V] { kd->build(pts, V); });
 }
 
-bool hmsg_resolve_ties(hmsg_ctx* h, TieBuf& tb, int* target) {
+bool hmsg_resolve_ties(hmsg_ctx* h, TieBuf& tb, int* target, hipStream_t s, long long* answered) {
     unsigned n = 0;
-    HIP_TRY(hipMemcpyAsync(&n, tb.count.p, 4, hipMemcpyDeviceToHost, h->stream));
-    HIP_TRY(hipStreamSynchronize(h->stream));
+    HIP_TRY(hipMemcpyAsync(&n, tb.count.p, 4, hipMemcpyDeviceToHost, s));
+    HIP_TRY(hipStreamSynchronize(s));
     if (n == 0) return true;
     if (n > tb.cap) {
         tb.cap = 0;
-        tb.prepare(h->stream, n + n / 2 + 1024);
+        tb.prepare(s, n + n / 2 + 1024);
         return false;
     }
     std::vector<TieRec> recs(n);
@@ -51,15 +51,17 @@
     }
     tb.pq.ensure(n);
     tb.pv.ensure(n);
-    HIP_TRY(hipMemcpyAsync(tb.pq.p, q.data(), (size_t)n * 8, hipMemcpyHostToDevice, h->stream));
-    HIP_TRY(hipMemcpyAsync(tb.pv.p, v.data(), (size_t)n * 4, hipMemcpyHostToDevice, h->stream));
-    hipLaunchKernelGGL(k_nn_patch, dim3(cdiv(n, 256)), dim3(256), 0, h->stream, (const long long*)tb.pq.p, (const int*)tb.pv.p, n,
+    HIP_TRY(hipMemcpyAsync(tb.pq.p, q.data(), (size_t)n * 8, hipMemcpyHostToDevice, s));
+    HIP_TRY(hipMemcpyAsync(tb.pv.p, v.data(), (size_t)n * 4, hipMemcpyHostToDevice, s));
+    hipLaunchKernelGGL(k_nn_patch, dim3(cdiv(n, 256)), dim3(256), 0, s, (const long long*)tb.pq.p, (const int*)tb.pv.p, n,
                        target);
     HMSG_CHECK_LAUNCH();
-    HIP_TRY(hipStreamSynchronize(h->stream));
-    h->n_tie_queries += n;
+    HIP_TRY(hipStreamSynchronize(s));
+    *answered += n;
     return true;
 }
+
+bool hmsg_resolve_ties(hmsg_ctx* h, TieBuf& tb, int* target) { return hmsg_resolve_ties(h, tb, target, h->stream, &h->n_tie_queries); }
 
 namespace {
 
@@ -195,6 +197,8 @@
     } catch (...) {
     }
     h->fold_cache.trim();
+    h->pool_cache.trim();
+    if (h->pool_stream) (void)hipStreamDestroy(h->pool_stream);
     if (h->stream) {
         (void)hipStreamSynchronize(h->stream);
         (void)hipStreamDestroy(h->stream);
@@ -509,6 +513,7 @@
     return guard(h, [&] {
         HMSG_REQUIRE(h->feats_final && sum && counter, HMSG_ERR_INVALID, "hmsg_set_feature_sums: run hmsg_fuse_frames first");
         HMSG_REQUIRE(!h->pooled, HMSG_ERR_INVALID, "hmsg_set_feature_sums after hmsg_pool_instances");
+        hmsg_pool_ahead_cancel(h);
         const size_t n = (size_t)h->V * h->cfg.feat_dim;
         copy_in(h->sum.p, sum, n * 4, h->stream);
         copy_in(h->cnt.p, counter, (size_t)h->V * 4, h->stream);
diff --git a/holoagent_amd/csrc/hmsg_comm.hip b/holoagent_amd/csrc/hmsg_comm.hip
--- a/holoagent_amd/csrc/hmsg_comm.hip
+++ b/holoagent_amd/csrc/hmsg_comm.hip
@@ -288,6 +288,7 @@
         else if (h->pooled) mine = "hmsg_allreduce_feature_sums after hmsg_pool_instances";
         if (!all_ranks_ok(c, mine.empty(), s))
             throw hmsg_error{HMSG_ERR_INVALID, mine.empty() ? "hmsg_allreduce_feature_sums: another rank is not ready (see its hmsg_last_error)" : mine};
+        hmsg_pool_ahead_cancel(h);
         const size_t n = (size_t)h->V * h->cfg.feat_dim;
         if (c->comm && n) {
             rccl_try(rccl().AllReduce(h->sum.p, h->sum.p, n, RCCL_FLOAT32, RCCL_SUM, c->comm, s), "ncclAllReduce (feature sums)");
diff --git a/holoagent_amd/csrc/hmsg_common.h b/holoagent_amd/csrc/hmsg_common.h
--- a/holoagent_amd/csrc/hmsg_common.h
+++ b/holoagent_amd/csrc/hmsg_common.h
@@ -558,6 +558,10 @@
     std::shared_ptr<struct FoldPipe> fold_pipe;
     int fold_pipe_frames = 0;
     DevCache fold_cache;
+    std::shared_ptr<struct PoolAhead> pool_ahead;
+    DevCache pool_cache;
+    hipStream_t pool_stream = nullptr;
+    std::vector<unsigned long long> inst_uid;
     bool inst_denoised = false;
     std::vector<hmsg_node> nodes;
     DevBuf<int> room_sel, room_fmap;
@@ -664,6 +668,8 @@
 void hmsg_merge(hmsg_ctx* h);
 void hmsg_fold_pipe_feed(hmsg_ctx* h, int f0, int nfr);
 void hmsg_fold_pipe_abort(hmsg_ctx* h);
+void hmsg_pool_ahead_go(hmsg_ctx* h);
+void hmsg_pool_ahead_cancel(hmsg_ctx* h);
 void hmsg_merge_tree_local_impl(hmsg_ctx* h, int total_frames, double* th_next, long long* lists_now, long long* my_index);
 void hmsg_merge_tree_join_impl(hmsg_ctx* h, int n_ext, const long long* ext_sizes, const double* ext_pts, double th, int final_pass);
 void hmsg_denoise_inst(hmsg_ctx* h, double eps, int min_points);
diff --git a/holoagent_amd/csrc/hmsg_fuse.hip b/holoagent_amd/csrc/hmsg_fuse.hip
--- a/holoagent_amd/csrc/hmsg_fuse.hip
+++ b/holoagent_amd/csrc/hmsg_fuse.hip
@@ -624,6 +624,7 @@
     hipStream_t s = h->stream;
     HMSG_REQUIRE(h->map_ready, HMSG_ERR_INVALID, "hmsg_fuse_frames: call hmsg_finalize_map first");
     HMSG_REQUIRE(!h->feats_final || h->n_fused == h->n_feat_frames, HMSG_ERR_INVALID, "feature map already finalised");
+    hmsg_pool_ahead_cancel(h);
     const int H = c.height, W = c.width, D = c.feat_dim, MS = h->MS, NW = h->NW;
     const size_t HW = (size_t)H * W;
     const long long V = h->V;
@@ -814,6 +815,7 @@
     HMSG_CHECK_LAUNCH();
     HIP_TRY(hipStreamSynchronize(s));
     h->feats_final = true;
+    if (h->fold_pipe && h->fold_pipe_frames == h->n_fused) hmsg_pool_ahead_go(h);
 }
 
 void hmsg_bitset_and_fp(hmsg_ctx* h, int first, int n, int M, const unsigned char* d_masks, const float* d_fg,
diff --git a/holoagent_amd/csrc/hmsg_merge.hip b/holoagent_amd/csrc/hmsg_merge.hip
--- a/holoagent_amd/csrc/hmsg_merge.hip
+++ b/holoagent_amd/csrc/hmsg_merge.hip
@@ -1,10 +1,12 @@
 #include "hmsg_cloudops.h"
+#include "hmsg_pool_ahead.h"
 
 #include <algorithm>
 #include <cmath>
 #include <numeric>
 #include <chrono>
 #include <unordered_map>
+#include <unordered_set>
 #include <condition_variable>
 #include <deque>
 #include <mutex>
@@ -21,6 +23,7 @@
     bool raw = false;
     bool anchor = false;
     unsigned long long uid = 0;
+    int born = 0;
     unsigned id = 0;
     int cap = 0;
     bool has_index = false;
@@ -541,6 +544,7 @@
     size_t cursor_clean = 0;
     SpinWait spin;
     unsigned long long next_uid = 1;
+    int step_now = 0;
     std::unordered_map<unsigned long long, double> ratio_cache;
     bool use_cache = false;
     bool use_anchor = true;
@@ -1328,6 +1332,7 @@
             k.anchor = k.fixed && r.n_clusters >= 1 && (r.changed || r.n_clusters == 1);
             k.fresh = true;
             k.uid = next_uid++;
+            k.born = step_now;
             int f = -1;
             for (int i : mem)
                 if (L[i].n > 0) {
@@ -1458,8 +1463,10 @@
     std::vector<CatSeg> cat;
     h->inst.off.assign(1, 0);
     h->inst.box.clear();
+    h->inst_uid.clear();
     for (auto& k : result) {
         if (k.n < min_points) continue;
+        h->inst_uid.push_back(k.uid);
         for (int a = 0; a < 3; ++a) h->inst.box.push_back(k.mn[a]);
         for (int a = 0; a < 3; ++a) h->inst.box.push_back(k.mx[a]);
         cat.push_back(CatSeg{k.off, keep_total, k.n, 0, (int)cat_blocks, 0});
@@ -1587,6 +1594,41 @@
     bool incremental = false, never = false;
     int f_switch = -1;
     double batch_mean = 0.0, switch_points = 1500000.0;
+    PoolAhead* ahead = nullptr;
+    int ahead_every = 64, ahead_quiet = 64;
+    std::unordered_set<unsigned long long> ahead_handed;
+    std::vector<std::unique_ptr<PoolAheadJob>> ahead_done;
+    int fail_at = -1;
+
+    void hand_over(size_t f) {
+        hmsg_pool_ahead_reap(ahead, ahead_done);
+        ahead_done.clear();
+        if (f % (size_t)ahead_every != 0) return;
+        std::vector<CatSeg> cat;
+        long long total = 0;
+        unsigned blocks = 0;
+        std::unique_ptr<PoolAheadJob> job(new PoolAheadJob());
+        for (auto& k : G) {
+            if (k.n < h->cfg.min_instance_points || (long long)f - k.born < ahead_quiet || ahead_handed.count(k.uid)) continue;
+            cat.push_back(CatSeg{k.off, total, k.n, 0, (int)blocks, 0});
+            blocks += cdiv((size_t)k.n, CAT_CHUNK);
+            total += k.n;
+            job->uid.push_back(k.uid);
+            job->n.push_back(k.n);
+        }
+        if (cat.empty()) return;
+        for (unsigned long long u : job->uid) ahead_handed.insert(u);
+        job->pts.alloc((size_t)total * 3);
+        job->tab.alloc(cat.size() * sizeof(CatSeg));
+        job->h_tab.assign((const char*)cat.data(), (const char*)cat.data() + cat.size() * sizeof(CatSeg));
+        HIP_TRY(hipMemcpyAsync(job->tab.p, job->h_tab.data(), job->h_tab.size(), hipMemcpyHostToDevice, m.s));
+        hipLaunchKernelGGL(k_concat, dim3(blocks), dim3(256), 0, m.s, (const double*)m.pool.p, (const CatSeg*)job->tab.p, (int)cat.size(),
+                           job->pts.p, (const unsigned char*)nullptr, (unsigned char*)nullptr, CAT_CHUNK);
+        HMSG_CHECK_LAUNCH();
+        HIP_TRY(hipEventCreateWithFlags(&job->ready, hipEventDisableTiming));
+        HIP_TRY(hipEventRecord(job->ready, m.s));
+        hmsg_pool_ahead_push(ahead, std::move(job));
+    }
 
     void init(hmsg_ctx* hh, hipStream_t stream, Prof* prof) {
         h = hh;
@@ -1599,6 +1641,8 @@
         switch_points = getenv("HMSG_FOLD_INCREMENTAL") ? 0.0 : 1500000.0;
         if (const char* e = getenv("HMSG_FOLD_SWITCH")) switch_points = atof(e);
         if (const char* e = getenv("HMSG_FOLD_BIG_ACTIVE")) m.big_active = atoll(e);
+        if (const char* e = getenv("HMSG_DEBUG_FOLD_FAIL_AT")) fail_at = atoi(e);
+        hmsg_pool_ahead_config(&ahead_every, &ahead_quiet);
     }
     void ingest(const double* src, long long npts, const long long* off, const std::vector<int>& nm, long long reserve) {
         if (m.pool.n == 0) {
@@ -1633,6 +1677,7 @@
                 k.n = sd.n;
                 k.raw = true;
                 k.uid = m.next_uid++;
+                k.born = (int)frames.size() - 1;
                 for (int a = 0; a < 3; ++a) {
                     k.mn[a] = sd.mn[a];
                     k.mx[a] = sd.mx[a];
@@ -1642,8 +1687,15 @@
     }
     bool pending() const { return f_next < frames.size(); }
     void step(bool input_complete) {
+        const size_t f = f_next;
+        HMSG_REQUIRE(fail_at < 0 || (int)f != fail_at, HMSG_ERR_INVALID, "merge fold: failure requested (HMSG_DEBUG_FOLD_FAIL_AT)");
+        fold_frame(input_complete);
+        if (ahead) hand_over(f);
+    }
+    void fold_frame(bool input_complete) {
         const hmsg_config& c = h->cfg;
         const size_t f = f_next++;
+        m.step_now = (int)f;
         if (f == 0) {
             G = std::move(frames[0]);
             std::vector<Cloud>().swap(frames[0]);
@@ -1679,6 +1731,7 @@
     }
     void finish() {
         const hmsg_config& c = h->cfg;
+        m.step_now = (int)f_next;
         std::vector<Cloud> result = incremental ? m.fold_step(std::move(G), c.init_overlap_thresh) : m.merge_3d_masks(std::move(G), c.init_overlap_thresh);
         if (getenv("HMSG_DEBUG_TIMING") && incremental) {
             fprintf(stderr, "[hmsg merge] incremental fold from frame %d of %zu\n", f_switch, frames.size());
@@ -1704,6 +1757,7 @@
     bool closed = false, aborted = false, failed = false;
     hmsg_error err{HMSG_OK, ""};
     Prof prof;
+    std::shared_ptr<PoolAhead> ahead;
     std::vector<std::unique_ptr<Batch>> spent;
 
     void run() {
@@ -1717,6 +1771,16 @@
             {
                 SeqFold sf;
                 sf.init(h, s, &prof);
+                sf.ahead = ahead.get();
+                struct Reap {
+                    SeqFold& sf;
+                    hipStream_t s;
+                    ~Reap() {
+                        if (!sf.ahead) return;
+                        (void)hipStreamSynchronize(s);
+                        hmsg_pool_ahead_reap(sf.ahead, sf.ahead_done);
+                    }
+                } reap{sf, s};
                 for (;;) {
                     std::unique_ptr<Batch> b;
                     bool have = false, done = false, complete = false;
@@ -1799,6 +1863,8 @@
         if (f0 != 0) return;
         h->fold_pipe = std::make_shared<FoldPipe>();
         h->fold_pipe->h = h;
+        h->pool_ahead = hmsg_pool_ahead_create(h);
+        h->fold_pipe->ahead = h->pool_ahead;
         h->fold_pipe->prof.enabled = h->prof.enabled;
         FoldPipe* fp = h->fold_pipe.get();
         fp->th = std::thread([fp] { fp->run(); });
@@ -1819,11 +1885,15 @@
 }
 
 void hmsg_fold_pipe_abort(hmsg_ctx* h) {
-    if (!h->fold_pipe) return;
+    if (!h->fold_pipe) {
+        hmsg_pool_ahead_cancel(h);
+        return;
+    }
     h->fold_pipe->join(true);
     h->fold_pipe->prof.clear();
     h->fold_pipe.reset();
     h->fold_pipe_frames = 0;
+    hmsg_pool_ahead_cancel(h);
 }
 
 void hmsg_merge(hmsg_ctx* h) {
@@ -1839,7 +1909,10 @@
         h->fold_pipe_frames = 0;
         for (auto& e : fp->prof.ev) h->prof.ev.push_back(e);
         fp->prof.ev.clear();
-        if (fp->failed) throw fp->err;
+        if (fp->failed) {
+            hmsg_pool_ahead_cancel(h);
+            throw fp->err;
+        }
         h->merged = true;
         return;
     }
diff --git a/holoagent_amd/csrc/hmsg_nn.h b/holoagent_amd/csrc/hmsg_nn.h
--- a/holoagent_amd/csrc/hmsg_nn.h
+++ b/holoagent_amd/csrc/hmsg_nn.h
@@ -172,6 +172,7 @@
     TieList list() { return TieList{count.p, recs.p, cap}; }
 };
 bool hmsg_resolve_ties(hmsg_ctx* h, TieBuf& tb, int* target);
+bool hmsg_resolve_ties(hmsg_ctx* h, TieBuf& tb, int* target, hipStream_t s, long long* answered);
 
 static inline NNIndex hmsg_nn_index(const hmsg_ctx* h) {
     NNIndex I;
diff --git a/holoagent_amd/csrc/hmsg_pool.hip b/holoagent_amd/csrc/hmsg_pool.hip
--- a/holoagent_amd/csrc/hmsg_pool.hip
+++ b/holoagent_amd/csrc/hmsg_pool.hip
@@ -1,9 +1,16 @@
 #include "hmsg_cloudops.h"
 #include "hmsg_nn.h"
 #include "hmsg_dbscan.h"
+#include "hmsg_pool_ahead.h"
 
 #include <algorithm>
+#include <chrono>
 #include <cmath>
+#include <condition_variable>
+#include <deque>
+#include <mutex>
+#include <thread>
+#include <unordered_map>
 
 typedef float f32x16 __attribute__((ext_vector_type(16)));
 
@@ -427,31 +434,41 @@
     HMSG_CHECK_LAUNCH();
 }
 
-void hmsg_pool(hmsg_ctx* h) {
+__global__ void k_pool_place(const float* const* __restrict__ src, int K, int D, float* __restrict__ out) {
+    const size_t t = (size_t)blockIdx.x * blockDim.x + threadIdx.x;
+    if (t >= (size_t)K * D) return;
+    const int k = (int)(t / D), d = (int)(t % D);
+    out[t] = src[k][d];
+}
+
+__global__ void k_pool_take(const double* __restrict__ src, const long long* __restrict__ tab, double* __restrict__ dst) {
+    const long long from = tab[blockIdx.y * 3] * 3, to = tab[blockIdx.y * 3 + 1] * 3, n = tab[blockIdx.y * 3 + 2] * 3;
+    for (long long i = (long long)blockIdx.x * blockDim.x + threadIdx.x; i < n; i += (long long)gridDim.x * blockDim.x) dst[to + i] = src[from + i];
+}
+
+void hmsg_pool_ranges(hmsg_ctx* h, hipStream_t s, CloudOps& ops, const double* pts, const std::vector<PoolRange>& ranges, float* out,
+                      std::vector<double>* flop_of, Prof* prof, DbgLaps* laps, bool dumps, long long* ties_answered) {
     const hmsg_config& c = h->cfg;
-    hipStream_t s = h->stream;
-    HMSG_REQUIRE(h->merged, HMSG_ERR_INVALID, "hmsg_pool_instances: run hmsg_merge_instances first");
-    const int K = (int)h->inst.off.size() - 1;
+    const int K = (int)ranges.size();
     const int D = c.feat_dim;
-    h->inst_feats.alloc((size_t)std::max(K, 1) * D);
-    if (K == 0) {
-        h->pooled = true;
-        return;
-    }
-    CloudOps ops;
-    ops.s = s;
-    DbgLaps laps("pool", s);
+    if (flop_of) flop_of->assign((size_t)K, 0.0);
+    if (K == 0) return;
+    auto lap = [&](const char* what) {
+        if (laps) laps->lap(what);
+    };
     std::vector<SegDesc> segs(K);
+    long long total = 0;
     for (int k = 0; k < K; ++k) {
-        segs[k].pt_base = h->inst.off[k];
-        segs[k].n = (int)(h->inst.off[k + 1] - h->inst.off[k]);
-    }
-    ops.bounds(h->inst.pts.p, segs);
+        segs[k].pt_base = ranges[k].pt_base;
+        segs[k].n = ranges[k].n;
+        total += ranges[k].n;
+    }
+    ops.bounds(pts, segs);
     DevBuf<double> ds;
-    ds.alloc((size_t)std::max<long long>(h->inst.total, 1) * 3);
+    ds.alloc((size_t)std::max<long long>(total, 1) * 3);
     std::vector<int> dn;
-    const long long P = ops.voxel_down_sample(h->inst.pts.p, segs, c.voxel_size, ds.p, dn);
-    laps.lap("voxel_down_sample");
+    const long long P = ops.voxel_down_sample(pts, segs, c.voxel_size, ds.p, dn);
+    lap("voxel_down_sample");
     DevBuf<int> idx;
     DevBuf<unsigned> valid, pos;
     idx.alloc((size_t)std::max<long long>(P, 1));
@@ -464,10 +481,10 @@
             hipLaunchKernelGGL(k_pool_nn, dim3(cdiv((size_t)P, 256)), dim3(256), 0, s, (const double*)ds.p, P, hmsg_nn_index(h),
                                c.pool_max_dist, idx.p, valid.p, ties.list());
             HMSG_CHECK_LAUNCH();
-            if (hmsg_resolve_ties(h, ties, idx.p)) break;
-        }
-    }
-    laps.lap("nearest map voxel");
+            if (hmsg_resolve_ties(h, ties, idx.p, s, ties_answered)) break;
+        }
+    }
+    lap("nearest map voxel");
     unsigned long long R = 0;
     if (P) hmsg_scan_u32(valid.p, pos.p, (size_t)P, s, ops.scan_tmp, &R);
     std::vector<long long> pstart(K + 1, 0);
@@ -512,6 +529,7 @@
         bitw += (long long)g.n * g.nw;
         tiles += (long long)g.nt * (g.nt + 1) / 2;
         maxn = std::max(maxn, g.n);
+        if (flop_of) (*flop_of)[(size_t)k] = (double)g.n * ((double)g.n + 1.0) * D;
     }
     DevBuf<PoolSeg> d_ps;
     d_ps.alloc(K);
@@ -539,37 +557,292 @@
     csize.zero(s);
     HIP_TRY(hipMemsetAsync(cfirst.p, 0xff, Rn * 4, s));
     best.zero(s);
-    laps.lap("row offsets + buffers");
+    lap("row offsets + buffers");
     if (R) {
         hipLaunchKernelGGL(k_pool_gather, dim3(cdiv((size_t)P * 64, 256)), dim3(256), 0, s, (const int*)idx.p,
                            (const unsigned*)valid.p, (const unsigned*)pos.p, P, (const float*)h->feats.p, D, X.p, Xn.p);
         hipLaunchKernelGGL(k_seg_rows, dim3(std::max(1u, std::min(cdiv(maxn, 256), 256u)), K), dim3(256), 0, s,
                            (const PoolSeg*)d_ps.p, seg_of_row.p);
-        laps.lap("gather + normalise");
+        lap("gather + normalise");
         {
             double flop = 0;
             for (auto& g : ps) flop += (double)g.n * ((double)g.n + 1.0) * D;
-            ProfScope psc(h->prof, s, "k_pool_gram", flop);
+            ProfScope psc(prof, s, "k_pool_gram", flop);
             hipLaunchKernelGGL(k_pool_gram, dim3((unsigned)tiles), dim3(256), 0, s, (const float*)Xn.p, D, (const PoolSeg*)d_ps.p, K,
                                (float)c.feat_dbscan_eps, adj.p, ncount.p);
         }
-        laps.lap("k_pool_gram");
+        lap("k_pool_gram");
         pool_cluster(s, (const PoolSeg*)d_ps.p, (long long)R, c.feat_dbscan_min, (const unsigned*)adj.p, (const unsigned*)ncount.p,
-                     (const int*)seg_of_row.p, label.p, seg_first.p, d_changed.p, flabel.p, csize.p, cfirst.p, best.p, &laps);
-    }
-    laps.lap("border + pick");
-    hmsg_dump("pool_ds", ds.p, (size_t)P * 24, s);
-    hmsg_dump("pool_idx", idx.p, (size_t)P * 4, s);
-    hmsg_dump("pool_valid", valid.p, (size_t)P * 4, s);
-    hmsg_dump("pool_ncount", ncount.p, (size_t)R * 4, s);
-    hmsg_dump("pool_flabel", flabel.p, (size_t)R * 4, s);
-    hmsg_dump("pool_label", label.p, (size_t)R * 4, s);
-    hmsg_dump("pool_segs", d_ps.p, (size_t)K * sizeof(PoolSeg), s);
+                     (const int*)seg_of_row.p, label.p, seg_first.p, d_changed.p, flabel.p, csize.p, cfirst.p, best.p, laps);
+    }
+    lap("border + pick");
+    if (dumps) {
+        hmsg_dump("pool_ds", ds.p, (size_t)P * 24, s);
+        hmsg_dump("pool_idx", idx.p, (size_t)P * 4, s);
+        hmsg_dump("pool_valid", valid.p, (size_t)P * 4, s);
+        hmsg_dump("pool_ncount", ncount.p, (size_t)R * 4, s);
+        hmsg_dump("pool_flabel", flabel.p, (size_t)R * 4, s);
+        hmsg_dump("pool_label", label.p, (size_t)R * 4, s);
+        hmsg_dump("pool_segs", d_ps.p, (size_t)K * sizeof(PoolSeg), s);
+    }
     hipLaunchKernelGGL(k_pool_mean, dim3(cdiv(D, 64), K), dim3(64), 0, s, (const float*)X.p, D, (const PoolSeg*)d_ps.p, K,
                        (const int*)flabel.p, (const unsigned*)csize.p, (const unsigned*)cfirst.p,
-                       (const unsigned long long*)best.p, h->inst_feats.p);
+                       (const unsigned long long*)best.p, out);
     HMSG_CHECK_LAUNCH();
     HIP_TRY(hipStreamSynchronize(s));
-    laps.lap("k_pool_mean");
+    lap("k_pool_mean");
+}
+
+namespace {
+template <typename F>
+void with_cache(DevCache& cache, F&& fn) {
+    dev_cache().swap_state(cache);
+    fn();
+    cache.swap_state(dev_cache());
+}
+}
+
+struct PoolAhead {
+    struct Batch {
+        DevBuf<float> rows;
+        std::vector<unsigned long long> uid;
+        std::vector<int> n;
+        std::vector<double> flop;
+    };
+    hmsg_ctx* h = nullptr;
+    hipStream_t s = nullptr;
+    std::thread th;
+    std::mutex mu;
+    std::condition_variable cv;
+    std::deque<std::unique_ptr<PoolAheadJob>> q;
+    std::vector<std::unique_ptr<PoolAheadJob>> spent;
+    std::vector<std::unique_ptr<Batch>> batches;
+    bool go = false, stop = false, failed = false;
+    hmsg_error err{HMSG_OK, ""};
+    long long ties = 0;
+
+    void run() {
+        dev_cache().swap_state(h->pool_cache);
+        try {
+            HIP_TRY(hipSetDevice(h->cfg.device_id));
+            CloudOps ops;
+            ops.s = s;
+            const char* const dl = getenv("HMSG_DEBUG_POOL_AHEAD_DELAY_MS");
+            const int delay_ms = dl ? atoi(dl) : 0;
+            for (;;) {
+                std::unique_ptr<PoolAheadJob> job;
+                {
+                    std::unique_lock<std::mutex> lk(mu);
+                    cv.wait(lk, [&] { return stop || (go && !q.empty()); });
+                    if (stop) break;
+                    job = std::move(q.front());
+                    q.pop_front();
+                }
+                std::unique_ptr<Batch> b(new Batch());
+                try {
+                    if (delay_ms > 0) std::this_thread::sleep_for(std::chrono::milliseconds(delay_ms));
+                    HIP_TRY(hipEventSynchronize(job->ready));
+                    std::vector<PoolRange> ranges(job->n.size());
+                    long long at = 0;
+                    for (size_t i = 0; i < ranges.size(); ++i) {
+                        ranges[i] = PoolRange{at, job->n[i]};
+                        at += job->n[i];
+                    }
+                    b->uid = job->uid;
+                    b->n = job->n;
+                    b->rows.alloc(std::max<size_t>(ranges.size(), 1) * (size_t)h->cfg.feat_dim);
+                    hmsg_pool_ranges(h, s, ops, job->pts.p, ranges, b->rows.p, &b->flop, nullptr, nullptr, false, &ties);
+                } catch (...) {
+                    (void)hipStreamSynchronize(s);
+                    std::lock_guard<std::mutex> lk(mu);
+                    spent.push_back(std::move(job));
+                    throw;
+                }
+                std::lock_guard<std::mutex> lk(mu);
+                batches.push_back(std::move(b));
+                spent.push_back(std::move(job));
+            }
+        } catch (const hmsg_error& e) {
+            fail(e);
+        } catch (const std::exception& e) {
+            fail(hmsg_error{HMSG_ERR_HIP, e.what()});
+        } catch (...) {
+            fail(hmsg_error{HMSG_ERR_HIP, "early pooler: unknown exception"});
+        }
+        (void)hipStreamSynchronize(s);
+        h->pool_cache.swap_state(dev_cache());
+    }
+    void fail(const hmsg_error& e) {
+        std::lock_guard<std::mutex> lk(mu);
+        failed = true;
+        err = e;
+    }
+    void join() {
+        {
+            std::lock_guard<std::mutex> lk(mu);
+            stop = true;
+        }
+        cv.notify_all();
+        if (th.joinable()) th.join();
+    }
+    void drop(bool fold_done) {
+        with_cache(h->pool_cache, [&] { batches.clear(); });
+        std::lock_guard<std::mutex> lk(mu);
+        for (auto& j : q) spent.push_back(std::move(j));
+        q.clear();
+        if (fold_done) with_cache(h->fold_cache, [&] { spent.clear(); });
+    }
+};
+
+void hmsg_pool_ahead_config(int* every, int* quiet) {
+    const char* e = getenv("HMSG_POOL_AHEAD_EVERY");
+    const char* q = getenv("HMSG_POOL_AHEAD_QUIET");
+    *every = std::max(1, e ? atoi(e) : 64);
+    *quiet = std::max(0, q ? atoi(q) : 64);
+}
+
+std::shared_ptr<PoolAhead> hmsg_pool_ahead_create(hmsg_ctx* h) {
+    const char* sw = getenv("HMSG_POOL_AHEAD");
+    if (sw && atoi(sw) == 0) return nullptr;
+    if (!h->pool_stream) HIP_TRY(hipStreamCreateWithFlags(&h->pool_stream, hipStreamNonBlocking));
+    std::shared_ptr<PoolAhead> pa = std::make_shared<PoolAhead>();
+    pa->h = h;
+    pa->s = h->pool_stream;
+    PoolAhead* p = pa.get();
+    pa->th = std::thread([p] { p->run(); });
+    return pa;
+}
+
+void hmsg_pool_ahead_push(PoolAhead* pa, std::unique_ptr<PoolAheadJob> job) {
+    {
+        std::lock_guard<std::mutex> lk(pa->mu);
+        if (pa->stop || pa->failed) pa->spent.push_back(std::move(job));
+        else pa->q.push_back(std::move(job));
+    }
+    pa->cv.notify_all();
+}
+
+void hmsg_pool_ahead_reap(PoolAhead* pa, std::vector<std::unique_ptr<PoolAheadJob>>& done) {
+    std::lock_guard<std::mutex> lk(pa->mu);
+    for (auto& j : pa->spent) done.push_back(std::move(j));
+    pa->spent.clear();
+}
+
+void hmsg_pool_ahead_go(hmsg_ctx* h) {
+    if (!h->pool_ahead) return;
+    hmsg_kd_join(h);
+    {
+        std::lock_guard<std::mutex> lk(h->pool_ahead->mu);
+        h->pool_ahead->go = true;
+    }
+    h->pool_ahead->cv.notify_all();
+}
+
+void hmsg_pool_ahead_cancel(hmsg_ctx* h) {
+    if (!h->pool_ahead) return;
+    std::shared_ptr<PoolAhead> pa = h->pool_ahead;
+    h->pool_ahead.reset();
+    pa->join();
+    pa->drop(!h->fold_pipe);
+}
+
+void hmsg_pool(hmsg_ctx* h) {
+    const hmsg_config& c = h->cfg;
+    hipStream_t s = h->stream;
+    HMSG_REQUIRE(h->merged, HMSG_ERR_INVALID, "hmsg_pool_instances: run hmsg_merge_instances first");
+    const int K = (int)h->inst.off.size() - 1;
+    const int D = c.feat_dim;
+    std::shared_ptr<PoolAhead> pa = h->pool_ahead;
+    h->pool_ahead.reset();
+    if (pa) pa->join();
+    struct Dropper {
+        PoolAhead* p;
+        ~Dropper() {
+            if (p) p->drop(true);
+        }
+    } dropper{pa.get()};
+    if (pa && pa->failed) throw pa->err;
+    h->inst_feats.alloc((size_t)std::max(K, 1) * D);
+    if (K == 0) {
+        h->pooled = true;
+        return;
+    }
+    CloudOps ops;
+    ops.s = s;
+    DbgLaps laps("pool", s);
+    std::vector<const float*> src((size_t)K, nullptr);
+    double n_early = 0, f_early = 0, n_vain = 0, f_vain = 0, n_late = 0, f_late = 0;
+    if (pa && h->inst_uid.size() == (size_t)K) {
+        std::unordered_map<unsigned long long, std::pair<const PoolAhead::Batch*, size_t>> stored;
+        for (auto& b : pa->batches)
+            for (size_t i = 0; i < b->uid.size(); ++i) stored[b->uid[i]] = {b.get(), i};
+        for (int k = 0; k < K; ++k) {
+            auto it = stored.find(h->inst_uid[(size_t)k]);
+            if (it == stored.end()) continue;
+            const PoolAhead::Batch& b = *it->second.first;
+            const size_t i = it->second.second;
+            if ((long long)b.n[i] != h->inst.off[(size_t)k + 1] - h->inst.off[(size_t)k]) continue;
+            src[(size_t)k] = b.rows.p + i * (size_t)D;
+            n_early += 1;
+            f_early += b.flop[i];
+            stored.erase(it);
+        }
+        for (auto& kv : stored) {
+            n_vain += 1;
+            f_vain += kv.second.first->flop[kv.second.second];
+        }
+        h->n_tie_queries += pa->ties;
+    }
+    std::vector<PoolRange> late;
+    std::vector<int> late_k;
+    for (int k = 0; k < K; ++k)
+        if (!src[(size_t)k]) {
+            late.push_back(PoolRange{h->inst.off[(size_t)k], (int)(h->inst.off[(size_t)k + 1] - h->inst.off[(size_t)k])});
+            late_k.push_back(k);
+        }
+    std::vector<double> flop;
+    long long ties = 0;
+    if ((int)late.size() == K) {
+        hmsg_pool_ranges(h, s, ops, h->inst.pts.p, late, h->inst_feats.p, &flop, &h->prof, &laps, true, &ties);
+    } else {
+        DevBuf<float> rows;
+        rows.alloc(std::max<size_t>(late.size(), 1) * (size_t)D);
+        if (!late.empty()) {
+            std::vector<long long> tab(late.size() * 3);
+            long long total = 0;
+            int maxn = 0;
+            for (size_t j = 0; j < late.size(); ++j) {
+                tab[j * 3] = late[j].pt_base;
+                tab[j * 3 + 1] = total;
+                tab[j * 3 + 2] = late[j].n;
+                late[j].pt_base = total;
+                total += late[j].n;
+                maxn = std::max(maxn, late[j].n);
+            }
+            DevBuf<long long> d_tab;
+            DevBuf<double> lpts;
+            d_tab.alloc(tab.size());
+            lpts.alloc((size_t)std::max<long long>(total, 1) * 3);
+            HIP_TRY(hipMemcpyAsync(d_tab.p, tab.data(), tab.size() * 8, hipMemcpyHostToDevice, s));
+            hipLaunchKernelGGL(k_pool_take, dim3(std::max(1u, std::min(cdiv((size_t)maxn * 3, 256), 64u)), (unsigned)late.size()), dim3(256), 0, s,
+                               (const double*)h->inst.pts.p, (const long long*)d_tab.p, lpts.p);
+            HMSG_CHECK_LAUNCH();
+            HIP_TRY(hipStreamSynchronize(s));
+            hmsg_pool_ranges(h, s, ops, lpts.p, late, rows.p, &flop, &h->prof, &laps, true, &ties);
+        }
+        for (size_t j = 0; j < late.size(); ++j) src[(size_t)late_k[j]] = rows.p + j * (size_t)D;
+        DevBuf<const float*> d_src;
+        d_src.alloc((size_t)K);
+        HIP_TRY(hipMemcpyAsync(d_src.p, src.data(), (size_t)K * sizeof(const float*), hipMemcpyHostToDevice, s));
+        hipLaunchKernelGGL(k_pool_place, dim3(cdiv((size_t)K * D, 256)), dim3(256), 0, s, (const float* const*)d_src.p, K, D, h->inst_feats.p);
+        HMSG_CHECK_LAUNCH();
+        HIP_TRY(hipStreamSynchronize(s));
+        laps.lap("rows into the table");
+    }
+    h->n_tie_queries += ties;
+    for (double f : flop) n_late += 1, f_late += f;
+    if (getenv("HMSG_DEBUG_TIMING"))
+        fprintf(stderr, "[hmsg pool ahead] %s: instances pooled early %.0f (%.3f GFLOP of Gram)  at the end %.0f (%.3f GFLOP)  early in vain %.0f (%.3f GFLOP)\n",
+                pa ? "on" : "off", n_early, f_early * 1e-9, n_late, f_late * 1e-9, n_vain, f_vain * 1e-9);
     h->pooled = true;
 }
diff --git a/holoagent_amd/csrc/hmsg_pool_ahead.h b/holoagent_amd/csrc/hmsg_pool_ahead.h
--- /dev/null
+++ b/holoagent_amd/csrc/hmsg_pool_ahead.h
@@ -0,0 +1,33 @@
+#pragma once
+#include "hmsg_cloudops.h"
+
+#include <memory>
+
+struct PoolRange {
+    long long pt_base;
+    int n;
+};
+
+void hmsg_pool_ranges(hmsg_ctx* h, hipStream_t s, CloudOps& ops, const double* pts, const std::vector<PoolRange>& ranges, float* out,
+                      std::vector<double>* flop, Prof* prof, DbgLaps* laps, bool dumps, long long* ties);
+
+struct PoolAheadJob {
+    DevBuf<double> pts;
+    DevBuf<char> tab;
+    std::vector<char> h_tab;
+    std::vector<unsigned long long> uid;
+    std::vector<int> n;
+    hipEvent_t ready = nullptr;
+    PoolAheadJob() = default;
+    PoolAheadJob(const PoolAheadJob&) = delete;
+    PoolAheadJob& operator=(const PoolAheadJob&) = delete;
+    ~PoolAheadJob() {
+        if (ready) (void)hipEventDestroy(ready);
+    }
+};
+
+struct PoolAhead;
+std::shared_ptr<PoolAhead> hmsg_pool_ahead_create(hmsg_ctx* h);
+void hmsg_pool_ahead_config(int* every, int* quiet);
+void hmsg_pool_ahead_push(PoolAhead* pa, std::unique_ptr<PoolAheadJob> job);
+void hmsg_pool_ahead_reap(PoolAhead* pa, std::vector<std::unique_ptr<PoolAheadJob>>& done);
```

After: 2646. -1.0%, worse.
